# Infini-AI-Lab/TriForce

Measured on AMD Instinct MI355X. Metric: decode tokens/sec + avg accepted len, Llama-7B-128K @124K ctx, higher is better.
Workload: dtype f16

## Files before the change

### include/triforce_hip.h

```cpp
#ifndef TRIFORCE_HIP_H
#define TRIFORCE_HIP_H

#include <stdint.h>

#ifdef __cplusplus
extern "C" {
#endif

#define TF_OK        0
#define TF_EINVAL  (-22)
#define TF_ENOSPC  (-28)
#define TF_ERANGE  (-34)

int tf_abi_version(void);

int64_t tf_attn_decode_ws_floats(int H, int sq, int D, int nsplit);
int tf_attn_decode_pick_nsplit(int H, int sk);
int tf_attn_decode(const void* q, const void* k, const void* v, void* out,
                   int64_t stride_t, int64_t stride_h,
                   int sq, int sk, const int32_t* sk_dev, int H, int D, float scale,
                   int nsplit, float* ws, int64_t ws_floats, void* stream);
int tf_attn_decode_fused(const void* q, const void* k, const void* v, void* out,
                         int64_t stride_t, int64_t stride_h,
                         int sq, int sk, const int32_t* sk_dev, int H, int D, float scale,
                         int nsplit, float* ws, int64_t ws_floats, uint32_t* tickets, void* stream);
int tf_attn_decode_act(const void* q, const void* k, const void* v, void* out, int64_t out_sm, int64_t out_sk,
                       int64_t stride_t, int64_t stride_h, int sq, int sk, const int32_t* sk_dev, int H, int D,
                       float scale, int nsplit, float* ws, int64_t ws_floats, uint32_t* tickets, void* stream);
int tf_attn_tune(int key, int value);

int64_t tf_attn_block_ws_floats(int H, int D, int nsplit);
int tf_attn_block_pick_nsplit(int H, int sq, int sk);
int tf_attn_block(const void* q, const void* k, const void* v, void* out,
                  int64_t stride_t, int64_t stride_h, int sq, int sk, int H, int D, float scale,
                  int nsplit, float* ws, int64_t ws_floats,
                  const uint32_t* mask, int mask_words, int mask_row0, int tree_start, void* stream);

int tf_attn_prefill_pick_nsplit(int H, int sq, int sk);
int64_t tf_attn_prefill_ws_floats(int H, int sq, int D, int nsplit);
int tf_attn_prefill(const void* q, const void* k, const void* v, void* out,
                    int64_t stride_t, int64_t stride_h, int sq, int sk, int H, int D, float scale,
                    int nsplit, float* ws, int64_t ws_floats, void* stream);

int tf_attn_rope_on_read(const void* q, const void* k, const void* v, const void* cos, const void* sin,
                         void* out, int64_t stride_t, int64_t stride_h,
                         int sq, int kv_len, int H, int D, float scale, void* stream);

#define TF_DRAFT_MAX_LAYERS 8
typedef struct TfDraftModel {
    const void* embed;
    const void* ln1[TF_DRAFT_MAX_LAYERS];
    const void* wqkv[TF_DRAFT_MAX_LAYERS];
    const void* wo[TF_DRAFT_MAX_LAYERS];
    const void* ln2[TF_DRAFT_MAX_LAYERS];
    const void* wgate[TF_DRAFT_MAX_LAYERS];
    const void* wup[TF_DRAFT_MAX_LAYERS];
    const void* wdown[TF_DRAFT_MAX_LAYERS];
    const void* norm;
    const void* lm_head;
    const void* cos;
    const void* sin;
    int32_t layers, hidden, heads, head_dim, inter, vocab;
    float eps, scale;
} TfDraftModel;
typedef struct TfDraftCache {
    void* k[TF_DRAFT_MAX_LAYERS];
    void* v[TF_DRAFT_MAX_LAYERS];
    int64_t stride_t, stride_h;
} TfDraftCache;
int64_t tf_draft_forward_ws_bytes(const TfDraftModel* model, int n);
int tf_draft_forward_68m(const TfDraftModel* model, const TfDraftCache* cache, const int64_t* ids, int n, int slot0,
                         int kv_len, float* logits_out, float* probs_out, float temperature, float top_p,
                         void* ws, int64_t ws_bytes, void* stream);

int64_t tf_draft_persist_ctl_bytes(void);
int64_t tf_draft_persist_ws_bytes(const TfDraftModel* model);
int tf_draft_persist_supported(const TfDraftModel* model, int n, int kv_len);
int tf_draft_forward_68m_persist(const TfDraftModel* model, const TfDraftCache* cache, const int64_t* ids, int n, int slot0,
                                 int kv_len, float* logits_out, float* probs_out, float temperature, float top_p,
                                 void* ws, int64_t ws_bytes, void* ctl, void* stream);
int tf_draft_persist_tune(int key, int value);
int tf_draft_persist_stamps(void* buf);
int tf_draft_persist_error(const void* ctl);
int tf_draft_persist_reset(void* ctl, void* host_mirror, int set_mirror);

int tf_retrieval_score(const void* k, int64_t stride_t, int64_t stride_h, const void* q,
                       void* scores, int C, int chunk, int H, int D, void* stream);
int tf_retrieval_topk(const void* scores, int32_t* idx, int C, int sets, int H, void* stream);
int tf_retrieval_gather(const void* k_src, const void* v_src, int64_t src_stride_t, int64_t src_stride_h,
                        const int32_t* idx, void* k_dst, void* v_dst, int64_t dst_stride_t,
                        int64_t dst_stride_h, int sets, int chunk, int H, int D, void* stream);

int tf_chunk_mean(const void* k, int64_t stride_t, int64_t stride_h, void* index_layer, int64_t index_stride_h,
                  int c0, int c1, int chunk, int H, int D, void* stream);
int tf_retrieval_score_indexed(const void* index_layer, int64_t index_stride_h, const void* q, void* scores,
                               int C, int H, int D, void* stream);

int tf_kv_copy_rows(const void* src, int64_t src_stride_l, int64_t src_stride_t, int64_t src_stride_h,
                    void* dst, int64_t dst_stride_l, int64_t dst_stride_t, int64_t dst_stride_h,
                    int src_t0, int dst_t0, int n, int L, int H, int D, void* stream);
int tf_kv_shift_rows(void* cache, int64_t stride_l, int64_t stride_t, int64_t stride_h,
                     int src_t0, int dst_t0, int n, int L, int H, int D, void* stream);
int tf_kv_copy_rows_pair(const void* src_k, const void* src_v, int64_t src_stride_l, int64_t src_stride_t,
                         int64_t src_stride_h, void* dst_k, void* dst_v, int64_t dst_stride_l, int64_t dst_stride_t,
                         int64_t dst_stride_h, int src_t0, int dst_t0, int n, int L, int H, int D, void* stream);
int tf_kv_shift_rows_pair(void* k_cache, void* v_cache, int64_t stride_l, int64_t stride_t, int64_t stride_h,
                          int src_t0, int dst_t0, int n, int L, int H, int D, void* stream);

int tf_kv_gather_rows(void* k_cache, void* v_cache, int64_t stride_l, int64_t stride_t, int64_t stride_h,
                      int offset, const int32_t* idx, int n, int L, int H, int D, void* stream);

int tf_rmsnorm(const void* x, const void* res, const void* w, void* y, void* sum_out,
               int rows, int hidden, float eps, void* stream);
int tf_rope_append(const void* qkv, int64_t qkv_row_stride, const void* cos, const void* sin,
                   const int64_t* positions, void* q_out, void* k_cache, void* v_cache,
                   int64_t stride_t, int64_t stride_h, int slot0, const int32_t* slot0_dev,
                   int rows, int H, int D, int rotate_k, void* stream);
int tf_silu_mul(const void* gate_up, void* out, int rows, int I, void* stream);
int tf_embed_rows(const void* embed, const int64_t* ids, void* out, int64_t out_sm, int64_t out_sk, int n, int hidden,
                  int vocab, void* stream);
int tf_set_tokens(int64_t* dst, int n_dst, const int64_t* host_vals, int n_vals, int64_t pad, int64_t* pos, int n_pos,
                  int64_t pos0, int32_t* slot, int32_t* sk, int32_t sk_val, void* stream);

int tf_skinny_gemm(const void* w_packed, const void* x, int64_t ldx, void* y, int64_t ldy, int M, int N, int K,
                   int out_f32, void* stream);
int tf_skinny_gemm_swiglu(const void* gate_packed, const void* up_packed, const void* x, int64_t ldx, void* act,
                          int64_t ldy, int M, int I, int K, void* stream);

int tf_skinny_gemm_ex(const void* w_packed, const void* x, int64_t ldx, const void* ln_w, float eps,
                      const float* ss_in, const void* resid, int64_t ldr, float* ss_out, void* y, int64_t ldy,
                      int M, int N, int K, int out_f32, void* stream);
int tf_skinny_gemm_swiglu_ex(const void* gate_packed, const void* up_packed, const void* x, int64_t ldx,
                             const void* ln_w, float eps, const float* ss_in, void* act, int64_t ldy,
                             int M, int I, int K, void* stream);
int tf_skinny_qkv_rope(const void* wqkv_packed, const void* x, int64_t ldx, const void* ln_w, float eps,
                       const float* ss_in, const void* cos, const void* sin, const int64_t* positions, void* q_out,
                       void* k_cache, void* v_cache, int64_t stride_t, int64_t stride_h, int slot0,
                       const int32_t* slot0_dev, int M, int H, int D, int K, int rotate_k, void* stream);

int tf_skinny_gemm_act(const void* w_packed, const void* x, int64_t xs_m, int64_t xs_k, const void* ln_w, float eps,
                       const float* ss_in, const void* resid, int64_t rs_m, int64_t rs_k, float* ss_out, void* y,
                       int64_t ys_m, int64_t ys_k, int M, int N, int K, int out_f32, void* stream);
int tf_skinny_gemm_swiglu_act(const void* gate_packed, const void* up_packed, const void* x, int64_t xs_m,
                              int64_t xs_k, const void* ln_w, float eps, const float* ss_in, void* act, int64_t ys_m,
                              int64_t ys_k, int M, int I, int K, void* stream);
int tf_skinny_qkv_rope_act(const void* wqkv_packed, const void* x, int64_t xs_m, int64_t xs_k, const void* ln_w,
                           float eps, const float* ss_in, const void* cos, const void* sin, const int64_t* positions,
                           void* q_out, void* k_cache, void* v_cache, int64_t stride_t, int64_t stride_h, int slot0,
                           const int32_t* slot0_dev, int M, int H, int D, int K, int rotate_k, void* stream);
int tf_sg_tune(int key, int value);
int tf_skinny_gemm_swiglu_n8(const void* gate_n8, const void* up_n8, const void* x, int64_t xs_m, int64_t xs_k,
                             const void* ln_w, float eps, const float* ss_in, void* act, int64_t ys_m, int64_t ys_k,
                             int M, int I, int K, void* stream);
int tf_skinny_qkv_rope_n8(const void* wqkv_n8, const void* x, int64_t xs_m, int64_t xs_k, const void* ln_w, float eps,
                          const float* ss_in, const void* cos, const void* sin, const int64_t* positions, void* q_out,
                          void* k_cache, void* v_cache, int64_t stride_t, int64_t stride_h, int slot0,
                          const int32_t* slot0_dev, int M, int H, int D, int K, int rotate_k, void* stream);
int tf_skinny_gemm_fp8_act(const void* w_fp8, const float* scale, const void* x, int64_t xs_m, int64_t xs_k,
                           const void* ln_w, float eps, const float* ss_in, const void* resid, int64_t rs_m, int64_t rs_k,
                           float* ss_out, void* y, int64_t ys_m, int64_t ys_k, int M, int N, int K, int out_f32,
                           void* stream);
int tf_skinny_gemm_swiglu_fp8_act(const void* gate_fp8, const float* gate_scale, const void* up_fp8,
                                  const float* up_scale, const void* x, int64_t xs_m, int64_t xs_k, const void* ln_w,
                                  float eps, const float* ss_in, void* act, int64_t ys_m, int64_t ys_k, int M, int I, int K,
                                  void* stream);
int tf_skinny_qkv_rope_fp8_act(const void* wqkv_fp8, const float* scale, const void* x, int64_t xs_m, int64_t xs_k,
                               const void* ln_w, float eps, const float* ss_in, const void* cos, const void* sin,
                               const int64_t* positions, void* q_out, void* k_cache, void* v_cache, int64_t stride_t,
                               int64_t stride_h, int slot0, const int32_t* slot0_dev, int M, int H, int D, int K,
                               int rotate_k, void* stream);
int tf_kv_quant_rows(const void* k_in, const void* v_in, int64_t in_stride_t, int64_t in_stride_h, void* k_codes,
                     void* v_codes, void* k_exp, void* v_exp, int64_t code_stride_t, int64_t code_stride_h,
                     int64_t exp_stride_h, int slot0, const int32_t* slot0_dev, int n, int H, int D, void* k_deq,
                     void* v_deq, void* stream);
int tf_attn_decode_fp8_act(const void* q, const void* k_codes, const void* v_codes, const void* k_exp, const void* v_exp,
                           void* out, int64_t out_sm, int64_t out_sk, int64_t stride_t, int64_t stride_h,
                           int64_t exp_stride_h, int sq, int sk, const int32_t* sk_dev, int H, int D, float scale,
                           int nsplit, float* ws, int64_t ws_floats, uint32_t* tickets, void* stream);
int tf_kv_dequant_rows_pair(const void* src_k, const void* src_v, int64_t src_stride_l, int64_t src_stride_t,
                            int64_t src_stride_h, const void* exp_k, const void* exp_v, int64_t exp_stride_l,
                            int64_t exp_stride_h, void* dst_k, void* dst_v, int64_t dst_stride_l, int64_t dst_stride_t,
                            int64_t dst_stride_h, int src_t0, int dst_t0, int n, int L, int H, int D, void* stream);
int tf_retrieval_gather_fp8(const void* k_src, const void* v_src, int64_t src_stride_t, int64_t src_stride_h,
                            const void* k_src_exp, const void* v_src_exp, int64_t src_exp_stride_h, const int32_t* idx,
                            void* k_codes, void* v_codes, void* k_exp, void* v_exp, int64_t code_stride_t,
                            int64_t code_stride_h, int64_t exp_stride_h, int sets, int chunk, int H, int D, void* stream);
int tf_kv_quant_rows_pair(const void* src_k, const void* src_v, int64_t src_stride_l, int64_t src_stride_t,
                          int64_t src_stride_h, const void* src_exp_k, const void* src_exp_v, int64_t src_exp_stride_l,
                          int64_t src_exp_stride_h, void* k_codes, void* v_codes, int64_t code_stride_l,
                          int64_t code_stride_t, int64_t code_stride_h, void* k_exp, void* v_exp, int64_t exp_stride_l,
                          int64_t exp_stride_h, int src_t0, int dst_t0, int n, int L, int H, int D, void* stream);
int tf_attn_decode_fp8_tail_act(const void* q, const void* k_codes, const void* v_codes, const void* k_exp, const void* v_exp,
                                const void* k_tail, const void* v_tail, void* out, int64_t out_sm, int64_t out_sk,
                                int64_t stride_t, int64_t stride_h, int64_t exp_stride_h, int64_t tail_stride_t,
                                int64_t tail_stride_h, int sq, int sk_codes, int n_tail, const int32_t* sk_dev, int H, int D,
                                float scale, int nsplit, float* ws, int64_t ws_floats, uint32_t* tickets, void* stream);
int tf_sg_workspace(void* ws, int64_t bytes);

int tf_topp_probs(const float* logits, float* probs, int rows, int V, float temperature, float top_p, void* stream);
int tf_topk_topp_probs(const float* logits, float* probs, int rows, int V, float temperature, int top_k, float top_p,
                       void* stream);
int tf_sample_inverse_cdf(const float* probs, const float* u, int64_t* token_out, int V, void* stream);
int tf_accept_chain(const float* p, const float* q, const int64_t* tokens, const float* uniforms,
                    int g2, int V, int inclusive, int64_t eos_token_id, int64_t* out, void* stream);
int tf_middle_accept(const float* p, const float* q_d, int64_t* tokens, const float* uniforms,
                     int n, int gamma, int V, int64_t* out, void* stream);
int tf_mid_record_tokens(const int64_t* rec, int64_t* tokens, int tokens_len, int n, void* stream);
int64_t tf_topp_multi_ctl_bytes(void);
int64_t tf_topp_multi_ws_bytes(int rows, int V);
int tf_topp_probs_multi(const float* logits, const float* panel_max, float* probs, int rows, int V, float temperature,
                        float top_p, void* ctl, void* ws, int64_t ws_bytes, void* stream);
int tf_topp_multi_tune(int key, int value);
int tf_topp_multi_error(const void* ctl);
int tf_topp_multi_reset(void* ctl);

int tf_sample_inverse_cdf_cur(const float* probs, const float* ubuf, const int64_t* cursor, int off, int64_t* token_out,
                              int V, void* stream);
int tf_middle_accept_cur(const float* p, const float* q_d, int64_t* tokens, int tokens_len, const float* ubuf,
                         int64_t* cursor, int n, int gamma, int V, int64_t* out, void* stream);
int tf_accept_chain_cur(const float* p, const float* q, const int64_t* tokens, const float* ubuf, int64_t* cursor, int g2,
                        int V, int inclusive, int64_t eos_token_id, int64_t* out, void* stream);
int tf_accept_chain_step(const float* p, const float* q, int64_t* tok_buf, int tok_len, const float* ubuf, int64_t* cursor,
                         int g2, int V, int inclusive, int64_t eos_token_id, int64_t pad, const int32_t* s_src, int nsets,
                         int64_t* pos_a, int n_pos_a, int32_t* slot_a, int32_t* sk_a, int qlen_a, int64_t* pos_b, int n_pos_b,
                         int32_t* slot_b, int32_t* sk_b, int qlen_b, int64_t* out, void* stream);

int tf_tree_accept(const float* p_rows, const float* draft_logits, const int64_t* tokens,
                   const int32_t* succ_off, const int32_t* succ, const float* uniforms, int V,
                   float temperature, int64_t* out, void* stream);

int tf_sample_without_replacement(const float* logits, const void* rand_f16, int64_t* out, int rows, int V, int k,
                                  float temperature, void* stream);

int tf_kv_h2d_async(void* dst_dev, int64_t dst_pitch_elems, const void* src_host, int64_t src_pitch_elems,
                    int64_t width_elems, int H, void* copy_stream);
int tf_kv_d2h_async(void* dst_host, int64_t dst_pitch_elems, const void* src_dev, int64_t src_pitch_elems,
                    int64_t width_elems, int H, void* copy_stream);

int tf_ar_flags_bytes(void);
int tf_ar_ipc_handle_bytes(void);
int tf_ar_alloc(int64_t bytes, void** ptr);
int tf_ar_free(void* ptr);
int tf_ar_get_ipc_handle(void* ptr, void* handle_out);
int tf_ar_open_ipc_handle(const void* handle, void** ptr_out);
int tf_ar_close_ipc_handle(void* ptr);
int tf_allreduce_oneshot(void* const* peer_data, void* const* peer_flags, int rank, int world, void* out, int64_t n,
                         void* stream);
int tf_allreduce_oneshot_add(void* const* peer_data, void* const* peer_flags, int rank, int world, const void* resid,
                             void* out, int64_t n, void* stream);
int tf_allreduce_oneshot_add_ss(void* const* peer_data, void* const* peer_flags, int rank, int world, const void* resid,
                                void* out, int64_t n, int hidden, float* ss_out, void* stream);
int tf_allreduce_oneshot_alt(void* const* peer_data, void* const* peer_flags, int rank, int world, const void* resid,
                             void* out, int64_t n, int hidden, float* ss_out, int64_t half_elems, int expect_half,
                             void* stream);
int tf_allreduce_oneshot_act(void* const* peer_data, void* const* peer_flags, int rank, int world, const void* resid,
                             void* out, int64_t n, int hidden, int pack_rows, float* ss_out, int64_t half_elems,
                             int expect_half, void* stream);
int64_t tf_xchg_ctl_bytes(void);
int tf_skinny_gemm_xchg(const void* w_packed, const void* x, int64_t xs_m, int64_t xs_k, void* const* peer_stage,
                        void* const* peer_ctl, int rank, int world, int64_t half_elems, const void* resid, int64_t rs_m,
                        int64_t rs_k, void* out, int64_t os_m, int64_t os_k, float* ss_out, int M, int N, int K,
                        void* stream);
int tf_xchg_error(const void* ctl);
int tf_xchg_set_error(void* ctl, int code, void* host_mirror, int set_mirror);
int tf_xchg_tune(int key, int value);
int tf_xchg_reset(void* ctl);
int tf_ar_litmus_stage(void* staging, int64_t n, int rank, uint32_t* it_dev, void* stream);
int tf_ar_litmus_check(const void* out, int64_t n, int world, const uint32_t* it_dev, uint64_t* bad, void* stream);
int tf_ar_error(const void* flags_local);
int64_t tf_ar_epoch(const void* flags_local);
int tf_ar_set_error_mirror(void* flags_local, void* host_word);
int tf_ar_inject_error(void* flags_local, int code);

int tf_attn_decode_gqa_act(const void* q, const void* k, const void* v, void* out, int64_t out_sm, int64_t out_sk,
                           int64_t stride_t, int64_t stride_h, int sq, int sk, const int32_t* sk_dev, int H, int Hkv, int D,
                           float scale, int nsplit, float* ws, int64_t ws_floats, uint32_t* tickets, void* stream);
int tf_attn_prefill_gqa(const void* q, const void* k, const void* v, void* out, int64_t stride_t, int64_t stride_h,
                        int sq, int sk, int H, int Hkv, int D, float scale, int nsplit, float* ws, int64_t ws_floats,
                        void* stream);
int tf_skinny_qkv_rope_gqa_act(const void* wqkv_packed, const void* x, int64_t xs_m, int64_t xs_k, const void* ln_w,
                               float eps, const float* ss_in, const void* cos, const void* sin, const int64_t* positions,
                               void* q_out, void* k_cache, void* v_cache, int64_t stride_t, int64_t stride_h, int slot0,
                               const int32_t* slot0_dev, int M, int H, int Hkv, int D, int K, int rotate_k, void* stream);
int tf_rope_append_gqa(const void* qkv, int64_t qkv_row_stride, const void* cos, const void* sin,
                       const int64_t* positions, void* q_out, void* k_cache, void* v_cache,
                       int64_t stride_t, int64_t stride_h, int slot0, const int32_t* slot0_dev,
                       int rows, int H, int Hkv, int D, int rotate_k, void* stream);

#ifdef __cplusplus
}
#endif
#endif
```

### triforce_amd/build.py

```python
import os
import shutil
import subprocess

HERE = os.path.dirname(os.path.abspath(__file__))
CSRC = os.path.join(HERE, "csrc")
LIB_DIR = os.path.join(HERE, "lib")
LIB_PATH = os.path.join(LIB_DIR, "libtriforce_hip.so")
SOURCES = ["attn.hip", "retrieval.hip", "elementwise.hip", "sampling.hip", "offload.hip", "gemv.hip", "gemv_fp8.hip", "kv_fp8.hip", "allreduce.hip", "draft.hip", "draft_persist.hip", "topp_multi.hip", "abi.hip"]
FLAGS = ["--offload-arch=gfx950", "-O3", "-std=c++17", "-fPIC", "-shared", "-ffp-contract=off",
         "-fno-gpu-rdc", "-Wno-unused-result", "-mllvm", "-amdgpu-kernarg-preload-count=14"]


def hipcc_path():
    p = shutil.which("hipcc") or "/opt/rocm/bin/hipcc"
    if not os.path.exists(p):
        raise RuntimeError("hipcc not found: cannot build libtriforce_hip.so")
    return p


def sources():
    return [os.path.join(CSRC, s) for s in SOURCES if os.path.exists(os.path.join(CSRC, s))]


def needs_build():
    if not os.path.exists(LIB_PATH):
        return True
    t = os.path.getmtime(LIB_PATH)
    deps = sources() + [os.path.join(CSRC, "common.h"), os.path.join(CSRC, "tree_mask.h"), os.path.join(CSRC, "select_common.h"),
                        os.path.join(CSRC, "sg_rule.h"),
                        os.path.join(HERE, "..", "include", "triforce_hip.h"), os.path.abspath(__file__)]
    return any(os.path.getmtime(d) > t for d in deps if os.path.exists(d))


def build_variant(name, defines, verbose=True):
    out = os.path.join(LIB_DIR, f"libtriforce_hip_{name}.so")
    drop = {d[1:] for d in defines if d.startswith("!")}
    flags = [f for f in FLAGS if f not in drop]
    if "kernarg-preload" in drop:
        flags = [f for f in flags if f != "-mllvm" and not f.startswith("-amdgpu-kernarg-preload-count")]
    cmd = [hipcc_path()] + flags + [d if d.startswith("-") else f"-D{d}" for d in defines if not d.startswith("!")] \
        + sources() + ["-o", out]
    if verbose:
        print("[triforce_amd.build]", " ".join(cmd), flush=True)
    subprocess.run(cmd, check=True)
    return out


def build_library(force=False, verbose=True):
    if not force and not needs_build():
        return LIB_PATH
    os.makedirs(LIB_DIR, exist_ok=True)
    cmd = [hipcc_path()] + FLAGS + sources() + ["-o", LIB_PATH]
    if verbose:
        print("[triforce_amd.build]", " ".join(cmd), flush=True)
    subprocess.run(cmd, check=True)
    return LIB_PATH


if __name__ == "__main__":
    build_library(force=True)
```

### triforce_amd/csrc/gemv.hip

```cpp
#include "common.h"
#include "sg_rule.h"

#define SG_LOAD(p) __builtin_nontemporal_load(p)

constexpr int SG_U = 4;

struct SgAct {
    int64_t sm, sk;
};

struct SgKsplit {
    float* ws;
    unsigned* tickets;
    unsigned long long* stamps;
};
#ifndef SG_STAMPS
#define SG_STAMPS 0
#endif
#if SG_STAMPS
#define SG_STAMP(i)                                                                                                      \
    do {                                                                                                                 \
        if (tid == 0 && kx.stamps) {                                                                                     \
            kx.stamps[((int64_t)blockIdx.x * gridDim.y + blockIdx.y) * 16 + (i)] = __builtin_readcyclecounter();        \
            if ((i) == 0 || (i) == 6) kx.stamps[((int64_t)blockIdx.x * gridDim.y + blockIdx.y) * 16 + 8 + (i) / 6] = wall_clock64(); \
        }                                                                                                                \
    } while (0)
#else
#define SG_STAMP(i) do { } while (0)
#endif
static void* g_sg_ws[16] = {};
static int64_t g_sg_ws_bytes[16] = {};
#define SG_WS_SLOTS 4
static hipStream_t g_sg_slot_stream[16][SG_WS_SLOTS] = {};
static int g_sg_slots_used[16] = {};
#include <mutex>
static std::mutex g_sg_slot_mutex;
static int sg_slot_of(int dev, hipStream_t st) {
    std::lock_guard<std::mutex> lock(g_sg_slot_mutex);
    for (int i = 0; i < g_sg_slots_used[dev]; ++i)
        if (g_sg_slot_stream[dev][i] == st) return i;
    if (g_sg_slots_used[dev] >= SG_WS_SLOTS) return -1;
    g_sg_slot_stream[dev][g_sg_slots_used[dev]] = st;
    return g_sg_slots_used[dev]++;
}

static SgKnobs g_sg_knobs;

__device__ __forceinline__ void sg_st_agent(float* p, float v) { __hip_atomic_store(p, v, __ATOMIC_RELAXED, __HIP_MEMORY_SCOPE_AGENT); }
__device__ __forceinline__ float sg_ld_agent(const float* p) { return __hip_atomic_load(p, __ATOMIC_RELAXED, __HIP_MEMORY_SCOPE_AGENT); }

#define XC_MAXP 512
#define XC_MAX_WORLD 8
#define XC_SPIN_LIMIT (1u << 27)
#define XC_WALL_HZ 100000000ull
static int g_xc_timeout_ms = 5000;
static int g_xc_fence = 0;
struct XcCtl {
    unsigned epoch, ticket, error, pad;
    unsigned long long mirror;
};
#define XC_PEPOCH_OFF (1024 + XC_MAX_WORLD * XC_MAXP * 4)
struct SgXchg {
    h16* stage[XC_MAX_WORLD];
    unsigned* pf[XC_MAX_WORLD];
    XcCtl* ctl;
    unsigned* pepoch;
    int64_t half_elems;
    int rank, world;
    int fence;
    unsigned long long timeout_ticks;
};
__device__ __forceinline__ unsigned xc_ld(const unsigned* p) { return __hip_atomic_load(p, __ATOMIC_RELAXED, __HIP_MEMORY_SCOPE_SYSTEM); }
__device__ __forceinline__ void xc_st(unsigned* p, unsigned v) { __hip_atomic_store(p, v, __ATOMIC_RELAXED, __HIP_MEMORY_SCOPE_SYSTEM); }
__device__ __forceinline__ void xc_st8(h16* p, half4 v) {
    __hip_atomic_store(reinterpret_cast<unsigned long long*>(p), __builtin_bit_cast(unsigned long long, v), __ATOMIC_RELAXED,
                       __HIP_MEMORY_SCOPE_SYSTEM);
}
__device__ __forceinline__ half4 xc_ld8(const h16* p) {
    return __builtin_bit_cast(half4, __hip_atomic_load(reinterpret_cast<const unsigned long long*>(p), __ATOMIC_RELAXED,
                                                       __HIP_MEMORY_SCOPE_SYSTEM));
}

struct SgRope {
    const h16* cosb;
    const h16* sinb;
    const int64_t* positions;
    h16* q_out;
    h16* k_cache;
    h16* v_cache;
    int64_t stride_t, stride_h;
    const int32_t* slot0_dev;
    int slot0, H, D, rotate_k;
};

template <int MODE>
__device__ __forceinline__ void sg_rope_heads(const SgRope& rp, int& H, int& Hkv) {
    if (MODE == SG_QKVG) {
        H = rp.H & 0xffff;
        Hkv = rp.H >> 16;
    } else {
        H = Hkv = rp.H;
    }
}

__device__ __forceinline__ half8 sg_normalise(half8 xv, half8 wv, float inv) {
    half8 o;
#pragma unroll
    for (int e = 0; e < 8; ++e) o[e] = hmul_rn(wv[e], (h16)((float)xv[e] * inv));
    return o;
}

template <int MT, int MODE, bool NORM, int WAVES, int P, bool KSPLIT, bool XCHG = false>
__global__ __launch_bounds__(WAVES * 64) void skinny_gemm_kernel(const half8* __restrict__ wp,
                                                                 const half8* __restrict__ wp_up,
                                                                 const h16* __restrict__ x,
                                                                 const float* __restrict__ ss_in,
                                                                 const h16* __restrict__ ln_w, int K, int M,
                                                                 int xa_sm, int xa_sk, float eps, int N,
                                                                 const h16* resid, SgAct ra, void* yv, SgAct ya,
                                                                 SgRope rp, float* __restrict__ ss_out, SgKsplit kx,
                                                                 SgXchg xc) {
    const SgAct xa = {(int64_t)xa_sm, (int64_t)xa_sk};
    static_assert(!XCHG || (MODE == SG_PLAIN && P == 1 && !KSPLIT), "the exchange form is the plain one-panel GEMM");
    constexpr bool GATEUP = MODE == SG_GATEUP;
    constexpr int NA = GATEUP ? 2 : 1;
    constexpr int U = (P * NA >= 2) ? (8 / (P * NA)) : SG_U;
    static_assert(P <= WAVES && U >= 1, "one epilogue wave per panel");
    const int panel0 = blockIdx.x * P;
    const int tid = threadIdx.x, lane = tid & 63, wave = tid >> 6;
    const int li = lane & 15, g = lane >> 4;
    SG_STAMP(0);
    const int nchunks = K >> 5;
    const int KS = KSPLIT ? (int)gridDim.y : 1, ks = KSPLIT ? (int)blockIdx.y : 0;
    const int g0c = (int)((int64_t)nchunks * ks / KS), g1c = (int)((int64_t)nchunks * (ks + 1) / KS);
    const int cpw = (g1c - g0c + WAVES - 1) / WAVES;
    const int c0 = g0c + wave * cpw, c1 = min(g1c, c0 + cpw);

    __shared__ float sm[WAVES][P * NA][MT][64][4];
    __shared__ float sm_ss[NORM ? WAVES : 1][MT][16];

    f32x4 acc[P][NA][MT];
#pragma unroll
    for (int j = 0; j < P; ++j)
#pragma unroll
        for (int a = 0; a < NA; ++a)
#pragma unroll
            for (int t = 0; t < MT; ++t) acc[j][a][t] = f32x4{0.f, 0.f, 0.f, 0.f};
    const int64_t pstride = (int64_t)nchunks * 64;
    const half8* wa = wp + (int64_t)panel0 * pstride + lane;
    const half8* wu = GATEUP ? (wp_up + (int64_t)panel0 * pstride + lane) : nullptr;
    const int64_t xcs = 4 * xa.sk;
    const h16* xr[MT];
    bool xok[MT];
#pragma unroll
    for (int t = 0; t < MT; ++t) {
        const int m = t * 16 + li;
        xok[t] = m < M;
        xr[t] = x + (int64_t)(xok[t] ? m : 0) * xa.sm + (int64_t)g * xa.sk;
    }
    const half8 zero8 = {0, 0, 0, 0, 0, 0, 0, 0};

    constexpr int SSB = MT == 1 ? 3 : 2;
    constexpr bool BPRE = MT == 1;
    constexpr int G = WAVES * 4;
    const int nparts = K >> 4;
    const int pg = tid >> 4, m16 = tid & 15;
    float ssv[MT][SSB][8], part0[MT];
    half8 a_pre[U][P][NA], b_pre[BPRE ? U : 1][MT];
    const bool pre = NORM && (c0 + U <= c1);
    if constexpr (NORM) {
        const float* ssp = ss_in ? ss_in : reinterpret_cast<const float*>(wp);
#pragma unroll
        for (int t = 0; t < MT; ++t)
#pragma unroll
            for (int bb = 0; bb < SSB; ++bb)
#pragma unroll
                for (int j = 0; j < 8; ++j) {
                    const int p = pg + bb * 8 * G + j * G;
                    const float v = ssp[(int64_t)min(p, nparts - 1) * 32 + t * 16 + m16];
                    ssv[t][bb][j] = (p < nparts) ? v : 0.f;
                }
        if constexpr (BPRE) {
#pragma unroll
            for (int u = 0; u < U; ++u) {
                const int cu = min(c0 + u, nchunks - 1);
#pragma unroll
                for (int t = 0; t < MT; ++t) {
                    const half8 v = load_half8(xr[t] + xcs * cu);
                    b_pre[u][t] = xok[t] ? v : zero8;
                }
            }
        }
#pragma unroll
        for (int u = 0; u < U; ++u) {
            const int cu = min(c0 + u, nchunks - 1);
#pragma unroll
            for (int j = 0; j < P; ++j) {
                a_pre[u][j][0] = SG_LOAD(wa + j * pstride + (int64_t)cu * 64);
                if (GATEUP) a_pre[u][j][NA - 1] = SG_LOAD(wu + j * pstride + (int64_t)cu * 64);
            }
        }
        asm volatile("" ::: "memory");
        __builtin_amdgcn_sched_barrier(0);
#pragma unroll
        for (int t = 0; t < MT; ++t) {
            float part = 0.f;
#pragma unroll
            for (int bb = 0; bb < SSB; ++bb)
#pragma unroll
                for (int j = 0; j < 8; ++j) part += ssv[t][bb][j];
            asm volatile("" : "+v"(part));
            part0[t] = part;
        }
        __builtin_amdgcn_sched_barrier(0);
    }

    SG_STAMP(1);
    float inv[MT];
#pragma unroll
    for (int t = 0; t < MT; ++t) inv[t] = 1.f;
    if (NORM) {
        float tot[MT];
        if (ss_in) {
            float* red = &sm[0][0][0][0][0];
#pragma unroll
            for (int t = 0; t < MT; ++t) {
                float part = part0[t];
                for (int p0 = pg + SSB * 8 * G; p0 < nparts; p0 += 8 * G) {
                    float v[8];
#pragma unroll
                    for (int j = 0; j < 8; ++j) {
                        const int p = p0 + j * G;
                        v[j] = (p < nparts) ? ss_in[(int64_t)p * 32 + t * 16 + m16] : 0.f;
                    }
#pragma unroll
                    for (int j = 0; j < 8; ++j) part += v[j];
                }
                red[(t * G + pg) * 16 + m16] = part;
            }
            __syncthreads();
#pragma unroll
            for (int t = 0; t < MT; ++t) {
                tot[t] = 0.f;
                for (int j = 0; j < G; ++j) tot[t] += red[(t * G + j) * 16 + li];
            }
            __syncthreads();
        } else {
            float ss[MT];
#pragma unroll
            for (int t = 0; t < MT; ++t) ss[t] = 0.f;
            const int cpa = (nchunks + WAVES - 1) / WAVES;
            const int n0 = wave * cpa, n1 = min(nchunks, n0 + cpa);
            int cc = n0;
            for (; cc + 8 <= n1; cc += 8) {
                half8 v[8][MT];
#pragma unroll
                for (int j = 0; j < 8; ++j)
#pragma unroll
                    for (int t = 0; t < MT; ++t) v[j][t] = xok[t] ? load_half8(xr[t] + xcs * (cc + j)) : zero8;
#pragma unroll
                for (int j = 0; j < 8; ++j)
#pragma unroll
                    for (int t = 0; t < MT; ++t)
#pragma unroll
                        for (int e = 0; e < 8; ++e) {
                            const float f = (float)v[j][t][e];
                            ss[t] = fmaf(f, f, ss[t]);
                        }
            }
            for (; cc < n1; ++cc) {
#pragma unroll
                for (int t = 0; t < MT; ++t) {
                    const half8 v = xok[t] ? load_half8(xr[t] + xcs * cc) : zero8;
#pragma unroll
                    for (int e = 0; e < 8; ++e) {
                        const float f = (float)v[e];
                        ss[t] = fmaf(f, f, ss[t]);
                    }
                }
            }
#pragma unroll
            for (int t = 0; t < MT; ++t) {
                ss[t] += __shfl_xor(ss[t], 16, 64);
                ss[t] += __shfl_xor(ss[t], 32, 64);
                if (g == 0) sm_ss[wave][t][li] = ss[t];
            }
            __syncthreads();
#pragma unroll
            for (int t = 0; t < MT; ++t) {
                tot[t] = 0.f;
#pragma unroll
                for (int w = 0; w < WAVES; ++w) tot[t] += sm_ss[w][t][li];
            }
        }
#pragma unroll
        for (int t = 0; t < MT; ++t) inv[t] = 1.0f / sqrtf(tot[t] / (float)K + eps);
    }

    SG_STAMP(2);
    const bool epi = wave < P;
    const int panel = panel0 + (epi ? wave : 0);

    unsigned xepoch = 0, xerr = 0;
    half4 rope_cs[MT], rope_sn[MT], res_pre[MT];
    int64_t r_off = 0, y_off = 0;
    bool res_early = false;
    auto prefetch_epi = [&]() {
        if constexpr (XCHG) {
            if (epi) {
                xepoch = xc_ld(&xc.pepoch[panel]) + 1u;
                xerr = xc_ld(&xc.ctl->error);
            }
        }
        if ((MODE == SG_QKV || MODE == SG_QKVG) && epi) {
            const int D = rp.D, pph = D >> 4;
            int H, Hkv;
            sg_rope_heads<MODE>(rp, H, Hkv);
            int sec = panel / (H * pph);
            if (MODE == SG_QKVG) sec = panel < H * pph ? 0 : (panel < (H + Hkv) * pph ? 1 : 2);
            const int pp = panel % pph;
            const int d = 8 * pp + 4 * (g & 1) + ((g >= 2) ? (D >> 1) : 0);
#pragma unroll
            for (int t = 0; t < MT; ++t) {
                const int m = t * 16 + li;
                rope_cs[t] = half4{0, 0, 0, 0};
                rope_sn[t] = half4{0, 0, 0, 0};
                if (m < M && sec != 2 && (sec == 0 || rp.rotate_k)) {
                    const int64_t pos = rp.positions[m];
                    rope_cs[t] = *reinterpret_cast<const half4*>(rp.cosb + pos * D + d);
                    rope_sn[t] = *reinterpret_cast<const half4*>(rp.sinb + pos * D + d);
                }
            }
        }
        r_off = (int64_t)(2 * panel + (g >> 1)) * ra.sk + 4 * (g & 1);
        y_off = (int64_t)(2 * panel + (g >> 1)) * ya.sk + 4 * (g & 1);
        res_early = MODE == SG_PLAIN && resid != nullptr && epi && (ra.sm % 4) == 0 &&
                    (ra.sk % 4) == 0 && (reinterpret_cast<uintptr_t>(resid) % 8) == 0;
        if (res_early) {
#pragma unroll
            for (int t = 0; t < MT; ++t) {
                const int m = t * 16 + li;
                res_pre[t] = half4{0, 0, 0, 0};
                if (m < M) res_pre[t] = *reinterpret_cast<const half4*>(resid + (int64_t)m * ra.sm + r_off);
            }
        }
    };
    constexpr bool EPI_LATE = !NORM;
    if (!EPI_LATE || !(c0 + U <= c1)) prefetch_epi();

    int c = c0;
    for (; c + U <= c1; c += U) {
        half8 a[U][P][NA], b[U][MT];
#pragma unroll
        for (int u = 0; u < U; ++u) {
#pragma unroll
            for (int j = 0; j < P; ++j) {
                if (NORM && c == c0 && pre) {
                    a[u][j][0] = a_pre[u][j][0];
                    if (GATEUP) a[u][j][NA - 1] = a_pre[u][j][NA - 1];
                } else {
                    a[u][j][0] = SG_LOAD(wa + j * pstride + (int64_t)(c + u) * 64);
                    if (GATEUP) a[u][j][NA - 1] = SG_LOAD(wu + j * pstride + (int64_t)(c + u) * 64);
                }
            }
#pragma unroll
            for (int t = 0; t < MT; ++t) {
                if (BPRE && NORM && c == c0 && pre) b[u][t] = b_pre[BPRE ? u : 0][t];
                else b[u][t] = xok[t] ? load_half8(xr[t] + xcs * (c + u)) : zero8;
                if (NORM) {
                    const half8 lw = load_half8(ln_w + 32 * (c + u) + 8 * g);
                    b[u][t] = sg_normalise(b[u][t], lw, inv[t]);
                }
            }
        }
        if constexpr (EPI_LATE) {
            if (c == c0) prefetch_epi();
        }
#pragma unroll
        for (int u = 0; u < U; ++u)
#pragma unroll
            for (int t = 0; t < MT; ++t)
#pragma unroll
                for (int j = 0; j < P; ++j)
#pragma unroll
                    for (int aa = 0; aa < NA; ++aa)
                        acc[j][aa][t] = __builtin_amdgcn_mfma_f32_16x16x32_f16(a[u][j][aa], b[u][t], acc[j][aa][t], 0, 0, 0);
#if SG_STAMPS
        if (c == c0) {
            asm volatile("s_nop 15\n\ts_nop 15" ::: "memory");
            SG_STAMP(3);
        }
#endif
    }
    SG_STAMP(4);
    if constexpr (NORM) {
        for (; c < c1; ++c) {
            half8 a[P][NA];
#pragma unroll
            for (int j = 0; j < P; ++j) {
                a[j][0] = SG_LOAD(wa + j * pstride + (int64_t)c * 64);
                if (GATEUP) a[j][NA - 1] = SG_LOAD(wu + j * pstride + (int64_t)c * 64);
            }
#pragma unroll
            for (int t = 0; t < MT; ++t) {
                half8 b = xok[t] ? load_half8(xr[t] + xcs * c) : zero8;
                if (NORM) b = sg_normalise(b, load_half8(ln_w + 32 * c + 8 * g), inv[t]);
#pragma unroll
                for (int j = 0; j < P; ++j)
#pragma unroll
                    for (int aa = 0; aa < NA; ++aa)
                        acc[j][aa][t] = __builtin_amdgcn_mfma_f32_16x16x32_f16(a[j][aa], b, acc[j][aa][t], 0, 0, 0);
            }
        }
    } else if (c < c1) {
        half8 a[U][P][NA], b[U][MT];
#pragma unroll
        for (int u = 0; u < U - 1; ++u) {
            const int cc = min(c + u, c1 - 1);
#pragma unroll
            for (int j = 0; j < P; ++j) {
                a[u][j][0] = SG_LOAD(wa + j * pstride + (int64_t)cc * 64);
                if (GATEUP) a[u][j][NA - 1] = SG_LOAD(wu + j * pstride + (int64_t)cc * 64);
            }
#pragma unroll
            for (int t = 0; t < MT; ++t) {
                b[u][t] = xok[t] ? load_half8(xr[t] + xcs * cc) : zero8;
                if (NORM) b[u][t] = sg_normalise(b[u][t], load_half8(ln_w + 32 * cc + 8 * g), inv[t]);
            }
        }
#pragma unroll
        for (int u = 0; u < U - 1; ++u)
            if (c + u < c1) {
#pragma unroll
                for (int t = 0; t < MT; ++t)
#pragma unroll
                    for (int j = 0; j < P; ++j)
#pragma unroll
                        for (int aa = 0; aa < NA; ++aa)
                            acc[j][aa][t] = __builtin_amdgcn_mfma_f32_16x16x32_f16(a[u][j][aa], b[u][t], acc[j][aa][t], 0, 0, 0);
            }
    }

#pragma unroll
    for (int j = 0; j < P; ++j)
#pragma unroll
        for (int aa = 0; aa < NA; ++aa)
#pragma unroll
            for (int t = 0; t < MT; ++t)
                *reinterpret_cast<f32x4*>(&sm[wave][j * NA + aa][t][lane][0]) = acc[j][aa][t];
    __syncthreads();
    SG_STAMP(5);
    if (!epi) return;
    float S[MT][4], S2[MT][4];
#pragma unroll
    for (int t = 0; t < MT; ++t) {
#pragma unroll
        for (int r = 0; r < 4; ++r) {
            S[t][r] = 0.f;
            S2[t][r] = 0.f;
        }
#pragma unroll
        for (int w = 0; w < WAVES; ++w) {
            const f32x4 v = *reinterpret_cast<const f32x4*>(&sm[w][wave * NA][t][lane][0]);
            f32x4 v2 = {0.f, 0.f, 0.f, 0.f};
            if (GATEUP) v2 = *reinterpret_cast<const f32x4*>(&sm[w][wave * NA + NA - 1][t][lane][0]);
#pragma unroll
            for (int r = 0; r < 4; ++r) {
                S[t][r] += v[r];
                if (GATEUP) S2[t][r] += v2[r];
            }
        }
    }
    if constexpr (KSPLIT) {
        float* base = kx.ws + ((int64_t)panel * KS * NA * MT) * 256 + lane * 4;
        float* mine = base + (int64_t)ks * NA * MT * 256;
#pragma unroll
        for (int t = 0; t < MT; ++t)
#pragma unroll
            for (int r = 0; r < 4; ++r) {
                sg_st_agent(mine + t * 256 + r, S[t][r]);
                if (GATEUP) sg_st_agent(mine + (MT + t) * 256 + r, S2[t][r]);
            }
        asm volatile("s_waitcnt vmcnt(0)" ::: "memory");
        unsigned tk = 0;
        if (lane == 0) tk = __hip_atomic_fetch_add(&kx.tickets[panel], 1u, __ATOMIC_RELAXED, __HIP_MEMORY_SCOPE_AGENT);
        tk = __builtin_amdgcn_readfirstlane(tk);
        if (tk != (unsigned)(KS - 1)) return;
        float P1[SG_KSPLIT_MAX][MT][4], P2[SG_KSPLIT_MAX][MT][4];
#pragma unroll
        for (int k = 0; k < SG_KSPLIT_MAX; ++k)
            if (k < KS) {
                const float* src = base + (int64_t)k * NA * MT * 256;
#pragma unroll
                for (int t = 0; t < MT; ++t)
#pragma unroll
                    for (int r = 0; r < 4; ++r) {
                        P1[k][t][r] = sg_ld_agent(src + t * 256 + r);
                        if (GATEUP) P2[k][t][r] = sg_ld_agent(src + (MT + t) * 256 + r);
                    }
            }
#pragma unroll
        for (int t = 0; t < MT; ++t)
#pragma unroll
            for (int r = 0; r < 4; ++r) {
                float a = 0.f, b = 0.f;
#pragma unroll
                for (int k = 0; k < SG_KSPLIT_MAX; ++k)
                    if (k < KS) {
                        a += P1[k][t][r];
                        if (GATEUP) b += P2[k][t][r];
                    }
                S[t][r] = a;
                S2[t][r] = b;
            }
        if (lane == 0) __hip_atomic_store(&kx.tickets[panel], 0u, __ATOMIC_RELAXED, __HIP_MEMORY_SCOPE_AGENT);
    }
    if constexpr (XCHG) {
        xepoch = __builtin_amdgcn_readfirstlane(xepoch);
        bool ok = __builtin_amdgcn_readfirstlane(xerr) == 0u;
        const int64_t hb = xc.half_elems * (int64_t)(xepoch & 1u);
        half4 part[MT];
#pragma unroll
        for (int t = 0; t < MT; ++t) {
#pragma unroll
            for (int r = 0; r < 4; ++r) part[t][r] = (h16)S[t][r];
            if (ok && t * 16 + li < M) xc_st8(xc.stage[xc.rank] + hb + (int64_t)(t * 16 + li) * ya.sm + y_off, part[t]);
        }
        asm volatile("s_waitcnt vmcnt(0)" ::: "memory");
        if (xc.fence) __builtin_amdgcn_fence(__ATOMIC_RELEASE, "");
        if (ok) {
            const bool peer = lane < xc.world && lane != xc.rank;
            if (peer) xc_st(xc.pf[lane] + xc.rank * XC_MAXP + panel, xepoch);
            bool seen = true;
            if (peer) {
                seen = false;
                const unsigned* slot = xc.pf[xc.rank] + lane * XC_MAXP + panel;
                const unsigned long long t0 = wall_clock64();
                for (unsigned spins = 0; spins < XC_SPIN_LIMIT; ++spins) {
                    if ((int)(xc_ld(slot) - xepoch) >= 0) { seen = true; break; }
                    __builtin_amdgcn_s_sleep(1);
                    if ((spins & 63u) == 63u && wall_clock64() - t0 > xc.timeout_ticks) break;
                }
            }
            ok = __builtin_amdgcn_ballot_w64(!seen) == 0ull;
            if (xc.fence) __builtin_amdgcn_fence(__ATOMIC_ACQUIRE, "");
            if (!ok && lane == 0) {
                xc_st(&xc.ctl->error, 1u);
                unsigned* mir = reinterpret_cast<unsigned*>(xc.ctl->mirror);
                if (mir) xc_st(mir, 1u);
            }
        }
        asm volatile("" ::: "memory");
#pragma unroll
        for (int t = 0; t < MT; ++t) {
            const bool rowv = t * 16 + li < M;
            half4 pv[XC_MAX_WORLD];
#pragma unroll
            for (int q = 0; q < XC_MAX_WORLD; ++q) {
                pv[q] = part[t];
                if (ok && rowv && q < xc.world && q != xc.rank)
                    pv[q] = xc_ld8(xc.stage[q] + hb + (int64_t)(t * 16 + li) * ya.sm + y_off);
            }
#pragma unroll
            for (int r = 0; r < 4; ++r) {
                float acc = 0.f;
#pragma unroll
                for (int q = 0; q < XC_MAX_WORLD; ++q)
                    if (q < xc.world) acc += (float)pv[q][r];
                S[t][r] = ok ? (float)(h16)acc : __builtin_nanf("");
            }
        }
    }
#pragma unroll
    for (int t = 0; t < MT; ++t) {
        const int m = t * 16 + li;
// ... 259 lines not shown
    for (int t = 0; t < MT; ++t) inv[t] = 1.0f / sqrtf(tot[t] / (float)K + eps);

    const bool epi = wave == 0;
    half4 rope_cs[MT], rope_sn[MT];
    if (MODE == SG_QKV && epi) {
        const int H = rp.H, D = rp.D, pph = D >> 3;
        const int sec = panel / (H * pph), pp = panel % pph;
        const int d = 4 * pp + ((g & 1) ? (D >> 1) : 0);
#pragma unroll
        for (int t = 0; t < MT; ++t) {
            const int m = t * 8 + lr;
            rope_cs[t] = half4{0, 0, 0, 0};
            rope_sn[t] = half4{0, 0, 0, 0};
            if (m < M && sec != 2 && (sec == 0 || rp.rotate_k)) {
                const int64_t pos = rp.positions[m];
                rope_cs[t] = *reinterpret_cast<const half4*>(rp.cosb + pos * D + d);
                rope_sn[t] = *reinterpret_cast<const half4*>(rp.sinb + pos * D + d);
            }
        }
    }

    auto compute = [&](int c) {
#pragma unroll
        for (int u = 0; u < U; ++u) {
            if (c + u < c1) {
#pragma unroll
                for (int t = 0; t < MT; ++t) {
                    const half8 bn = sg_normalise(b[u][t], lw[u], inv[t]);
#pragma unroll
                    for (int aa = 0; aa < NA; ++aa)
                        acc[aa][t] = __builtin_amdgcn_mfma_f32_16x16x32_f16(a[u][aa], bn, acc[aa][t], 0, 0, 0);
                }
            }
        }
    };
    compute(c0);
    for (int c = c0 + U; c < c1; c += U) {
#pragma unroll
        for (int u = 0; u < U; ++u) {
            const int cu = min(c + u, last);
#pragma unroll
            for (int t = 0; t < MT; ++t) {
                const half8 v = load_half8(xr[t] + xcs * cu);
                b[u][t] = xok[t] ? v : zero8;
            }
            lw[u] = load_half8(lnp + 64 * cu);
        }
#pragma unroll
        for (int u = 0; u < U; ++u) {
            const int cu = min(c + u, last);
            a[u][0] = SG_LOAD(wa + (int64_t)cu * 64);
            if (GATEUP) a[u][NA - 1] = SG_LOAD(wu + (int64_t)cu * 64);
        }
        compute(c);
    }

#pragma unroll
    for (int aa = 0; aa < NA; ++aa)
#pragma unroll
        for (int t = 0; t < MT; ++t) *reinterpret_cast<f32x4*>(&sm[wave][aa][t][lane][0]) = acc[aa][t];
    __syncthreads();
    if (!epi) return;
    const bool vl = g < 2 && li < 8;
    const int lo = vl ? lane : 0, hi_l = vl ? lane + 40 : 40;
    float S[MT][4], S2[MT][4];
#pragma unroll
    for (int t = 0; t < MT; ++t) {
#pragma unroll
        for (int r = 0; r < 4; ++r) {
            S[t][r] = 0.f;
            S2[t][r] = 0.f;
        }
#pragma unroll 2
        for (int w = 0; w < WAVES; ++w) {
            const f32x4 e0 = *reinterpret_cast<const f32x4*>(&sm[w][0][t][lo][0]);
            const f32x4 o0 = *reinterpret_cast<const f32x4*>(&sm[w][0][t][hi_l][0]);
#pragma unroll
            for (int r = 0; r < 4; ++r) S[t][r] += e0[r] + o0[r];
            if (GATEUP) {
                const f32x4 e1 = *reinterpret_cast<const f32x4*>(&sm[w][NA - 1][t][lo][0]);
                const f32x4 o1 = *reinterpret_cast<const f32x4*>(&sm[w][NA - 1][t][hi_l][0]);
#pragma unroll
                for (int r = 0; r < 4; ++r) S2[t][r] += e1[r] + o1[r];
            }
        }
    }
#pragma unroll
    for (int t = 0; t < MT; ++t) {
        const int m = t * 8 + lr;
        if (MODE == SG_QKV) {
            const int H = rp.H, D = rp.D, half = D >> 1, pph = D >> 3;
            const int sec = panel / (H * pph), hd = (panel / pph) % H, pp = panel % pph;
            h16 val[4], oth[4];
#pragma unroll
            for (int r = 0; r < 4; ++r) {
                val[r] = (h16)S[t][r];
                oth[r] = (h16)__shfl_xor((float)val[r], 16, 64);
            }
            if (!vl || m >= M) continue;
            const int slot = (rp.slot0_dev ? *rp.slot0_dev : rp.slot0) + m;
            half4 out;
            if (sec == 2) {
#pragma unroll
                for (int r = 0; r < 4; ++r) out[r] = val[r];
                h16* dst = rp.v_cache + (int64_t)slot * rp.stride_t + (int64_t)hd * rp.stride_h + 8 * pp + 4 * g;
                *reinterpret_cast<half4*>(dst) = out;
                continue;
            }
            const bool hi = g == 1;
            const int d = 4 * pp + (hi ? half : 0);
            if (sec == 0 || rp.rotate_k) {
#pragma unroll
                for (int r = 0; r < 4; ++r) {
                    const h16 cs = rope_cs[t][r], sn = rope_sn[t][r];
                    const h16 rh = hi ? oth[r] : (h16)(-(float)oth[r]);
                    out[r] = hadd_rn(hmul_rn(val[r], cs), hmul_rn(rh, sn));
                }
            } else {
#pragma unroll
                for (int r = 0; r < 4; ++r) out[r] = val[r];
            }
            h16* dst = (sec == 0) ? rp.q_out + ((int64_t)m * H + hd) * D + d
                                  : rp.k_cache + (int64_t)slot * rp.stride_t + (int64_t)hd * rp.stride_h + d;
            *reinterpret_cast<half4*>(dst) = out;
        } else {
            if (!vl || m >= M) continue;
            half4 o;
#pragma unroll
            for (int r = 0; r < 4; ++r) {
                const h16 gt = (h16)S[t][r], up = (h16)S2[t][r];
                const float gf = (float)gt;
                const h16 act = (h16)(gf / (1.0f + expf(-gf)));
                o[r] = hmul_rn(act, up);
            }
            h16* dst = (h16*)yv + (int64_t)m * ya.sm + (int64_t)panel * ya.sk + 4 * g;
            if (((ya.sm | ya.sk) % 4) == 0 && (reinterpret_cast<uintptr_t>(yv) % 8) == 0) {
                *reinterpret_cast<half4*>(dst) = o;
            } else {
#pragma unroll
                for (int r = 0; r < 4; ++r) dst[r] = o[r];
            }
        }
    }
}

struct SgArgs {
    const void *wp, *wp_up, *x, *ln_w, *resid;
    void* y;
    SgAct xa, ra, ya;
    float eps;
    int M, N, K;
    const float* ss_in;
    float* ss_out;
};

static unsigned long long* sg_stamps_ptr() {
#if SG_STAMPS
    int dev = 0;
    if (hipGetDevice(&dev) == hipSuccess && dev >= 0 && dev < 16 && g_sg_ws[dev] && g_sg_ws_bytes[dev] >= (6 << 20))
        return reinterpret_cast<unsigned long long*>(reinterpret_cast<char*>(g_sg_ws[dev]) + (4 << 20));
#endif
    return nullptr;
}

static int sg_ksplit(const SgArgs& a, const SgForm& f, int mode, SgKsplit& kx, hipStream_t st) {
    const int panels = a.N / 16, NA = mode == SG_GATEUP ? 2 : 1;
    const int ks = sg_pick_ks(panels, f.P, a.K >> 5, f.WAVES, mode, g_sg_knobs);
    int dev = 0;
    if (ks <= 1 || hipGetDevice(&dev) != hipSuccess || dev < 0 || dev >= 16 || !g_sg_ws[dev]) return 1;
    const int64_t need = (int64_t)SG_TICKETS * 4 + (int64_t)panels * ks * NA * f.MT * 256 * 4;
    const int64_t slot_bytes = (g_sg_ws_bytes[dev] / SG_WS_SLOTS) & ~(int64_t)255;
    if (need > slot_bytes) return 1;
    const int slot = sg_slot_of(dev, st);
    if (slot < 0) return 1;
    char* base = reinterpret_cast<char*>(g_sg_ws[dev]) + slot * slot_bytes;
    kx.tickets = reinterpret_cast<unsigned*>(base);
    kx.ws = reinterpret_cast<float*>(base + (int64_t)SG_TICKETS * 4);
    return ks;
}

template <int MT, int MODE, bool NORM, int WAVES, int P>
static int launch_sg_form(const SgArgs& a, const SgRope& rp, const SgKsplit& kx, int ks, hipStream_t st) {
    constexpr bool REACHABLE = MODE != SG_GATEUP || WAVES == SG_WAVES || MT == 2;
    constexpr bool CAN_SPLIT = P == 1 && MODE != SG_F32;
#define SG_LAUNCH(KSPLIT_)                                                                                                 \
    hipLaunchKernelGGL((skinny_gemm_kernel<MT, MODE, NORM, WAVES, P, KSPLIT_>), dim3(a.N / 16 / P, ks), dim3(WAVES * 64), 0, \
                       st, (const half8*)a.wp, (const half8*)a.wp_up, (const h16*)a.x, a.ss_in, (const h16*)a.ln_w, a.K,  \
                       a.M, (int)a.xa.sm, (int)a.xa.sk, a.eps, a.N, (const h16*)a.resid, a.ra, a.y, a.ya, rp, a.ss_out,  \
                       kx, SgXchg{})
    if constexpr (!REACHABLE) {
        return TF_EINVAL;
    } else {
        if (ks == 1) {
            SG_LAUNCH(false);
        } else if constexpr (CAN_SPLIT) {
            SG_LAUNCH(true);
        } else {
            return TF_EINVAL;
        }
        TF_LAUNCH_CHECK();
        return TF_OK;
    }
#undef SG_LAUNCH
}

template <int MODE, bool NORM>
static int launch_sg(const SgArgs& a, const SgRope& rp, hipStream_t st) {
    const SgForm f = sg_pick_form(MODE, NORM, a.M, a.N, a.K, g_sg_knobs);
    SgKsplit kx = {nullptr, nullptr, (f.P == 1 && MODE != SG_F32) ? sg_stamps_ptr() : nullptr};
    const int ks = sg_ksplit(a, f, MODE, kx, st);
#define SG_FORM(MT_, W_, P_) \
    if (f.MT == MT_ && f.WAVES == W_ && f.P == P_) return launch_sg_form<MT_, MODE, NORM, W_, P_>(a, rp, kx, ks, st)
    SG_FORM(1, SG_WAVES, 1);
    SG_FORM(2, SG_WAVES, 1);
    SG_FORM(1, SG_WAVES_WIDE, 1);
    SG_FORM(2, SG_WAVES_WIDE, 1);
    SG_FORM(1, SG_WAVES, 2);
    SG_FORM(2, SG_WAVES, 2);
#undef SG_FORM
    return TF_EINVAL;
}

static bool sg_act_ok(const SgAct& s) { return s.sm > 0 && s.sk > 0 && (s.sm % 8) == 0 && (s.sk % 8) == 0; }

static bool sg_shape_ok(int M, int N, int K, const SgAct& xa) {
    return M >= 1 && M <= 32 && N >= 16 && (N % 16) == 0 && K >= 32 && (K % 32) == 0 && sg_act_ok(xa) &&
           xa.sm <= 0x7fffffff && xa.sk <= 0x7fffffff;
}

extern "C" int tf_sg_tune(int key, int value) {
    SgKnobs& k = g_sg_knobs;
    int* slot = key == 0 ? &k.p2_rows : key == 2 ? &k.p2_groups : key == 3 ? &k.ksplit_max_groups
                : key == 4 ? &k.ksplit_force : key == 5 ? &k.few_panels : nullptr;
    if (!slot) return -1;
    const int old = *slot;
    *slot = value;
    return old;
}

extern "C" int tf_sg_workspace(void* ws, int64_t bytes) {
    int dev = 0;
    hipError_t e = hipGetDevice(&dev);
    if (e != hipSuccess) return (int)e;
    if (dev < 0 || dev >= 16 || (ws && bytes < (int64_t)SG_TICKETS * 4 + 4096) || (reinterpret_cast<uintptr_t>(ws) % 16)) return TF_EINVAL;
    g_sg_ws[dev] = ws;
    g_sg_ws_bytes[dev] = ws ? bytes : 0;
    {
        std::lock_guard<std::mutex> lock(g_sg_slot_mutex);
        g_sg_slots_used[dev] = 0;
    }
    return TF_OK;
}

extern "C" int tf_skinny_gemm_act(const void* w_packed, const void* x, int64_t xs_m, int64_t xs_k, const void* ln_w,
                                  float eps, const float* ss_in, const void* resid, int64_t rs_m, int64_t rs_k,
                                  float* ss_out, void* y, int64_t ys_m, int64_t ys_k, int M, int N, int K, int out_f32,
                                  void* stream) {
    SgArgs a = {};
    a.wp = w_packed, a.x = x, a.ln_w = ln_w, a.resid = resid, a.y = y;
    a.xa = SgAct{xs_m, xs_k}, a.ra = SgAct{rs_m, rs_k}, a.ya = SgAct{ys_m, ys_k};
    a.eps = eps, a.M = M, a.N = N, a.K = K, a.ss_in = ss_in, a.ss_out = ss_out;
    if (!w_packed || !x || !y || !sg_shape_ok(M, N, K, a.xa)) return TF_EINVAL;
    if ((out_f32 && (resid || ss_out)) || (ss_in && !ln_w)) return TF_EINVAL;
    if (ys_m <= 0 || (!out_f32 && ys_k <= 0) || (resid && (rs_m <= 0 || rs_k <= 0))) return TF_EINVAL;
    hipStream_t st = (hipStream_t)stream;
    const SgRope rp = {};
    if (out_f32) return ln_w ? launch_sg<SG_F32, true>(a, rp, st) : launch_sg<SG_F32, false>(a, rp, st);
    return ln_w ? launch_sg<SG_PLAIN, true>(a, rp, st) : launch_sg<SG_PLAIN, false>(a, rp, st);
}

extern "C" int tf_skinny_gemm_ex(const void* w_packed, const void* x, int64_t ldx, const void* ln_w, float eps,
                                 const float* ss_in, const void* resid, int64_t ldr, float* ss_out, void* y,
                                 int64_t ldy, int M, int N, int K, int out_f32, void* stream) {
    return tf_skinny_gemm_act(w_packed, x, ldx, 8, ln_w, eps, ss_in, resid, ldr, 8, ss_out, y, ldy, 8, M, N, K, out_f32,
                              stream);
}

extern "C" int tf_skinny_gemm(const void* w_packed, const void* x, int64_t ldx, void* y, int64_t ldy, int M, int N,
                              int K, int out_f32, void* stream) {
    return tf_skinny_gemm_ex(w_packed, x, ldx, nullptr, 0.f, nullptr, nullptr, 0, nullptr, y, ldy, M, N, K, out_f32, stream);
}

extern "C" int tf_skinny_gemm_swiglu_act(const void* gate_packed, const void* up_packed, const void* x, int64_t xs_m,
                                         int64_t xs_k, const void* ln_w, float eps, const float* ss_in, void* act,
                                         int64_t ys_m, int64_t ys_k, int M, int I, int K, void* stream) {
    SgArgs a = {};
    a.wp = gate_packed, a.wp_up = up_packed, a.x = x, a.ln_w = ln_w, a.y = act;
    a.xa = SgAct{xs_m, xs_k}, a.ya = SgAct{ys_m, ys_k}, a.ra = SgAct{8, 8};
    a.eps = eps, a.M = M, a.N = I, a.K = K, a.ss_in = ss_in;
    if (!gate_packed || !up_packed || !x || !act || !sg_shape_ok(M, I, K, a.xa) || (ss_in && !ln_w)) return TF_EINVAL;
    if (ys_m <= 0 || ys_k <= 0) return TF_EINVAL;
    hipStream_t st = (hipStream_t)stream;
    const SgRope rp = {};
    return ln_w ? launch_sg<SG_GATEUP, true>(a, rp, st) : launch_sg<SG_GATEUP, false>(a, rp, st);
}

extern "C" int tf_skinny_gemm_swiglu_ex(const void* gate_packed, const void* up_packed, const void* x, int64_t ldx,
                                        const void* ln_w, float eps, const float* ss_in, void* act, int64_t ldy, int M,
                                        int I, int K, void* stream) {
    return tf_skinny_gemm_swiglu_act(gate_packed, up_packed, x, ldx, 8, ln_w, eps, ss_in, act, ldy, 8, M, I, K, stream);
}

extern "C" int tf_skinny_gemm_swiglu(const void* gate_packed, const void* up_packed, const void* x, int64_t ldx,
                                     void* act, int64_t ldy, int M, int I, int K, void* stream) {
    return tf_skinny_gemm_swiglu_ex(gate_packed, up_packed, x, ldx, nullptr, 0.f, nullptr, act, ldy, M, I, K, stream);
}

extern "C" int tf_skinny_qkv_rope_act(const void* wqkv_packed, const void* x, int64_t xs_m, int64_t xs_k,
                                      const void* ln_w, float eps, const float* ss_in, const void* cosb,
                                      const void* sinb, const int64_t* positions, void* q_out, void* k_cache,
                                      void* v_cache, int64_t stride_t, int64_t stride_h, int slot0,
                                      const int32_t* slot0_dev, int M, int H, int D, int K, int rotate_k, void* stream) {
    if (!wqkv_packed || !x || !cosb || !sinb || !positions || !q_out || !k_cache || !v_cache) return TF_EINVAL;
    SgArgs a = {};
    a.wp = wqkv_packed, a.x = x, a.ln_w = ln_w;
    a.xa = SgAct{xs_m, xs_k}, a.ra = SgAct{8, 8}, a.ya = SgAct{8, 8};
    a.eps = eps, a.M = M, a.N = 3 * H * D, a.K = K, a.ss_in = ss_in;
    if (H < 1 || D < 32 || (D % 32) || !sg_shape_ok(M, a.N, K, a.xa) || (ss_in && !ln_w)) return TF_EINVAL;
    if ((stride_t % 4) || (stride_h % 4)) return TF_EINVAL;
    hipStream_t st = (hipStream_t)stream;
    SgRope rp;
    rp.cosb = (const h16*)cosb;
    rp.sinb = (const h16*)sinb;
    rp.positions = positions;
    rp.q_out = (h16*)q_out;
    rp.k_cache = (h16*)k_cache;
    rp.v_cache = (h16*)v_cache;
    rp.stride_t = stride_t;
    rp.stride_h = stride_h;
    rp.slot0_dev = slot0_dev;
    rp.slot0 = slot0;
    rp.H = H;
    rp.D = D;
    rp.rotate_k = rotate_k;
    return ln_w ? launch_sg<SG_QKV, true>(a, rp, st) : launch_sg<SG_QKV, false>(a, rp, st);
}

extern "C" int tf_skinny_qkv_rope_gqa_act(const void* wqkv_packed, const void* x, int64_t xs_m, int64_t xs_k,
                                          const void* ln_w, float eps, const float* ss_in, const void* cosb,
                                          const void* sinb, const int64_t* positions, void* q_out, void* k_cache,
                                          void* v_cache, int64_t stride_t, int64_t stride_h, int slot0,
                                          const int32_t* slot0_dev, int M, int H, int Hkv, int D, int K, int rotate_k,
                                          void* stream) {
    if (!wqkv_packed || !x || !cosb || !sinb || !positions || !q_out || !k_cache || !v_cache) return TF_EINVAL;
    if (H < 1 || Hkv < 1 || (H % Hkv) || H > 0x7fff || (D != 64 && D != 128)) return TF_EINVAL;
    SgArgs a = {};
    a.wp = wqkv_packed, a.x = x, a.ln_w = ln_w;
    a.xa = SgAct{xs_m, xs_k}, a.ra = SgAct{8, 8}, a.ya = SgAct{8, 8};
    a.eps = eps, a.M = M, a.N = (H + 2 * Hkv) * D, a.K = K, a.ss_in = ss_in;
    if (!sg_shape_ok(M, a.N, K, a.xa) || (ss_in && !ln_w)) return TF_EINVAL;
    if ((stride_t % 4) || (stride_h % 4)) return TF_EINVAL;
    hipStream_t st = (hipStream_t)stream;
    SgRope rp;
    rp.cosb = (const h16*)cosb;
    rp.sinb = (const h16*)sinb;
    rp.positions = positions;
    rp.q_out = (h16*)q_out;
    rp.k_cache = (h16*)k_cache;
    rp.v_cache = (h16*)v_cache;
    rp.stride_t = stride_t;
    rp.stride_h = stride_h;
    rp.slot0_dev = slot0_dev;
    rp.slot0 = slot0;
    rp.H = H | (Hkv << 16);
    rp.D = D;
    rp.rotate_k = rotate_k;
    return ln_w ? launch_sg<SG_QKVG, true>(a, rp, st) : launch_sg<SG_QKVG, false>(a, rp, st);
}

extern "C" int tf_skinny_qkv_rope(const void* wqkv_packed, const void* x, int64_t ldx, const void* ln_w, float eps,
                                  const float* ss_in, const void* cosb, const void* sinb, const int64_t* positions,
                                  void* q_out, void* k_cache, void* v_cache, int64_t stride_t, int64_t stride_h,
                                  int slot0, const int32_t* slot0_dev, int M, int H, int D, int K, int rotate_k,
                                  void* stream) {
    return tf_skinny_qkv_rope_act(wqkv_packed, x, ldx, 8, ln_w, eps, ss_in, cosb, sinb, positions, q_out, k_cache,
                                  v_cache, stride_t, stride_h, slot0, slot0_dev, M, H, D, K, rotate_k, stream);
}

static bool sg_n8_ok(int M, int N, int K, const SgAct& xa) {
    return M >= 1 && M <= 24 && N >= 8 && (N % 8) == 0 && K >= 64 * 2 * SG_N8_WAVES && (K % 64) == 0 && sg_act_ok(xa) &&
           xa.sm <= 0x7fffffff && xa.sk <= 0x7fffffff;
}

template <int MODE>
static int launch_sg_n8(const SgArgs& a, const SgRope& rp, hipStream_t st) {
    const SgN8Form f = sg_pick_n8(MODE, a.M, a.K);
#define N8_FORM(MT_, U_, FOR_)                                                                                               \
    if constexpr (FOR_) {                                                                                                    \
        if (f.MT == MT_ && f.U == U_) {                                                                                      \
            hipLaunchKernelGGL((skinny_gemm_n8_kernel<MT_, MODE, SG_N8_WAVES, U_>), dim3(a.N / 8), dim3(SG_N8_WAVES * 64), 0, \
                               st, (const half8*)a.wp, (const half8*)a.wp_up, (const h16*)a.x, a.ss_in, (const h16*)a.ln_w,   \
                               a.K, a.M, (int)a.xa.sm, (int)a.xa.sk, a.eps, a.y, a.ya, rp);                                  \
            TF_LAUNCH_CHECK();                                                                                               \
            return TF_OK;                                                                                                    \
        }                                                                                                                    \
    }
    N8_FORM(1, 5, true)
    N8_FORM(1, 8, true)
    N8_FORM(2, 5, true)
    N8_FORM(3, 5, true)
    N8_FORM(2, 4, MODE == SG_GATEUP)
    N8_FORM(3, 4, MODE == SG_GATEUP)
    N8_FORM(2, 8, MODE != SG_GATEUP)
#undef N8_FORM
    return TF_EINVAL;
}

extern "C" int tf_skinny_gemm_swiglu_n8(const void* gate_n8, const void* up_n8, const void* x, int64_t xs_m, int64_t xs_k,
                                        const void* ln_w, float eps, const float* ss_in, void* act, int64_t ys_m,
                                        int64_t ys_k, int M, int I, int K, void* stream) {
    SgArgs a = {};
    a.wp = gate_n8, a.wp_up = up_n8, a.x = x, a.ln_w = ln_w, a.y = act;
    a.xa = SgAct{xs_m, xs_k}, a.ya = SgAct{ys_m, ys_k}, a.ra = SgAct{8, 8};
    a.eps = eps, a.M = M, a.N = I, a.K = K, a.ss_in = ss_in;
    if (!gate_n8 || !up_n8 || !x || !act || !ln_w || !sg_n8_ok(M, I, K, a.xa)) return TF_EINVAL;
    if (ys_m <= 0 || ys_k <= 0) return TF_EINVAL;
    const SgRope rp = {};
    return launch_sg_n8<SG_GATEUP>(a, rp, (hipStream_t)stream);
}

extern "C" int tf_skinny_qkv_rope_n8(const void* wqkv_n8, const void* x, int64_t xs_m, int64_t xs_k, const void* ln_w,
                                     float eps, const float* ss_in, const void* cosb, const void* sinb,
                                     const int64_t* positions, void* q_out, void* k_cache, void* v_cache, int64_t stride_t,
                                     int64_t stride_h, int slot0, const int32_t* slot0_dev, int M, int H, int D, int K,
                                     int rotate_k, void* stream) {
    if (!wqkv_n8 || !x || !ln_w || !cosb || !sinb || !positions || !q_out || !k_cache || !v_cache) return TF_EINVAL;
    SgArgs a = {};
    a.wp = wqkv_n8, a.x = x, a.ln_w = ln_w;
    a.xa = SgAct{xs_m, xs_k}, a.ra = SgAct{8, 8}, a.ya = SgAct{8, 8};
    a.eps = eps, a.M = M, a.N = 3 * H * D, a.K = K, a.ss_in = ss_in;
    if (H < 1 || D < 32 || (D % 32) || !sg_n8_ok(M, a.N, K, a.xa)) return TF_EINVAL;
    if ((stride_t % 4) || (stride_h % 4)) return TF_EINVAL;
    SgRope rp;
    rp.cosb = (const h16*)cosb;
    rp.sinb = (const h16*)sinb;
    rp.positions = positions;
    rp.q_out = (h16*)q_out;
    rp.k_cache = (h16*)k_cache;
    rp.v_cache = (h16*)v_cache;
    rp.stride_t = stride_t;
    rp.stride_h = stride_h;
    rp.slot0_dev = slot0_dev;
    rp.slot0 = slot0;
    rp.H = H;
    rp.D = D;
    rp.rotate_k = rotate_k;
    return launch_sg_n8<SG_QKV>(a, rp, (hipStream_t)stream);
}

extern "C" int64_t tf_xchg_ctl_bytes(void) { return XC_PEPOCH_OFF + (int64_t)XC_MAXP * 4; }

extern "C" int tf_skinny_gemm_xchg(const void* w_packed, const void* x, int64_t xs_m, int64_t xs_k,
                                   void* const* peer_stage, void* const* peer_ctl, int rank, int world, int64_t half_elems,
                                   const void* resid, int64_t rs_m, int64_t rs_k, void* out, int64_t os_m, int64_t os_k,
                                   float* ss_out, int M, int N, int K, void* stream) {
    SgArgs a = {};
    a.wp = w_packed, a.x = x, a.resid = resid, a.y = out;
    a.xa = SgAct{xs_m, xs_k}, a.ra = SgAct{rs_m, rs_k}, a.ya = SgAct{os_m, os_k};
    a.M = M, a.N = N, a.K = K, a.ss_out = ss_out;
    if (!w_packed || !x || !out || !peer_stage || !peer_ctl || !sg_shape_ok(M, N, K, a.xa) || !sg_act_ok(a.ya)) return TF_EINVAL;
    if (world < 1 || world > XC_MAX_WORLD || rank < 0 || rank >= world || N / 16 > XC_MAXP) return TF_EINVAL;
    if (half_elems < 8 || (half_elems % 8) || (resid && !sg_act_ok(a.ra))) return TF_EINVAL;
    const int64_t last = (int64_t)(M - 1) * os_m + (int64_t)(N / 8 - 1) * os_k + 7;
    if (last >= half_elems) return TF_EINVAL;
    SgXchg xc = {};
    for (int r = 0; r < world; ++r) {
        if (!peer_stage[r] || !peer_ctl[r]) return TF_EINVAL;
        xc.stage[r] = (h16*)peer_stage[r];
        xc.pf[r] = reinterpret_cast<unsigned*>(reinterpret_cast<char*>(peer_ctl[r]) + 1024);
    }
    xc.ctl = reinterpret_cast<XcCtl*>(peer_ctl[rank]);
    xc.pepoch = reinterpret_cast<unsigned*>(reinterpret_cast<char*>(peer_ctl[rank]) + XC_PEPOCH_OFF);
    xc.half_elems = half_elems, xc.rank = rank, xc.world = world;
    xc.fence = g_xc_fence;
    xc.timeout_ticks = (unsigned long long)(g_xc_timeout_ms > 0 ? g_xc_timeout_ms : 1) * (XC_WALL_HZ / 1000ull);
    if ((const void*)out == (const void*)xc.stage[rank] || (const void*)resid == (const void*)xc.stage[rank]) return TF_EINVAL;
    hipStream_t st = (hipStream_t)stream;
    const SgRope rp = {};
    const SgKsplit kx = {nullptr, nullptr, sg_stamps_ptr()};
    const bool wide = sg_xchg_waves(K) == SG_WAVES_WIDE;
#define XCHG_LAUNCH(MT_, W_)                                                                                                  \
    hipLaunchKernelGGL((skinny_gemm_kernel<MT_, SG_PLAIN, false, W_, 1, false, true>), dim3(N / 16), dim3(W_ * 64), 0, st, \
                       (const half8*)a.wp, (const half8*)nullptr, (const h16*)a.x, (const float*)nullptr,              \
                       (const h16*)nullptr, a.K, a.M, (int)a.xa.sm, (int)a.xa.sk, 0.f, a.N, (const h16*)a.resid, a.ra, a.y, a.ya, rp, a.ss_out, \
                       kx, xc)
    if (M <= 16) {
        if (wide) XCHG_LAUNCH(1, SG_WAVES_WIDE);
        else XCHG_LAUNCH(1, SG_WAVES);
    } else {
        if (wide) XCHG_LAUNCH(2, SG_WAVES_WIDE);
        else XCHG_LAUNCH(2, SG_WAVES);
    }
#undef XCHG_LAUNCH
    TF_LAUNCH_CHECK();
    return TF_OK;
}

extern "C" int tf_xchg_tune(int key, int value) {
    int* slot = key == 0 ? &g_xc_fence : key == 1 ? &g_xc_timeout_ms : nullptr;
    if (!slot) return -1;
    const int old = *slot;
    if (key == 0 && value != 0 && value != 1) return old;
    if (key == 1 && value < 1) return old;
    *slot = value;
    return old;
}

extern "C" int tf_xchg_reset(void* ctl) {
    if (!ctl) return TF_EINVAL;
    hipError_t e = hipDeviceSynchronize();
    if (e != hipSuccess) return (int)e;
    XcCtl c;
    e = hipMemcpy(&c, ctl, sizeof(c), hipMemcpyDeviceToHost);
    if (e != hipSuccess) return (int)e;
    const unsigned long long mirror = c.mirror;
    e = hipMemset(ctl, 0, (size_t)tf_xchg_ctl_bytes());
    if (e != hipSuccess) return (int)e;
    e = hipMemcpy(&reinterpret_cast<XcCtl*>(ctl)->mirror, &mirror, sizeof(mirror), hipMemcpyHostToDevice);
    if (e != hipSuccess) return (int)e;
    if (mirror) *reinterpret_cast<volatile unsigned*>(mirror) = 0u;
    return (int)hipDeviceSynchronize();
}

extern "C" int tf_xchg_error(const void* ctl) {
    if (!ctl) return TF_EINVAL;
    XcCtl c;
    hipError_t e = hipMemcpy(&c, ctl, sizeof(c), hipMemcpyDeviceToHost);
    return e == hipSuccess ? (int)c.error : (int)e;
}
extern "C" int tf_xchg_set_error(void* ctl, int code, void* host_mirror, int set_mirror) {
    if (!ctl || code < 0) return TF_EINVAL;
    XcCtl* c = reinterpret_cast<XcCtl*>(ctl);
    const unsigned v = (unsigned)code;
    hipError_t e = hipMemcpy(&c->error, &v, sizeof(v), hipMemcpyHostToDevice);
    if (e != hipSuccess) return (int)e;
    if (set_mirror) {
        const unsigned long long m = (unsigned long long)(uintptr_t)host_mirror;
        e = hipMemcpy(&c->mirror, &m, sizeof(m), hipMemcpyHostToDevice);
        if (e != hipSuccess) return (int)e;
    }
    unsigned long long m = 0;
    e = hipMemcpy(&m, &c->mirror, sizeof(m), hipMemcpyDeviceToHost);
    if (e != hipSuccess) return (int)e;
    if (m) *reinterpret_cast<volatile unsigned*>(m) = v;
    return TF_OK;
}
```

### triforce_amd/hip.py

```python
import ctypes
import os

from .build import LIB_PATH

_c = ctypes
_vp, _i32, _i64, _f32 = _c.c_void_p, _c.c_int, _c.c_int64, _c.c_float

SIGNATURES = {
    "tf_abi_version": (_i32, []),
    "tf_attn_decode_ws_floats": (_i64, [_i32, _i32, _i32, _i32]),
    "tf_attn_decode_pick_nsplit": (_i32, [_i32, _i32]),
    "tf_attn_decode": (_i32, [_vp, _vp, _vp, _vp, _i64, _i64, _i32, _i32, _vp, _i32, _i32, _f32, _i32, _vp, _i64, _vp]),
    "tf_attn_decode_fused": (_i32, [_vp, _vp, _vp, _vp, _i64, _i64, _i32, _i32, _vp, _i32, _i32, _f32, _i32, _vp, _i64, _vp,
                                    _vp]),
    "tf_attn_decode_act": (_i32, [_vp, _vp, _vp, _vp, _i64, _i64, _i64, _i64, _i32, _i32, _vp, _i32, _i32, _f32, _i32, _vp,
                                  _i64, _vp, _vp]),
    "tf_attn_tune": (_i32, [_i32, _i32]),
    "tf_attn_block_ws_floats": (_i64, [_i32, _i32, _i32]),
    "tf_attn_block_pick_nsplit": (_i32, [_i32, _i32, _i32]),
    "tf_attn_prefill_pick_nsplit": (_i32, [_i32, _i32, _i32]),
    "tf_attn_prefill_ws_floats": (_i64, [_i32, _i32, _i32, _i32]),
    "tf_attn_prefill": (_i32, [_vp, _vp, _vp, _vp, _i64, _i64, _i32, _i32, _i32, _i32, _f32, _i32, _vp, _i64, _vp]),
    "tf_attn_block": (_i32, [_vp, _vp, _vp, _vp, _i64, _i64, _i32, _i32, _i32, _i32, _f32, _i32, _vp, _i64, _vp, _i32,
                             _i32, _i32, _vp]),
    "tf_attn_rope_on_read": (_i32, [_vp, _vp, _vp, _vp, _vp, _vp, _i64, _i64, _i32, _i32, _i32, _i32, _f32, _vp]),
    "tf_retrieval_score": (_i32, [_vp, _i64, _i64, _vp, _vp, _i32, _i32, _i32, _i32, _vp]),
    "tf_retrieval_topk": (_i32, [_vp, _vp, _i32, _i32, _i32, _vp]),
    "tf_retrieval_gather": (_i32, [_vp, _vp, _i64, _i64, _vp, _vp, _vp, _i64, _i64, _i32, _i32, _i32, _i32, _vp]),
    "tf_chunk_mean": (_i32, [_vp, _i64, _i64, _vp, _i64, _i32, _i32, _i32, _i32, _i32, _vp]),
    "tf_retrieval_score_indexed": (_i32, [_vp, _i64, _vp, _vp, _i32, _i32, _i32, _vp]),
    "tf_kv_copy_rows": (_i32, [_vp, _i64, _i64, _i64, _vp, _i64, _i64, _i64, _i32, _i32, _i32, _i32, _i32, _i32, _vp]),
    "tf_kv_shift_rows": (_i32, [_vp, _i64, _i64, _i64, _i32, _i32, _i32, _i32, _i32, _i32, _vp]),
    "tf_kv_copy_rows_pair": (_i32, [_vp, _vp, _i64, _i64, _i64, _vp, _vp, _i64, _i64, _i64, _i32, _i32, _i32, _i32, _i32,
                                    _i32, _vp]),
    "tf_kv_shift_rows_pair": (_i32, [_vp, _vp, _i64, _i64, _i64, _i32, _i32, _i32, _i32, _i32, _i32, _vp]),
    "tf_kv_gather_rows": (_i32, [_vp, _vp, _i64, _i64, _i64, _i32, _vp, _i32, _i32, _i32, _i32, _vp]),
    "tf_tree_accept": (_i32, [_vp, _vp, _vp, _vp, _vp, _vp, _i32, _f32, _vp, _vp]),
    "tf_sample_without_replacement": (_i32, [_vp, _vp, _vp, _i32, _i32, _i32, _f32, _vp]),
    "tf_rmsnorm": (_i32, [_vp, _vp, _vp, _vp, _vp, _i32, _i32, _f32, _vp]),
    "tf_rope_append": (_i32, [_vp, _i64, _vp, _vp, _vp, _vp, _vp, _vp, _i64, _i64, _i32, _vp, _i32, _i32, _i32, _i32, _vp]),
    "tf_silu_mul": (_i32, [_vp, _vp, _i32, _i32, _vp]),
    "tf_embed_rows": (_i32, [_vp, _vp, _vp, _i64, _i64, _i32, _i32, _i32, _vp]),
    "tf_set_tokens": (_i32, [_vp, _i32, _vp, _i32, _i64, _vp, _i32, _i64, _vp, _vp, _i32, _vp]),
    "tf_skinny_gemm": (_i32, [_vp, _vp, _i64, _vp, _i64, _i32, _i32, _i32, _i32, _vp]),
    "tf_skinny_gemm_ex": (_i32, [_vp, _vp, _i64, _vp, _f32, _vp, _vp, _i64, _vp, _vp, _i64, _i32, _i32, _i32, _i32, _vp]),
    "tf_skinny_gemm_swiglu_ex": (_i32, [_vp, _vp, _vp, _i64, _vp, _f32, _vp, _vp, _i64, _i32, _i32, _i32, _vp]),
    "tf_skinny_qkv_rope": (_i32, [_vp, _vp, _i64, _vp, _f32, _vp, _vp, _vp, _vp, _vp, _vp, _vp, _i64, _i64, _i32, _vp,
                                  _i32, _i32, _i32, _i32, _i32, _vp]),
    "tf_skinny_gemm_swiglu": (_i32, [_vp, _vp, _vp, _i64, _vp, _i64, _i32, _i32, _i32, _vp]),
    "tf_skinny_gemm_act": (_i32, [_vp, _vp, _i64, _i64, _vp, _f32, _vp, _vp, _i64, _i64, _vp, _vp, _i64, _i64, _i32, _i32,
                                  _i32, _i32, _vp]),
    "tf_skinny_gemm_swiglu_act": (_i32, [_vp, _vp, _vp, _i64, _i64, _vp, _f32, _vp, _vp, _i64, _i64, _i32, _i32, _i32, _vp]),
    "tf_skinny_qkv_rope_act": (_i32, [_vp, _vp, _i64, _i64, _vp, _f32, _vp, _vp, _vp, _vp, _vp, _vp, _vp, _i64, _i64, _i32,
                                      _vp, _i32, _i32, _i32, _i32, _i32, _vp]),
    "tf_skinny_gemm_swiglu_n8": (_i32, [_vp, _vp, _vp, _i64, _i64, _vp, _f32, _vp, _vp, _i64, _i64, _i32, _i32, _i32, _vp]),
    "tf_skinny_qkv_rope_n8": (_i32, [_vp, _vp, _i64, _i64, _vp, _f32, _vp, _vp, _vp, _vp, _vp, _vp, _vp, _i64, _i64, _i32,
                                     _vp, _i32, _i32, _i32, _i32, _i32, _vp]),
    "tf_sg_tune": (_i32, [_i32, _i32]),
    "tf_skinny_gemm_fp8_act": (_i32, [_vp, _vp, _vp, _i64, _i64, _vp, _f32, _vp, _vp, _i64, _i64, _vp, _vp, _i64, _i64, _i32,
                                      _i32, _i32, _i32, _vp]),
    "tf_skinny_gemm_swiglu_fp8_act": (_i32, [_vp, _vp, _vp, _vp, _vp, _i64, _i64, _vp, _f32, _vp, _vp, _i64, _i64, _i32, _i32,
                                             _i32, _vp]),
    "tf_skinny_qkv_rope_fp8_act": (_i32, [_vp, _vp, _vp, _i64, _i64, _vp, _f32, _vp, _vp, _vp, _vp, _vp, _vp, _vp, _i64, _i64,
                                          _i32, _vp, _i32, _i32, _i32, _i32, _i32, _vp]),
    "tf_sg_workspace": (_i32, [_vp, _i64]),
    "tf_kv_quant_rows": (_i32, [_vp, _vp, _i64, _i64, _vp, _vp, _vp, _vp, _i64, _i64, _i64, _i32, _vp, _i32, _i32, _i32, _vp,
                                _vp, _vp]),
    "tf_attn_decode_fp8_act": (_i32, [_vp, _vp, _vp, _vp, _vp, _vp, _i64, _i64, _i64, _i64, _i64, _i32, _i32, _vp, _i32, _i32,
                                      _f32, _i32, _vp, _i64, _vp, _vp]),
    "tf_kv_dequant_rows_pair": (_i32, [_vp, _vp, _i64, _i64, _i64, _vp, _vp, _i64, _i64, _vp, _vp, _i64, _i64, _i64, _i32, _i32,
                                       _i32, _i32, _i32, _i32, _vp]),
    "tf_retrieval_gather_fp8": (_i32, [_vp, _vp, _i64, _i64, _vp, _vp, _i64, _vp, _vp, _vp, _vp, _vp, _i64, _i64, _i64, _i32, _i32,
                                       _i32, _i32, _vp]),
    "tf_kv_quant_rows_pair": (_i32, [_vp, _vp, _i64, _i64, _i64, _vp, _vp, _i64, _i64, _vp, _vp, _i64, _i64, _i64, _vp, _vp, _i64,
                                     _i64, _i32, _i32, _i32, _i32, _i32, _i32, _vp]),
    "tf_attn_decode_fp8_tail_act": (_i32, [_vp, _vp, _vp, _vp, _vp, _vp, _vp, _vp, _i64, _i64, _i64, _i64, _i64, _i64, _i64, _i32,
                                           _i32, _i32, _vp, _i32, _i32, _f32, _i32, _vp, _i64, _vp, _vp]),
    "tf_topp_probs": (_i32, [_vp, _vp, _i32, _i32, _f32, _f32, _vp]),
    "tf_topk_topp_probs": (_i32, [_vp, _vp, _i32, _i32, _f32, _i32, _f32, _vp]),
    "tf_sample_inverse_cdf": (_i32, [_vp, _vp, _vp, _i32, _vp]),
    "tf_accept_chain": (_i32, [_vp, _vp, _vp, _vp, _i32, _i32, _i32, _i64, _vp, _vp]),
    "tf_middle_accept": (_i32, [_vp, _vp, _vp, _vp, _i32, _i32, _i32, _vp, _vp]),
    "tf_mid_record_tokens": (_i32, [_vp, _vp, _i32, _i32, _vp]),
    "tf_sample_inverse_cdf_cur": (_i32, [_vp, _vp, _vp, _i32, _vp, _i32, _vp]),
    "tf_middle_accept_cur": (_i32, [_vp, _vp, _vp, _i32, _vp, _vp, _i32, _i32, _i32, _vp, _vp]),
    "tf_accept_chain_step": (_i32, [_vp, _vp, _vp, _i32, _vp, _vp, _i32, _i32, _i32, _i64, _i64, _vp, _i32,
                                    _vp, _i32, _vp, _vp, _i32, _vp, _i32, _vp, _vp, _i32, _vp, _vp]),
    "tf_accept_chain_cur": (_i32, [_vp, _vp, _vp, _vp, _vp, _i32, _i32, _i32, _i64, _vp, _vp]),
    "tf_kv_h2d_async": (_i32, [_vp, _i64, _vp, _i64, _i64, _i32, _vp]),
    "tf_kv_d2h_async": (_i32, [_vp, _i64, _vp, _i64, _i64, _i32, _vp]),
    "tf_ar_flags_bytes": (_i32, []),
    "tf_ar_ipc_handle_bytes": (_i32, []),
    "tf_ar_alloc": (_i32, [_i64, _vp]),
    "tf_ar_free": (_i32, [_vp]),
    "tf_ar_get_ipc_handle": (_i32, [_vp, _vp]),
    "tf_ar_open_ipc_handle": (_i32, [_vp, _vp]),
    "tf_ar_close_ipc_handle": (_i32, [_vp]),
    "tf_allreduce_oneshot": (_i32, [_vp, _vp, _i32, _i32, _vp, _i64, _vp]),
    "tf_allreduce_oneshot_add": (_i32, [_vp, _vp, _i32, _i32, _vp, _vp, _i64, _vp]),
    "tf_allreduce_oneshot_add_ss": (_i32, [_vp, _vp, _i32, _i32, _vp, _vp, _i64, _i32, _vp, _vp]),
    "tf_allreduce_oneshot_alt": (_i32, [_vp, _vp, _i32, _i32, _vp, _vp, _i64, _i32, _vp, _i64, _i32, _vp]),
    "tf_allreduce_oneshot_act": (_i32, [_vp, _vp, _i32, _i32, _vp, _vp, _i64, _i32, _i32, _vp, _i64, _i32, _vp]),
    "tf_ar_litmus_stage": (_i32, [_vp, _i64, _i32, _vp, _vp]),
    "tf_ar_litmus_check": (_i32, [_vp, _i64, _i32, _vp, _vp, _vp]),
    "tf_xchg_ctl_bytes": (_i64, []),
    "tf_skinny_gemm_xchg": (_i32, [_vp, _vp, _i64, _i64, _vp, _vp, _i32, _i32, _i64, _vp, _i64, _i64, _vp, _i64, _i64, _vp,
                                   _i32, _i32, _i32, _vp]),
    "tf_xchg_error": (_i32, [_vp]),
    "tf_xchg_set_error": (_i32, [_vp, _i32, _vp, _i32]),
    "tf_xchg_tune": (_i32, [_i32, _i32]),
    "tf_xchg_reset": (_i32, [_vp]),
    "tf_ar_error": (_i32, [_vp]),
    "tf_ar_epoch": (_i64, [_vp]),
    "tf_ar_set_error_mirror": (_i32, [_vp, _vp]),
    "tf_ar_inject_error": (_i32, [_vp, _i32]),
}

TF_DRAFT_MAX_LAYERS = 8


class TfDraftModel(_c.Structure):
    _fields_ = ([("embed", _vp)] + [(n, _vp * TF_DRAFT_MAX_LAYERS) for n in
                                    ("ln1", "wqkv", "wo", "ln2", "wgate", "wup", "wdown")]
                + [("norm", _vp), ("lm_head", _vp), ("cos", _vp), ("sin", _vp)]
                + [(n, _i32) for n in ("layers", "hidden", "heads", "head_dim", "inter", "vocab")]
                + [("eps", _f32), ("scale", _f32)])


class TfDraftCache(_c.Structure):
    _fields_ = [("k", _vp * TF_DRAFT_MAX_LAYERS), ("v", _vp * TF_DRAFT_MAX_LAYERS), ("stride_t", _i64), ("stride_h", _i64)]


SIGNATURES["tf_draft_forward_ws_bytes"] = (_i64, [_c.POINTER(TfDraftModel), _i32])
SIGNATURES["tf_draft_forward_68m"] = (_i32, [_c.POINTER(TfDraftModel), _c.POINTER(TfDraftCache), _vp, _i32, _i32, _i32, _vp,
                                             _vp, _f32, _f32, _vp, _i64, _vp])
SIGNATURES["tf_topp_multi_ctl_bytes"] = (_i64, [])
SIGNATURES["tf_topp_multi_ws_bytes"] = (_i64, [_i32, _i32])
SIGNATURES["tf_topp_probs_multi"] = (_i32, [_vp, _vp, _vp, _i32, _i32, _f32, _f32, _vp, _vp, _i64, _vp])
SIGNATURES["tf_topp_multi_tune"] = (_i32, [_i32, _i32])
SIGNATURES["tf_topp_multi_error"] = (_i32, [_vp])
SIGNATURES["tf_topp_multi_reset"] = (_i32, [_vp])
SIGNATURES["tf_draft_persist_ctl_bytes"] = (_i64, [])
SIGNATURES["tf_draft_persist_ws_bytes"] = (_i64, [_c.POINTER(TfDraftModel)])
SIGNATURES["tf_draft_persist_supported"] = (_i32, [_c.POINTER(TfDraftModel), _i32, _i32])
SIGNATURES["tf_draft_forward_68m_persist"] = (_i32, [_c.POINTER(TfDraftModel), _c.POINTER(TfDraftCache), _vp, _i32, _i32, _i32,
                                                     _vp, _vp, _f32, _f32, _vp, _i64, _vp, _vp])
SIGNATURES["tf_draft_persist_tune"] = (_i32, [_i32, _i32])
SIGNATURES["tf_draft_persist_stamps"] = (_i32, [_vp])
SIGNATURES["tf_draft_persist_error"] = (_i32, [_vp])
SIGNATURES["tf_draft_persist_reset"] = (_i32, [_vp, _vp, _i32])

SIGNATURES["tf_attn_decode_gqa_act"] = (_i32, [_vp, _vp, _vp, _vp, _i64, _i64, _i64, _i64, _i32, _i32, _vp, _i32, _i32, _i32,
                                               _f32, _i32, _vp, _i64, _vp, _vp])
SIGNATURES["tf_attn_prefill_gqa"] = (_i32, [_vp, _vp, _vp, _vp, _i64, _i64, _i32, _i32, _i32, _i32, _i32, _f32, _i32, _vp,
                                            _i64, _vp])
SIGNATURES["tf_skinny_qkv_rope_gqa_act"] = (_i32, [_vp, _vp, _i64, _i64, _vp, _f32, _vp, _vp, _vp, _vp, _vp, _vp, _vp, _i64,
                                                   _i64, _i32, _vp, _i32, _i32, _i32, _i32, _i32, _i32, _vp])
SIGNATURES["tf_rope_append_gqa"] = (_i32, [_vp, _i64, _vp, _vp, _vp, _vp, _vp, _vp, _i64, _i64, _i32, _vp, _i32, _i32, _i32,
                                           _i32, _i32, _vp])

ABI_VERSION = 1
_lib = None


class TriforceHipError(RuntimeError):
    pass


def _preload_torch_hip_runtime():
    import torch
    cand = os.path.join(os.path.dirname(torch.__file__), "lib", "libamdhip64.so")
    if os.path.exists(cand):
        ctypes.CDLL(cand, mode=ctypes.RTLD_GLOBAL)


def lib():
    global _lib
    if _lib is None:
        _preload_torch_hip_runtime()
        path = os.environ.get("TRIFORCE_HIP_LIB", LIB_PATH)
        if not os.path.exists(path):
            raise TriforceHipError(
                f"{path} not found: the HIP extension is required (python -m triforce_amd.build); "
                "there is no CPU fallback")
        L = ctypes.CDLL(path)
        for name, (res, args) in SIGNATURES.items():
            try:
                fn = getattr(L, name)
            except AttributeError as e:
                raise TriforceHipError(f"{path} does not export {name}") from e
            fn.restype, fn.argtypes = res, args
        if L.tf_abi_version() != ABI_VERSION:
            raise TriforceHipError(f"ABI mismatch: library {L.tf_abi_version()} != binding {ABI_VERSION}")
        _lib = L
    return _lib


def check(rc, what):
    if rc != 0:
        kind = {-22: "TF_EINVAL", -28: "TF_ENOSPC", -34: "TF_ERANGE"}.get(rc, f"hipError {rc}" if rc > 0 else str(rc))
        raise TriforceHipError(f"{what} failed: {kind}")
```

### triforce_amd/models/llama_core.py

```python
import json
import math
import os
import zlib

import torch

from .. import ops
from .config_yarn import LlamaConfig


def rope_tables_plain(dim, max_pos, base):
    inv_freq = 1.0 / (base ** (torch.arange(0, dim, 2).float() / dim))
    freqs = torch.outer(torch.arange(max_pos, dtype=inv_freq.dtype), inv_freq)
    emb = torch.cat((freqs, freqs), dim=-1)
    return emb.cos().to(torch.float16), emb.sin().to(torch.float16)


def rope_tables_yarn(dim, max_pos, factor, orig_max_pos, base=10000.0, beta_fast=32, beta_slow=1):
    def corr_dim(n_rot):
        return (dim * math.log(orig_max_pos / (n_rot * 2 * math.pi))) / (2 * math.log(base))

    pos_freqs = base ** (torch.arange(0, dim, 2).float() / dim)
    inv_extrapolation = 1.0 / pos_freqs
    inv_interpolation = 1.0 / (factor * pos_freqs)
# ... 2 lines not shown
    if low == high:
        high += 0.001
    ramp = torch.clamp((torch.arange(dim // 2, dtype=torch.float32) - low) / (high - low), 0, 1)
    mask = 1 - ramp
    inv_freq = inv_interpolation * (1 - mask) + inv_extrapolation * mask
    mscale = 1.0 if factor <= 1 else 0.1 * math.log(factor) + 1.0
    freqs = torch.outer(torch.arange(max_pos, dtype=torch.float32), inv_freq)
    emb = torch.cat((freqs, freqs), dim=-1)
    return (emb.cos() * mscale).to(torch.float16), (emb.sin() * mscale).to(torch.float16)


def rope_tables_for(cfg, force_plain=False):
    D = cfg.hidden_size // cfg.num_attention_heads
    rs = cfg.rope_scaling
    if rs is None or force_plain:
        return rope_tables_plain(D, cfg.max_position_embeddings, cfg.rope_theta)
    return rope_tables_yarn(D, cfg.max_position_embeddings, rs["factor"], rs["original_max_position_embeddings"])


def softmax_scale_for(head_dim):
    return float(1 / torch.sqrt(torch.tensor(head_dim, dtype=torch.float16)))


RETRIEVAL_WEIGHTS_ENV = "TRIFORCE_RETRIEVAL_WEIGHTS"


def retrieval_weights():
    v = os.environ.get(RETRIEVAL_WEIGHTS_ENV, "fp16").strip().lower() or "fp16"
    if v not in ("fp16", "fp8"):
        raise ValueError(f"{RETRIEVAL_WEIGHTS_ENV}={v!r}: expected fp16 or fp8")
    if v == "fp8" and ops.FUSE_MODE != "all":
        raise ValueError(f"{RETRIEVAL_WEIGHTS_ENV}=fp8 needs the fused decode layer (TRIFORCE_FUSE=all, got {ops.FUSE_MODE!r}): "
                         "the FP8 kernels exist only in that form")
    return v


class CausalLMOutput:
    __slots__ = ("logits", "probs")

    def __init__(self, logits, probs=None):
        self.logits = logits
        self.probs = probs


class LlamaWeights:

    def __init__(self, cfg: LlamaConfig, device, rank=0, world_size=1):
        self.cfg, self.device, self.rank, self.world_size = cfg, torch.device(device), rank, world_size
        self.L = cfg.num_hidden_layers
        self.H = cfg.num_attention_heads
        self.D = cfg.hidden_size // self.H
        self.Hkv = cfg.num_key_value_heads
        if self.Hkv != self.H and world_size > 1:
            raise ValueError(f"GQA ({self.H} query / {self.Hkv} KV heads) is not supported by tensor-parallel weight shards "
                             f"(world_size={world_size})")
        assert self.H % world_size == 0 and cfg.intermediate_size % world_size == 0
        self.H_local = self.H // world_size
        self.Hkv_local = self.Hkv // world_size if self.Hkv == self.H else self.Hkv
        self.I_local = cfg.intermediate_size // world_size
        self.eps = cfg.rms_norm_eps
        self.embed = self.lm_head = self.norm = None
        self.wqkv, self.wo, self.wgu, self.wd, self.ln1, self.ln2 = [], [], [], [], [], []
        self.aligned = None
        self.capture = None
        self.retrieval_fp8 = False
        self.fp8_tier = True

    def _shard_rows(self, w, n_local):
        return w[self.rank * n_local:(self.rank + 1) * n_local]

    def _shard_cols(self, w, n_local):
        return w[:, self.rank * n_local:(self.rank + 1) * n_local]

    def load_state_dict(self, sd):
        dev, hd, kvd = self.device, self.H_local * self.D, self.Hkv_local * self.D

        def get(name):
            return sd[name].to(torch.float16)

        self.embed = get("model.embed_tokens.weight").to(dev)
        self.lm_head = get("lm_head.weight").to(dev) if "lm_head.weight" in sd else self.embed
        self.norm = get("model.norm.weight").to(dev)
        for i in range(self.L):
            p = f"model.layers.{i}."
            q = self._shard_rows(get(p + "self_attn.q_proj.weight"), hd)
            k = self._shard_rows(get(p + "self_attn.k_proj.weight"), kvd)
            v = self._shard_rows(get(p + "self_attn.v_proj.weight"), kvd)
            self.wqkv.append(torch.cat([q, k, v], dim=0).contiguous().to(dev))
            self.wo.append(self._shard_cols(get(p + "self_attn.o_proj.weight"), hd).contiguous().to(dev))
            g = self._shard_rows(get(p + "mlp.gate_proj.weight"), self.I_local)
            u = self._shard_rows(get(p + "mlp.up_proj.weight"), self.I_local)
            self.wgu.append(torch.cat([g, u], dim=0).contiguous().to(dev))
            self.wd.append(self._shard_cols(get(p + "mlp.down_proj.weight"), self.I_local).contiguous().to(dev))
            self.ln1.append(get(p + "input_layernorm.weight").to(dev))
            self.ln2.append(get(p + "post_attention_layernorm.weight").to(dev))
        return self.finalize()

    def init_random(self, seed, std=0.02):
        dev, cfg = self.device, self.cfg
        hid, hd = cfg.hidden_size, self.H_local * self.D

        def draw(tag, *shape):
            g = torch.Generator(device=dev)
            g.manual_seed((seed * 1000003 + zlib.crc32(repr(tag).encode())) % (2 ** 31))
            return (torch.randn(*shape, generator=g, device=dev, dtype=torch.float32) * std).to(torch.float16)

        self.embed = draw("embed", cfg.vocab_size, hid)
        self.lm_head = draw("lm_head", cfg.vocab_size, hid)
        self.norm = torch.ones(hid, dtype=torch.float16, device=dev)
        for i in range(self.L):
            self.wqkv.append(draw(("qkv", i, self.rank), hd + 2 * self.Hkv_local * self.D, hid))
            self.wo.append(draw(("o", i, self.rank), hid, hd))
            self.wgu.append(draw(("gu", i, self.rank), 2 * self.I_local, hid))
            self.wd.append(draw(("d", i, self.rank), hid, self.I_local))
            self.ln1.append(torch.ones(hid, dtype=torch.float16, device=dev))
            self.ln2.append(torch.ones(hid, dtype=torch.float16, device=dev))
        return self.finalize()

    def overwrite_random_(self, seed, std=0.02):
        dev, cfg = self.device, self.cfg
        assert isinstance(self.lm_head, ops.PackedLinear), "finalize() first"

        def draw_into(dst, tag):
            g = torch.Generator(device=dev)
            g.manual_seed((seed * 1000003 + zlib.crc32(repr(tag).encode())) % (2 ** 31))
            dst.copy_((torch.randn(*dst.shape, generator=g, device=dev, dtype=torch.float32) * std).to(torch.float16))

        tied = self.embed is self.lm_head.w
        draw_into(self.lm_head.w, "lm_head")
        self.lm_head.refresh_()
        if not tied:
            draw_into(self.embed, "embed")
        self.norm.fill_(1.0)
        for i in range(self.L):
            for lst, tag in ((self.wqkv, "qkv"), (self.wo, "o"), (self.wgu, "gu"), (self.wd, "d")):
                draw_into(lst[i].w, (tag, i, self.rank))
                lst[i].refresh_()
            self.ln1[i].fill_(1.0)
            self.ln2[i].fill_(1.0)
        self.aligned = None
        return self

    def init_aligned(self, spec, role, attn_keys=4096):
        from . import aligned
        from .config_yarn import refuse_gqa
        refuse_gqa(self.cfg, "aligned synthetic weights (models/aligned.py init_aligned)")
        return aligned.init_weights(self, spec, role, attn_keys=attn_keys)

    def finalize(self):
        PL = ops.PackedLinear
        if isinstance(self.lm_head, PL):
            return self
        tied = self.lm_head is self.embed
        self.lm_head = PL(self.lm_head)
        if tied:
            self.embed = self.lm_head.w
        rope = (self.H_local, self.D) if self.Hkv == self.H else (self.H_local, self.Hkv_local, self.D)
        self.wqkv = [PL(w, rope=rope) for w in self.wqkv]
        self.wo = [PL(w) for w in self.wo]
        self.wgu = [PL(w, split=2) for w in self.wgu]
        self.wd = [PL(w) for w in self.wd]
        if self.retrieval_fp8:
            self.build_fp8_()
        return self

    def build_fp8_(self):
        if self.Hkv != self.H:
            raise ValueError(f"GQA ({self.H} query / {self.Hkv} KV heads) is not supported by {RETRIEVAL_WEIGHTS_ENV}=fp8: "
                             "no grouped-query FP8 q|k|v epilogue exists")
        for pl in [self.lm_head] + self.wqkv + self.wo + self.wgu + self.wd:
            if pl.fp8 is None:
                pl.fp8 = ops.Fp8Linear(pl)
        return self

    def fp8_active(self):
        return self.retrieval_fp8 and self.fp8_tier and self.lm_head.fp8 is not None

    def nbytes(self):
        ts = [self.embed, self.lm_head, self.norm] + self.wqkv + self.wo + self.wgu + self.wd + self.ln1 + self.ln2
        ts = [ops._w(t) for t in ts]
        return sum(t.numel() * t.element_size() for t in ts)


class DecoderLayers:

    def __init__(self, W, cos, sin, rotate_k=True):
        self.W, self.cos, self.sin, self.rotate_k = W, cos, sin, rotate_k

    def _kv_heads(self):
        W = self.W
        return {} if W.Hkv_local == W.H_local else {"Hkv": W.Hkv_local}

    def _capture(self, x):
        if self.W.capture is not None:
            self.W.capture.append(x.rows() if isinstance(x, ops.Act) else x.clone())

    def qkv_fused(self, i, x, ss, pos, kl, vl, slot, slot_dev=None, f8=False):
        W = self.W
        w = W.wqkv[i]
        return ops.qkv_rope(x, w.fp8 if f8 else w, W.ln1[i], W.eps, self.cos, self.sin, pos, kl, vl, slot, W.H_local, W.D,
                            rotate_k=self.rotate_k, slot0_dev=slot_dev, ss_in=ss if i > 0 else None, **self._kv_heads())

    def o_fused(self, i, a, x, ss, f8=False, out=None):
        w = self.W.wo[i].fp8 if f8 else self.W.wo[i]
        if out is None:
            return ops.linear(a, w, resid=x, out=x, ss_out=ss)
        return ops.linear(a, w, out=out)

    def gate_up_fused(self, i, x, ss, f8=False):
        W = self.W
        w = W.wgu[i]
        return ops.mlp_act(x, w.fp8 if f8 else w, ln=W.ln2[i], eps=W.eps, ss_in=ss)

    def down_fused(self, i, act, x, ss, f8=False, out=None):
        w = self.W.wd[i].fp8 if f8 else self.W.wd[i]
        if out is None:
            return ops.linear(act, w, resid=x, out=x, ss_out=ss)
        return ops.linear(act, w, out=out)

    def head_fused(self, x, ss, f8=False):
        W = self.W
        self._capture(x)
        return ops.linear(x, W.lm_head.fp8 if f8 else W.lm_head, out_f32=True, ln=W.norm, eps=W.eps, ss_in=ss).unsqueeze(0)

    def qkv(self, i, x, d, pos, kl, vl, slot, slot_dev=None):
        W = self.W
        if d is None:
            h = ops.rmsnorm(x, W.ln1[i], W.eps)
        else:
            h = ops.rmsnorm(d, W.ln1[i], W.eps, residual=x, sum_out=x)
        return ops.rope_append(ops.linear(h, W.wqkv[i]), self.cos, self.sin, pos, kl, vl, slot, W.H_local, W.D,
                               rotate_k=self.rotate_k, slot0_dev=slot_dev, **self._kv_heads())

    def o_proj(self, i, a, out=None):
        return ops.linear(a, self.W.wo[i], out=out)

    def mlp(self, i, x, o, out=None):
        W = self.W
        h = ops.rmsnorm(o, W.ln2[i], W.eps, residual=x, sum_out=x)
        return ops.linear(ops.mlp_act(h, W.wgu[i]), W.wd[i], out=out)

    def head(self, x, d, last_rows=None):
        W = self.W
        h = ops.rmsnorm(d, W.norm, W.eps, residual=x, sum_out=x)
        self._capture(x)
        if last_rows is not None and last_rows < h.shape[0]:
            h = h[-last_rows:]
        return ops.linear(h, W.lm_head, out_f32=True).unsqueeze(0)


def load_checkpoint_state_dict(path):
    sd = {}
    st_files = sorted(f for f in os.listdir(path) if f.endswith(".safetensors"))
    if st_files:
        from safetensors.torch import load_file
        for f in st_files:
            sd.update(load_file(os.path.join(path, f)))
        return sd
    bins = sorted(f for f in os.listdir(path) if f.endswith(".bin"))
    if not bins:
        raise FileNotFoundError(f"no *.safetensors / *.bin weights under {path}")
    for f in bins:
        sd.update(torch.load(os.path.join(path, f), map_location="cpu"))
    return sd


def parse_random_spec(name_or_path):
    if isinstance(name_or_path, str) and name_or_path.startswith("random"):
        parts = name_or_path.split(":")
        return int(parts[1]) if len(parts) > 1 and parts[1] else 0
    return None


def save_config(cfg, path):
    os.makedirs(path, exist_ok=True)
    with open(os.path.join(path, "config.json"), "w") as f:
        json.dump({k: v for k, v in cfg.to_dict().items() if not k.startswith("_")}, f, indent=1)
```

### triforce_amd/ops.py

```python
import ctypes
import functools

import torch
import torch.nn.functional as F

from . import hip

_HALF = torch.float16


def _stream():
    return ctypes.c_void_p(torch.cuda.current_stream().cuda_stream)


def _ptr(t):
    return ctypes.c_void_p(t.data_ptr()) if t is not None else None


def _dev(*ts):
    for t in ts:
        if t is not None and not t.is_cuda:
            raise hip.TriforceHipError("triforce_amd ops need HIP device tensors (no CPU fallback)")


def _dev_or_pinned(t):
    if not (t.is_cuda or t.is_pinned()):
        raise hip.TriforceHipError("result record must be a HIP device tensor or pinned host memory")


def _kv(t):
    assert t.dim() == 3 and t.stride(2) == 1 and t.dtype == _HALF, "KV layer view must be (H,T,D) fp16, D contiguous"
    return t.stride(1), t.stride(0)


SKINNY_MAX_ROWS = 32
import os as _os


def fuse_mode():
    v = _os.environ.get("TRIFORCE_FUSE", "all")
    if v not in ("all", "none"):
        raise ValueError(f"TRIFORCE_FUSE={v!r}: expected all or none")
    return v


FUSE_MODE = fuse_mode()


def pack_weight(w):
    N, K = w.shape
    assert N % 16 == 0 and K % 32 == 0 and w.dtype == _HALF
    return w.view(N // 16, 16, K // 32, 4, 8).permute(0, 2, 3, 1, 4).contiguous()


def rope_row_order(H, Hkv, D, device=None):
    assert D % 32 == 0
    d = torch.arange(D // 2, device=device).view(D // 16, 8)
    per_head = torch.cat([d, d + D // 2], dim=1).reshape(-1)
    qk = (torch.arange(H + Hkv, device=device).view(-1, 1) * D + per_head.view(1, -1)).reshape(-1)
    return torch.cat([qk, torch.arange((H + Hkv) * D, (H + 2 * Hkv) * D, device=device)])


def gqa_stack(g, sq):
    assert g >= 1 and 1 <= sq <= SKINNY_MAX_ROWS
    gs = max(d for d in range(1, g + 1) if g % d == 0 and d * sq <= SKINNY_MAX_ROWS)
    return gs, g // gs


def group_mean_query(q, Hkv):
    H, D = q.shape
    if H == Hkv:
        return q
    assert H % Hkv == 0
    return q.view(Hkv, H // Hkv, D).float().mean(dim=1).to(q.dtype)


N8_ENABLED = _os.environ.get("TRIFORCE_GEMM_N8", "1") != "0"
N8_MAX_PANELS = int(_os.environ.get("TRIFORCE_GEMM_N8_MAX_PANELS", "128"))
N8_MAX_ROWS = 24
N8_MIN_K = 1024


def pack_weight_n8(w):
    N, K = w.shape
    assert N % 8 == 0 and K % 64 == 0 and w.dtype == _HALF
    return w.view(N // 8, 8, K // 64, 2, 4, 8).permute(0, 2, 4, 3, 1, 5).contiguous()


def rope_row_order_n8(H, D, device=None):
    assert D % 32 == 0
    d = torch.arange(D // 2, device=device).view(D // 8, 4)
    per_head = torch.cat([d, d + D // 2], dim=1).reshape(-1)
    qk = (torch.arange(2 * H, device=device).view(-1, 1) * D + per_head.view(1, -1)).reshape(-1)
    return torch.cat([qk, torch.arange(2 * H * D, 3 * H * D, device=device)])


def n8_applies(N_stream, K):
    return (N8_ENABLED and N_stream % 16 == 0 and N_stream // 16 <= N8_MAX_PANELS and K % 64 == 0 and K >= N8_MIN_K)


_SG_WS = {}
_SG_WS_BYTES = 8 << 20


def _ensure_sg_workspace(device):
    device = torch.device(device)
    if device.type != "cuda" or device in _SG_WS:
        return
    with torch.cuda.device(device):
        ws = torch.zeros(_SG_WS_BYTES, dtype=torch.uint8, device=device)
        torch.cuda.synchronize(device)
        hip.check(hip.lib().tf_sg_workspace(_ptr(ws), ws.numel()), "tf_sg_workspace")
        if _os.environ.get("TRIFORCE_GEMM_KSPLIT", "0") == "1":
            hip.lib().tf_sg_tune(3, 200)
        if "TRIFORCE_GEMM_P2_GROUPS" in _os.environ:
            hip.lib().tf_sg_tune(2, int(_os.environ["TRIFORCE_GEMM_P2_GROUPS"]))
        if "TRIFORCE_GEMM_FEW_PANELS" in _os.environ:
            hip.lib().tf_sg_tune(5, int(_os.environ["TRIFORCE_GEMM_FEW_PANELS"]))
    _SG_WS[device] = ws


def _rope3(rope):
    return (rope[0], rope[0], rope[1]) if len(rope) == 2 else tuple(rope)


def _rope_rows(rope):
    H, Hkv, D = _rope3(rope)
    return (H + 2 * Hkv) * D


class PackedLinear:

    def __init__(self, w, split=1, pack=None, rope=None):
        self.w = w
        self.N, self.K = w.shape
        self.split = split
        pack = w.is_cuda if pack is None else pack
        ok = pack and (self.N // split) % 16 == 0 and self.K % 32 == 0
        if ok and w.is_cuda:
            _ensure_sg_workspace(w.device)
        self.parts = [pack_weight(b) for b in w.chunk(split, dim=0)] if ok else None
        self.wp = self.parts[0] if (ok and split == 1) else None
        self.rope = rope
        self.wp_rope = None
        self.gqa = rope is not None and len(rope) == 3 and rope[1] != rope[0]
        if rope is not None and len(rope) == 3 and not self.gqa:
            self.rope = rope = (rope[0], rope[2])
        if ok and rope is not None and rope[-1] % 32 == 0 and self.N == _rope_rows(rope):
            self.wp_rope = pack_weight(w[rope_row_order(*_rope3(rope), w.device)])
        self.parts_n8 = self.wp_rope_n8 = None
        if ok and w.is_cuda and split == 2 and n8_applies(self.N // split, self.K):
            self.parts_n8 = [pack_weight_n8(b) for b in w.chunk(split, dim=0)]
        if self.wp_rope is not None and not self.gqa and w.is_cuda and n8_applies(self.N, self.K):
            self.wp_rope_n8 = pack_weight_n8(w[rope_row_order_n8(rope[0], rope[1], w.device)])
        self.fp8 = None

    def refresh_(self):
        if self.parts is not None:
            for dst, blk in zip(self.parts, self.w.chunk(self.split, dim=0)):
                dst.copy_(pack_weight(blk))
        if self.wp_rope is not None:
            self.wp_rope.copy_(pack_weight(self.w[rope_row_order(*_rope3(self.rope), self.w.device)]))
        if self.parts_n8 is not None:
            for dst, blk in zip(self.parts_n8, self.w.chunk(self.split, dim=0)):
                dst.copy_(pack_weight_n8(blk))
        if self.wp_rope_n8 is not None:
            self.wp_rope_n8.copy_(pack_weight_n8(self.w[rope_row_order_n8(self.rope[0], self.rope[1], self.w.device)]))
        if self.fp8 is not None:
            self.fp8.refresh_()
        return self


FP8_MAX = 448.0


def quantize_fp8_rows(w):
    w32 = w.float()
    amax = w32.abs().amax(dim=1)
    s = torch.where(amax > 0, amax / FP8_MAX, torch.ones_like(amax))
    q = (w32 / s[:, None]).clamp_(-FP8_MAX, FP8_MAX).to(torch.float8_e4m3fn)
    return q.view(torch.uint8), s


def dequantize_fp8_rows(codes, scale):
    return codes.view(torch.float8_e4m3fn).float() * scale.float()[:, None]


def pack_weight_fp8(codes):
    N, K = codes.shape
    assert N % 16 == 0 and K % 64 == 0 and codes.dtype == torch.uint8
    return codes.view(N // 16, 16, K // 64, 2, 4, 8).permute(0, 2, 4, 1, 3, 5).reshape(N // 16, K // 64, 4, 16, 16).contiguous()


def unpack_weight_fp8(packed):
    P, S = packed.shape[0], packed.shape[1]
    return packed.view(P, S, 4, 16, 2, 8).permute(0, 3, 1, 4, 2, 5).reshape(P * 16, S * 64).contiguous()


class Fp8Linear:

    def __init__(self, pl):
        assert isinstance(pl, PackedLinear)
        self.src, self.N, self.K, self.split, self.rope = pl, pl.N, pl.K, pl.split, pl.rope
        if getattr(pl, "gqa", False):
            raise ValueError(f"GQA q|k|v weight (H, Hkv, D = {pl.rope}) is not supported by the FP8 weight tier (Fp8Linear): "
                             "no grouped-query FP8 epilogue exists")
        if not pl.w.is_cuda:
            raise hip.TriforceHipError("FP8 weights need a HIP device tensor (no CPU fallback)")
        if self.K % 64 or (self.N // self.split) % 16 or self.N % self.split:
            raise hip.TriforceHipError(f"FP8 weights: unsupported shape {self.N} x {self.K} (rows per stream % 16, K % 64)")
        if self.rope is not None and (self.rope[1] % 32 or self.N != 3 * self.rope[0] * self.rope[1]):
            raise hip.TriforceHipError(f"FP8 weights: q|k|v weight {self.N} x {self.K} does not match H, D = {self.rope}")
        self.codes, self.scales = [], []
        for blk in self._streams():
            c, s = quantize_fp8_rows(blk)
            self.codes.append(pack_weight_fp8(c))
            self.scales.append(s.contiguous())

    def _streams(self):
        w = self.src.w
        if self.rope is not None:
            return [w[rope_row_order(self.rope[0], self.rope[0], self.rope[1], w.device)]]
        return list(w.chunk(self.split, dim=0))

    def refresh_(self):
        for dst_c, dst_s, blk in zip(self.codes, self.scales, self._streams()):
            c, s = quantize_fp8_rows(blk)
            dst_c.copy_(pack_weight_fp8(c))
            dst_s.copy_(s)
        return self

    def dequantized(self):
        rows = [dequantize_fp8_rows(unpack_weight_fp8(c), s) for c, s in zip(self.codes, self.scales)]
        w = torch.cat(rows, dim=0)
        if self.rope is not None:
            out = torch.empty_like(w)
            out[rope_row_order(self.rope[0], self.rope[0], self.rope[1], w.device)] = w
            return out
        return w

    def nbytes(self):
        return sum(c.numel() + 4 * s.numel() for c, s in zip(self.codes, self.scales))


def _fp8_rows_ok(x, w):
    if not (x.is_cuda and x.shape[0] <= SKINNY_MAX_ROWS and x.dtype == _HALF and x.shape[1] == w.K):
        raise hip.TriforceHipError(f"FP8 weights run only on the skinny decode kernels (<= {SKINNY_MAX_ROWS} fp16 device rows "
                                   f"of width {w.K}); got {tuple(x.shape)} {x.dtype}")


def _w(w):
    return w.w if isinstance(w, PackedLinear) else w


ACT_LAYOUT = _os.environ.get("TRIFORCE_ACT_LAYOUT", "auto")
ACT_PACKED_MIN_ROWS = int(_os.environ.get("TRIFORCE_ACT_PACKED_MIN_ROWS", "17"))


def act_packed(rows):
    if ACT_LAYOUT == "packed":
        return True
    if ACT_LAYOUT == "rows":
        return False
    return rows >= ACT_PACKED_MIN_ROWS


class Act:
    __slots__ = ("t", "M", "K")

    def __init__(self, t, M):
        assert t.dim() == 3 and t.shape[2] == 8 and t.is_contiguous() and t.dtype == _HALF and t.shape[1] >= M
        self.t, self.M, self.K = t, M, t.shape[0] * 8

    @classmethod
    def empty(cls, M, K, device, R=None):
        return cls(torch.empty(K // 8, M if R is None else R, 8, dtype=_HALF, device=device), M)

    @classmethod
    def from_rows(cls, x, R=None):
        return cls(pack_act(x, R), x.shape[0])

    @classmethod
    def over(cls, flat, M, K):
        assert flat.numel() == M * K and flat.is_contiguous()
        return cls(flat.view(K // 8, M, 8), M)

    R = property(lambda self: self.t.shape[1])
    sm = property(lambda self: 8)
    sk = property(lambda self: 8 * self.t.shape[1])
    shape = property(lambda self: (self.M, self.K))
    device = property(lambda self: self.t.device)
    dtype = property(lambda self: self.t.dtype)
    is_cuda = property(lambda self: self.t.is_cuda)

    def data_ptr(self):
        return self.t.data_ptr()

    def numel(self):
        return self.M * self.K

    def rows(self):
        return unpack_act(self.t, self.M)

    def clone(self):
        return Act(self.t.clone(), self.M)

    def copy_(self, other):
        if isinstance(other, Act):
            assert other.shape == self.shape and other.R == self.R
            self.t.copy_(other.t)
        else:
            self.t[:, :self.M].copy_(other.view(self.M, self.K // 8, 8).permute(1, 0, 2))
        return self


def _lay(x):
    if x is None:
        return None, 8, 8
    if isinstance(x, Act):
        return _ptr(x.t), x.sm, x.sk
    assert x.dim() == 2 and x.stride(1) == 1 and x.dtype == _HALF
    return _ptr(x), x.stride(0), 8


def pack_act(x, R=None):
    M, K = x.shape
    R = M if R is None else R
    assert K % 8 == 0 and R >= M and x.dtype == _HALF
    out = torch.zeros(K // 8, R, 8, dtype=_HALF, device=x.device)
    out[:, :M] = x.reshape(M, K // 8, 8).permute(1, 0, 2)
    return out


def unpack_act(xp, M):
    K8, R, _ = xp.shape
    return xp[:, :M].permute(1, 0, 2).reshape(M, K8 * 8).contiguous()


def embed_rows(embed, ids, packed, out=None):
    ids = ids.reshape(-1)
    if not packed:
        if embed.is_cuda and embed.dtype == _HALF and embed.is_contiguous() and ids.numel() <= 32 and ids.dtype == torch.int64 \
                and ids.is_contiguous() and embed.shape[1] % 8 == 0 and (out is None or (out.is_contiguous() and out.dtype == _HALF)):
            n, (V, hid) = ids.numel(), embed.shape
            x = torch.empty(n, hid, dtype=_HALF, device=embed.device) if out is None else out
            assert tuple(x.shape) == (n, hid)
            hip.check(hip.lib().tf_embed_rows(_ptr(embed), _ptr(ids), _ptr(x), hid, 8, n, hid, V, _stream()), "tf_embed_rows")
            return x
        if out is None:
            return embed[ids]
        return out.copy_(embed[ids])
    _dev(embed, ids)
    assert embed.dtype == _HALF and embed.is_contiguous() and ids.dtype == torch.int64 and ids.is_contiguous()
    n, (V, hid) = ids.numel(), embed.shape
    x = Act.empty(n, hid, embed.device) if out is None else out
    assert isinstance(x, Act) and x.shape == (n, hid)
    hip.check(hip.lib().tf_embed_rows(_ptr(embed), _ptr(ids), _ptr(x.t), x.sm, x.sk, n, hid, V, _stream()), "tf_embed_rows")
    return x


def set_tokens(dst, vals, pad, pos=None, pos0=0, slot=None, sk=None, sk_val=0):
    n_dst = 0 if dst is None else dst.numel()
    n_vals = len(vals)
    assert n_vals <= 32 and n_dst <= 32 and (dst is None or (dst.dtype == torch.int64 and dst.is_contiguous()))
    assert pos is None or (pos.dtype == torch.int64 and pos.is_contiguous() and pos.numel() <= 64)
    assert (slot is None or slot.dtype == torch.int32) and (sk is None or sk.dtype == torch.int32)
    _dev(dst, pos, slot, sk)
    host = (ctypes.c_int64 * max(n_vals, 1))(*[int(v) for v in vals])
    hip.check(hip.lib().tf_set_tokens(_ptr(dst), n_dst, host, n_vals, int(pad), _ptr(pos), 0 if pos is None else pos.numel(),
                                      int(pos0), _ptr(slot), _ptr(sk), int(sk_val), _stream()), "tf_set_tokens")


def can_fuse(x, *ws):
    return (x.is_cuda and x.dim() == 2 and x.shape[0] <= SKINNY_MAX_ROWS and x.dtype == _HALF and x.stride(1) == 1
            and all(isinstance(w, PackedLinear) and w.parts is not None for w in ws))


def can_fuse_rows(rows, embed, *ws):
    return (embed.is_cuda and embed.dtype == _HALF and rows <= SKINNY_MAX_ROWS
            and all(isinstance(w, PackedLinear) and w.parts is not None for w in ws))


def linear(x, w, out_f32=False, ln=None, eps=0.0, resid=None, out=None, ss_in=None, ss_out=None):
    M = x.shape[0]
    f8 = isinstance(w, Fp8Linear)
    if f8:
        _fp8_rows_ok(x, w)
        assert w.split == 1 and w.rope is None, "an FP8 gate|up / q|k|v weight runs through mlp_act / qkv_rope"
    if f8 or (isinstance(w, PackedLinear) and w.wp is not None and M <= SKINNY_MAX_ROWS and x.is_cuda):
        assert x.dtype == _HALF and x.shape[1] == w.K
        if out is None:
            if out_f32 or not isinstance(x, Act):
                out = torch.empty(M, w.N, dtype=torch.float32 if out_f32 else _HALF, device=x.device)
            else:
                out = Act.empty(M, w.N, x.device)
        assert tuple(out.shape) == (M, w.N)
        if resid is not None:
            assert tuple(resid.shape) == tuple(out.shape) and resid.dtype == _HALF and not out_f32
        if ss_in is not None:
            assert ss_in.dtype == torch.float32 and ss_in.shape == (w.K // 16, 32) and ss_in.is_contiguous()
        if ss_out is not None:
            assert ss_out.dtype == torch.float32 and ss_out.shape == (w.N // 16, 32) and ss_out.is_contiguous()
        xp, xsm, xsk = _lay(x)
        rp, rsm, rsk = _lay(resid)
        if out_f32:
            assert out.dtype == torch.float32 and out.stride(1) == 1
            yp, ysm, ysk = _ptr(out), out.stride(0), 8
        else:
            yp, ysm, ysk = _lay(out)
        if f8:
            hip.check(hip.lib().tf_skinny_gemm_fp8_act(_ptr(w.codes[0]), _ptr(w.scales[0]), xp, xsm, xsk, _ptr(ln), float(eps),
                                                       _ptr(ss_in), rp, rsm, rsk, _ptr(ss_out), yp, ysm, ysk, M, w.N, w.K,
                                                       1 if out_f32 else 0, _stream()), "tf_skinny_gemm_fp8_act")
            return out
        hip.check(hip.lib().tf_skinny_gemm_act(_ptr(w.wp), xp, xsm, xsk, _ptr(ln), float(eps), _ptr(ss_in), rp, rsm, rsk,
                                               _ptr(ss_out), yp, ysm, ysk, M, w.N, w.K, 1 if out_f32 else 0, _stream()),
                  "tf_skinny_gemm_act")
        return out
    assert ln is None and resid is None and out is None and ss_in is None and ss_out is None, \
        "fused linear needs the skinny kernel (ops.can_fuse)"
    assert not isinstance(x, Act), "k-octet-major activations exist only on the skinny decode path"
    y = F.linear(x, _w(w))
    return y.float() if out_f32 else y


def mlp_act(h, wgu, ln=None, eps=0.0, ss_in=None):
    M = h.shape[0]
    if isinstance(wgu, Fp8Linear):
        _fp8_rows_ok(h, wgu)
        assert wgu.split == 2, "mlp_act takes a fused gate|up weight"
        I = wgu.N // 2
        act = Act.empty(M, I, h.device) if isinstance(h, Act) else torch.empty(M, I, dtype=_HALF, device=h.device)
        hp, hsm, hsk = _lay(h)
        ap, asm, ask = _lay(act)
        hip.check(hip.lib().tf_skinny_gemm_swiglu_fp8_act(_ptr(wgu.codes[0]), _ptr(wgu.scales[0]), _ptr(wgu.codes[1]),
                                                          _ptr(wgu.scales[1]), hp, hsm, hsk, _ptr(ln), float(eps), _ptr(ss_in),
                                                          ap, asm, ask, M, I, wgu.K, _stream()), "tf_skinny_gemm_swiglu_fp8_act")
        return act
    if isinstance(wgu, PackedLinear) and wgu.parts is not None and wgu.split == 2 and M <= SKINNY_MAX_ROWS \
            and h.is_cuda:
        I = wgu.N // 2
        act = Act.empty(M, I, h.device) if isinstance(h, Act) else torch.empty(M, I, dtype=_HALF, device=h.device)
        hp, hsm, hsk = _lay(h)
        ap, asm, ask = _lay(act)
        if wgu.parts_n8 is not None and ln is not None and M <= N8_MAX_ROWS:
            hip.check(hip.lib().tf_skinny_gemm_swiglu_n8(_ptr(wgu.parts_n8[0]), _ptr(wgu.parts_n8[1]), hp, hsm, hsk, _ptr(ln),
                                                         float(eps), _ptr(ss_in), ap, asm, ask, M, I, wgu.K, _stream()),
                      "tf_skinny_gemm_swiglu_n8")
            return act
        hip.check(hip.lib().tf_skinny_gemm_swiglu_act(_ptr(wgu.parts[0]), _ptr(wgu.parts[1]), hp, hsm, hsk, _ptr(ln),
                                                      float(eps), _ptr(ss_in), ap, asm, ask, M, I, wgu.K, _stream()),
                  "tf_skinny_gemm_swiglu_act")
        return act
    assert ln is None and not isinstance(h, Act), "fused mlp_act needs the skinny kernel (ops.can_fuse)"
    return silu_mul(F.linear(h, _w(wgu)))


def ss_buffer(hidden, device):
    return torch.empty(hidden // 16, 32, dtype=torch.float32, device=device)


def qkv_rope(x, wqkv, ln, eps, cos, sin, positions, k_layer, v_layer, slot0, H, D, rotate_k=True, slot0_dev=None,
             ss_in=None, Hkv=None):
    _dev(ln, cos, sin, positions, k_layer, v_layer, slot0_dev)
    gqa = Hkv is not None and Hkv != H
    f8 = isinstance(wqkv, Fp8Linear)
    if f8:
        _fp8_rows_ok(x, wqkv)
    assert f8 or (isinstance(wqkv, PackedLinear) and wqkv.wp_rope is not None)
    assert wqkv.rope == ((H, Hkv, D) if gqa else (H, D))
    rows = x.shape[0]
    assert x.is_cuda and x.dtype == _HALF and x.shape[1] == wqkv.K and rows <= SKINNY_MAX_ROWS
    assert positions.dtype == torch.int64 and positions.numel() == rows and positions.is_contiguous()
    assert cos.dtype == _HALF and cos.is_contiguous() and cos.shape[1] == D
    st, sh = _kv(k_layer)
    assert _kv(v_layer) == (st, sh)
    q = torch.empty(rows, H, D, dtype=_HALF, device=x.device)
    xp, xsm, xsk = _lay(x)
    if gqa:
        assert not f8 and k_layer.shape[0] == Hkv and v_layer.shape[0] == Hkv and H % Hkv == 0
        hip.check(hip.lib().tf_skinny_qkv_rope_gqa_act(_ptr(wqkv.wp_rope), xp, xsm, xsk, _ptr(ln), float(eps), _ptr(ss_in),
                                                       _ptr(cos), _ptr(sin), _ptr(positions), _ptr(q), _ptr(k_layer),
                                                       _ptr(v_layer), st, sh, int(slot0), _ptr(slot0_dev), rows, H, Hkv, D,
                                                       wqkv.K, 1 if rotate_k else 0, _stream()), "tf_skinny_qkv_rope_gqa_act")
        return q
    if f8:
        hip.check(hip.lib().tf_skinny_qkv_rope_fp8_act(_ptr(wqkv.codes[0]), _ptr(wqkv.scales[0]), xp, xsm, xsk, _ptr(ln),
                                                       float(eps), _ptr(ss_in), _ptr(cos), _ptr(sin), _ptr(positions), _ptr(q),
                                                       _ptr(k_layer), _ptr(v_layer), st, sh, int(slot0), _ptr(slot0_dev), rows,
                                                       H, D, wqkv.K, 1 if rotate_k else 0, _stream()),
                  "tf_skinny_qkv_rope_fp8_act")
        return q
    if wqkv.wp_rope_n8 is not None and ln is not None and rows <= N8_MAX_ROWS:
        hip.check(hip.lib().tf_skinny_qkv_rope_n8(_ptr(wqkv.wp_rope_n8), xp, xsm, xsk, _ptr(ln), float(eps), _ptr(ss_in),
                                                  _ptr(cos), _ptr(sin), _ptr(positions), _ptr(q), _ptr(k_layer),
                                                  _ptr(v_layer), st, sh, int(slot0), _ptr(slot0_dev), rows, H, D, wqkv.K,
                                                  1 if rotate_k else 0, _stream()), "tf_skinny_qkv_rope_n8")
        return q
    hip.check(hip.lib().tf_skinny_qkv_rope_act(_ptr(wqkv.wp_rope), xp, xsm, xsk, _ptr(ln), float(eps), _ptr(ss_in),
                                               _ptr(cos), _ptr(sin), _ptr(positions), _ptr(q), _ptr(k_layer),
                                               _ptr(v_layer), st, sh, int(slot0), _ptr(slot0_dev), rows, H, D, wqkv.K,
                                               1 if rotate_k else 0, _stream()), "tf_skinny_qkv_rope_act")
    return q


def rmsnorm(x, w, eps, residual=None, sum_out=None):
    _dev(x, w, residual, sum_out)
    assert x.dtype == _HALF and x.is_contiguous() and x.dim() == 2
    y = torch.empty_like(x)
    hip.check(hip.lib().tf_rmsnorm(_ptr(x), _ptr(residual), _ptr(w), _ptr(y), _ptr(sum_out), x.shape[0], x.shape[1],
                                   float(eps), _stream()), "tf_rmsnorm")
    return y


def rope_append(qkv, cos, sin, positions, k_layer, v_layer, slot0, H, D, rotate_k=True, slot0_dev=None, Hkv=None):
    _dev(qkv, cos, sin, positions, k_layer, v_layer)
    rows = qkv.shape[0]
    if Hkv is not None and Hkv != H:
        assert qkv.dtype == _HALF and qkv.stride(1) == 1 and qkv.shape[1] == (H + 2 * Hkv) * D and H % Hkv == 0
        assert positions.dtype == torch.int64 and positions.numel() == rows and positions.is_contiguous()
        assert cos.dtype == _HALF and cos.is_contiguous() and cos.shape[1] == D
        st, sh = _kv(k_layer)
        assert _kv(v_layer) == (st, sh) and k_layer.shape[0] == Hkv and v_layer.shape[0] == Hkv
        q = torch.empty(rows, H, D, dtype=_HALF, device=qkv.device)
        hip.check(hip.lib().tf_rope_append_gqa(_ptr(qkv), qkv.stride(0), _ptr(cos), _ptr(sin), _ptr(positions), _ptr(q),
                                               _ptr(k_layer), _ptr(v_layer), st, sh, int(slot0), _ptr(slot0_dev), rows, H, Hkv,
                                               D, 1 if rotate_k else 0, _stream()), "tf_rope_append_gqa")
        return q
    assert qkv.dtype == _HALF and qkv.stride(1) == 1 and qkv.shape[1] == 3 * H * D
    assert positions.dtype == torch.int64 and positions.numel() == rows and positions.is_contiguous()
    assert cos.dtype == _HALF and cos.is_contiguous() and cos.shape[1] == D
    st, sh = _kv(k_layer)
    assert _kv(v_layer) == (st, sh)
    q = torch.empty(rows, H, D, dtype=_HALF, device=qkv.device)
    hip.check(hip.lib().tf_rope_append(_ptr(qkv), qkv.stride(0), _ptr(cos), _ptr(sin), _ptr(positions), _ptr(q),
                                       _ptr(k_layer), _ptr(v_layer), st, sh, int(slot0), _ptr(slot0_dev), rows, H, D,
                                       1 if rotate_k else 0, _stream()), "tf_rope_append")
    return q


def silu_mul(gate_up):
    _dev(gate_up)
    rows, two_i = gate_up.shape
    assert gate_up.dtype == _HALF and gate_up.is_contiguous()
    out = torch.empty(rows, two_i // 2, dtype=_HALF, device=gate_up.device)
    hip.check(hip.lib().tf_silu_mul(_ptr(gate_up), _ptr(out), rows, two_i // 2, _stream()), "tf_silu_mul")
    return out


def _workspace(device, floats):
    return torch.empty(int(floats), dtype=torch.float32, device=device)


ATTN_TIMER = None
ATTN_TIMER_EVERY = max(1, int(_os.environ.get("TRIFORCE_ATTN_TIMER_EVERY", "8")))
_attn_calls = 0


_NSPLIT_FORCE = int(_os.environ.get("TRIFORCE_ATTN_NSPLIT", "0"))


@functools.lru_cache(maxsize=4096)
def _pick_nsplit(H, sk):
    if _NSPLIT_FORCE > 0:
        return max(1, min(_NSPLIT_FORCE, (int(sk) + 15) // 16))
    return hip.lib().tf_attn_decode_pick_nsplit(H, sk)


@functools.lru_cache(maxsize=4096)
def _ws_floats(H, sq, D, nsplit):
    return hip.lib().tf_attn_decode_ws_floats(H, sq, D, nsplit)


ATTN_FUSED_MERGE = _os.environ.get("TRIFORCE_ATTN_FUSED_MERGE", "1") != "0"
if _os.environ.get("TRIFORCE_ATTN_RENDEZVOUS", "0") == "1":
    hip.lib().tf_attn_tune(0, 1)
_TICKET_ROWS, _TICKET_WORDS = 64, 128
_tickets = {}


def _ticket_row(device, stream):
    dev = _tickets.get(device)
    if dev is None:
        dev = _tickets[device] = (torch.zeros(_TICKET_ROWS, _TICKET_WORDS, dtype=torch.int32, device=device), {})
    block, rows = dev
    row = rows.get(stream)
    if row is None:
        if len(rows) >= _TICKET_ROWS:
            return None
        row = rows[stream] = len(rows)
    return block[row]


def attn_decode(q, k_layer, v_layer, sk, scale, sk_dev=None, nsplit=None, packed=False):
    _dev(q, k_layer, v_layer, sk_dev)
    sq, H, D = q.shape
    if k_layer.shape[0] != H:
        return attn_decode_gqa(q, k_layer, v_layer, sk, scale, sk_dev=sk_dev, nsplit=nsplit, packed=packed)
    assert q.dtype == _HALF and q.is_contiguous()
    st, sh = _kv(k_layer)
    assert _kv(v_layer) == (st, sh)
    L = hip.lib()
    if nsplit is None:
        nsplit = _pick_nsplit(H, int(sk))
    ws = _workspace(q.device, _ws_floats(H, sq, D, nsplit))
    out = Act.empty(sq, H * D, q.device) if packed else torch.empty(sq, H * D, dtype=_HALF, device=q.device)
    op, osm, osk = _lay(out)
    timed = False
    if ATTN_TIMER is not None and not torch.cuda.is_current_stream_capturing():
        global _attn_calls
        _attn_calls += 1
        timed = _attn_calls % ATTN_TIMER_EVERY == 0
    if timed:
        ev0, ev1 = torch.cuda.Event(enable_timing=True), torch.cuda.Event(enable_timing=True)
        ev0.record()
    stream = _stream()
    tickets = _ticket_row(q.device, stream.value or 0) if ATTN_FUSED_MERGE and H <= _TICKET_WORDS else None
    hip.check(L.tf_attn_decode_act(_ptr(q), _ptr(k_layer), _ptr(v_layer), op, osm, osk, st, sh, sq, int(sk), _ptr(sk_dev),
                                   H, D, float(scale), nsplit, _ptr(ws), ws.numel(), _ptr(tickets), stream),
              "tf_attn_decode_act")
    if timed:
        ev1.record()
        ATTN_TIMER.append((ev0, ev1, int(sk), H, D))
    return out


def attn_decode_gqa(q, k_layer, v_layer, sk, scale, sk_dev=None, nsplit=None, packed=False, fused_merge=None, out=None):
    _dev(q, k_layer, v_layer, sk_dev)
    sq, H, D = q.shape
    Hkv = k_layer.shape[0]
    assert q.dtype == _HALF and q.is_contiguous() and v_layer.shape[0] == Hkv
    if Hkv < 1 or H % Hkv or sq > SKINNY_MAX_ROWS:
        raise hip.TriforceHipError(f"attn_decode_gqa: {H} query heads over {Hkv} KV heads, {sq} rows")
    st, sh = _kv(k_layer)
    assert _kv(v_layer) == (st, sh)
    gs, sub = gqa_stack(H // Hkv, sq)
    cols = Hkv * sub
    if nsplit is None:
        nsplit = _pick_nsplit(cols, int(sk))
    ws = _workspace(q.device, _ws_floats(cols, gs * sq, D, nsplit))
    if out is None:
        out = Act.empty(sq, H * D, q.device) if packed else torch.empty(sq, H * D, dtype=_HALF, device=q.device)
    assert tuple(out.shape) == (sq, H * D)
    op, osm, osk = _lay(out)
    stream = _stream()
    fused = ATTN_FUSED_MERGE if fused_merge is None else fused_merge
    tickets = _ticket_row(q.device, stream.value or 0) if fused and cols <= _TICKET_WORDS else None
    hip.check(hip.lib().tf_attn_decode_gqa_act(_ptr(q), _ptr(k_layer), _ptr(v_layer), op, osm, osk, st, sh, sq, int(sk),
                                               _ptr(sk_dev), H, Hkv, D, float(scale), nsplit, _ptr(ws), ws.numel(),
                                               _ptr(tickets), stream), "tf_attn_decode_gqa_act")
    return out
# ... 161 lines not shown
class KvQuantPairPlan:

    def __init__(self, src_k, src_v, dst_kc, dst_vc, dst_ke, dst_ve, src_exp=None):
        _dev(src_k, src_v, dst_kc, dst_vc, dst_ke, dst_ve)
        L, H, _, D = src_k.shape
        assert src_k.shape == src_v.shape and dst_kc.shape == dst_vc.shape and dst_ke.shape == dst_ve.shape
        assert dst_kc.shape[0] == L and dst_kc.shape[1] == H and dst_kc.shape[3] == D and dst_ke.shape[:2] == (L, H)
        if src_exp is None:
            src = _lhtd(src_k)
            assert _lhtd(src_v) == src
            exp = (None, None, 0, 0)
            self.src_rows = src_k.shape[2]
        else:
            src = _lhtd_f8(src_k)
            assert _lhtd_f8(src_v) == src
            sek, sev = src_exp
            _dev(sek, sev)
            assert _lht_exp(sek) == _lht_exp(sev) and sek.shape[:2] == (L, H) and sev.shape == sek.shape
            exp = (_ptr(sek), _ptr(sev)) + _lht_exp(sek)
            self.src_rows = min(src_k.shape[2], sek.shape[2])
        dst = _lhtd_f8(dst_kc)
        assert _lhtd_f8(dst_vc) == dst and _lht_exp(dst_ke) == _lht_exp(dst_ve)
        self.keep = (src_k, src_v, dst_kc, dst_vc, dst_ke, dst_ve, src_exp)
        self.dst_rows = min(dst_kc.shape[2], dst_ke.shape[2])
        self.head = (_ptr(src_k), _ptr(src_v)) + src + exp + (_ptr(dst_kc), _ptr(dst_vc)) + dst \
            + (_ptr(dst_ke), _ptr(dst_ve)) + _lht_exp(dst_ke)
        self.dims = (L, H, D)
        self.fn = hip.lib().tf_kv_quant_rows_pair

    def __call__(self, src_t0, dst_t0, n):
        if n <= 0:
            return
        if src_t0 < 0 or dst_t0 < 0 or src_t0 + n > self.src_rows or dst_t0 + n > self.dst_rows:
            raise IndexError(f"kv_quant_rows_pair: rows [{src_t0}, {src_t0 + n}) of {self.src_rows} -> [{dst_t0}, {dst_t0 + n}) of "
                             f"{self.dst_rows} leave the cache (the kernel does not bounds-check)")
        hip.check(self.fn(*self.head, int(src_t0), int(dst_t0), int(n), *self.dims, _stream()), "tf_kv_quant_rows_pair")


def kv_quant_rows_pair(src_k, src_v, dst_kc, dst_vc, dst_ke, dst_ve, src_t0, dst_t0, n, src_exp=None):
    if n <= 0:
        return
    KvQuantPairPlan(src_k, src_v, dst_kc, dst_vc, dst_ke, dst_ve, src_exp)(src_t0, dst_t0, n)


def attn_block(q, k_layer, v_layer, sk, scale, nsplit=None, tree_mask=None, mask_row0=0, tree_start=0):
    _dev(q, k_layer, v_layer, tree_mask)
    sq, H, D = q.shape
    assert q.dtype == _HALF and q.is_contiguous() and sq <= 128
    st, sh = _kv(k_layer)
    assert _kv(v_layer) == (st, sh)
    L = hip.lib()
    if nsplit is None:
        nsplit = L.tf_attn_block_pick_nsplit(H, sq, int(sk))
    ws = _workspace(q.device, L.tf_attn_block_ws_floats(H, D, nsplit))
    out = torch.empty(sq, H * D, dtype=_HALF, device=q.device)
    words = 0
    if tree_mask is not None:
        assert tree_mask.dtype == torch.int32 and tree_mask.dim() == 2 and tree_mask.is_contiguous()
        assert mask_row0 + sq <= tree_mask.shape[0]
        words = tree_mask.shape[1]
    hip.check(L.tf_attn_block(_ptr(q), _ptr(k_layer), _ptr(v_layer), _ptr(out), st, sh, sq, int(sk), H, D, float(scale),
                              nsplit, _ptr(ws), ws.numel(), _ptr(tree_mask), words, int(mask_row0), int(tree_start),
                              _stream()), "tf_attn_block")
    return out


def attn_tree(q, k_layer, v_layer, sk, scale, tree_mask, tree_start, mask_row0=0):
    sq = q.shape[0]
    if sq <= 128:
        return attn_block(q, k_layer, v_layer, sk, scale, tree_mask=tree_mask, mask_row0=mask_row0, tree_start=tree_start)
    outs = []
    for r0 in range(0, sq, 128):
        r1 = min(sq, r0 + 128)
        outs.append(attn_block(q[r0:r1].contiguous(), k_layer, v_layer, sk, scale, tree_mask=tree_mask,
                               mask_row0=mask_row0 + r0, tree_start=tree_start))
    return torch.cat(outs, dim=0)


def pack_tree_mask(visible):
    rows, T = visible.shape
    words = (T + 31) // 32
    v = torch.zeros(rows, words * 32, dtype=torch.int64, device=visible.device)
    v[:, :T] = (visible != 0).to(torch.int64)
    w = (v.view(rows, words, 32) << torch.arange(32, device=visible.device, dtype=torch.int64)).sum(dim=-1)
    w = torch.where(w >= 2 ** 31, w - 2 ** 32, w)
    return w.to(torch.int32).contiguous()


ATTN_PREFILL_ONE_LAUNCH = _os.environ.get("TRIFORCE_PREFILL_ONE_LAUNCH", "1") != "0"


def attn_prefill(q, k_layer, v_layer, sk, scale):
    sq = q.shape[0]
    if sq <= 32:
        return attn_decode(q, k_layer, v_layer, sk, scale)
    if k_layer.shape[0] != q.shape[1]:
        return attn_prefill_gqa(q, k_layer, v_layer, sk, scale)
    if sq <= 128:
        return attn_block(q, k_layer, v_layer, sk, scale)
    if not ATTN_PREFILL_ONE_LAUNCH or sq > 4096:
        outs = []
        for r0 in range(0, sq, 128):
            r1 = min(sq, r0 + 128)
            outs.append(attn_block(q[r0:r1].contiguous(), k_layer, v_layer, sk - (sq - r1), scale))
        return torch.cat(outs, dim=0)
    _dev(q, k_layer, v_layer)
    _, H, D = q.shape
    assert q.dtype == _HALF and q.is_contiguous()
    st, sh = _kv(k_layer)
    assert _kv(v_layer) == (st, sh)
    L = hip.lib()
    nsplit = L.tf_attn_prefill_pick_nsplit(H, sq, int(sk))
    ws = _workspace(q.device, L.tf_attn_prefill_ws_floats(H, sq, D, nsplit))
    out = torch.empty(sq, H * D, dtype=_HALF, device=q.device)
    hip.check(L.tf_attn_prefill(_ptr(q), _ptr(k_layer), _ptr(v_layer), _ptr(out), st, sh, sq, int(sk), H, D, float(scale),
                                nsplit, _ptr(ws), ws.numel(), _stream()), "tf_attn_prefill")
    return out


def attn_prefill_gqa(q, k_layer, v_layer, sk, scale):
    _dev(q, k_layer, v_layer)
    sq, H, D = q.shape
    Hkv = k_layer.shape[0]
    if not ATTN_PREFILL_ONE_LAUNCH:
        raise ValueError("TRIFORCE_PREFILL_ONE_LAUNCH=0 is not supported with a GQA model: the per-block kernel "
                         "(tf_attn_block) has one head count")
    if Hkv < 1 or H % Hkv:
        raise hip.TriforceHipError(f"attn_prefill_gqa: {H} query heads over {Hkv} KV heads")
    if sq > 4096:
        outs = []
        for r0 in range(0, sq, 4096):
            r1 = min(sq, r0 + 4096)
            outs.append(attn_prefill_gqa(q[r0:r1].contiguous(), k_layer, v_layer, sk - (sq - r1), scale))
        return torch.cat(outs, dim=0)
    assert q.dtype == _HALF and q.is_contiguous() and v_layer.shape[0] == Hkv
    st, sh = _kv(k_layer)
    assert _kv(v_layer) == (st, sh)
    L = hip.lib()
    nsplit = L.tf_attn_prefill_pick_nsplit(H, sq, int(sk))
    ws = _workspace(q.device, L.tf_attn_prefill_ws_floats(H, sq, D, nsplit))
    out = torch.empty(sq, H * D, dtype=_HALF, device=q.device)
    hip.check(L.tf_attn_prefill_gqa(_ptr(q), _ptr(k_layer), _ptr(v_layer), _ptr(out), st, sh, sq, int(sk), H, Hkv, D,
                                    float(scale), nsplit, _ptr(ws), ws.numel(), _stream()), "tf_attn_prefill_gqa")
    return out


def draft_model_struct(embed, ln1, wqkv, wo, ln2, wgu, wd, norm, lm_head, cos, sin, H, D, eps, scale):
    L = len(wqkv)
    ws = list(wqkv) + list(wo) + list(wgu) + list(wd) + [lm_head]
    if L > hip.TF_DRAFT_MAX_LAYERS or D != 64 or not all(isinstance(w, PackedLinear) and w.parts is not None for w in ws):
        return None
    if any(w.wp_rope is None for w in wqkv) or any(w.split != 2 for w in wgu) or not embed.is_cuda:
        return None
    m = hip.TfDraftModel()
    m.embed = embed.data_ptr()
    for i in range(L):
        m.ln1[i], m.ln2[i] = ln1[i].data_ptr(), ln2[i].data_ptr()
        m.wqkv[i], m.wo[i], m.wdown[i] = wqkv[i].wp_rope.data_ptr(), wo[i].wp.data_ptr(), wd[i].wp.data_ptr()
        m.wgate[i], m.wup[i] = wgu[i].parts[0].data_ptr(), wgu[i].parts[1].data_ptr()
    m.norm, m.lm_head, m.cos, m.sin = norm.data_ptr(), lm_head.wp.data_ptr(), cos.data_ptr(), sin.data_ptr()
    m.layers, m.hidden, m.heads, m.head_dim = L, embed.shape[1], H, D
    m.inter, m.vocab, m.eps, m.scale = wgu[0].N // 2, lm_head.N, float(eps), float(scale)
    return m


def draft_cache_struct(cache, L):
    c = hip.TfDraftCache()
    st = sh = None
    for i in range(L):
        kl, vl = cache.layer_kv(i)
        _dev(kl, vl)
        assert _kv(vl) == _kv(kl) and (st is None or (st, sh) == _kv(kl))
        st, sh = _kv(kl)
        c.k[i], c.v[i] = kl.data_ptr(), vl.data_ptr()
    c.stride_t, c.stride_h = st, sh
    return c


class DraftPersist:

    def __init__(self, model, device):
        L = hip.lib()
        self.device = torch.device(device)
        self.ctl = torch.zeros(int(L.tf_draft_persist_ctl_bytes()), dtype=torch.uint8, device=self.device)
        self.ws = torch.empty(int(L.tf_draft_persist_ws_bytes(ctypes.byref(model))), dtype=torch.uint8, device=self.device)
        self.mirror = None
        assert self.ctl.data_ptr() % 64 == 0 and self.ws.data_ptr() % 256 == 0
        self.enable_mirror()

    def check(self):
        if self.mirror is not None and int(self.mirror[0]) != 0:
            raise hip.TriforceHipError(f"one-launch draft forward: wait on edge {int(self.mirror[0]) - 1} timed out "
                                       "(a workgroup never became resident, or an arrival was lost); outputs are NaN until "
                                       "DraftPersist.reset()")

    def enable_mirror(self):
        if self.mirror is None:
            self.mirror = torch.zeros(1, dtype=torch.int32).pin_memory()
            hip.check(hip.lib().tf_draft_persist_reset(_ptr(self.ctl), self.mirror.data_ptr(), 1), "tf_draft_persist_reset")
        return self.mirror

    def error(self):
        if self.mirror is not None:
            return int(self.mirror[0])
        return int(hip.lib().tf_draft_persist_error(_ptr(self.ctl)))

    def reset(self):
        hip.check(hip.lib().tf_draft_persist_reset(_ptr(self.ctl), None, 0), "tf_draft_persist_reset")


DRAFT_PERSIST = _os.environ.get("TRIFORCE_DRAFT_PERSIST", "1") != "0"


def draft_persist_supported(model, n, kv_len):
    return hip.lib().tf_draft_persist_supported(ctypes.byref(model), int(n), int(kv_len)) == 0


def draft_forward(model, cache, ids, slot0, kv_len, probs=None, persist=None):
    _dev(ids)
    n = ids.numel()
    assert ids.dtype == torch.int64 and ids.is_contiguous() and 1 <= n <= SKINNY_MAX_ROWS
    L = hip.lib()
    logits = torch.empty(n, model.vocab, dtype=torch.float32, device=ids.device)
    p = torch.empty(model.vocab, dtype=torch.float32, device=ids.device) if probs is not None else None
    T, top_p = probs if probs is not None else (1.0, 1.0)
    if persist is not None and DRAFT_PERSIST and draft_persist_supported(model, n, kv_len):
        hip.check(L.tf_draft_forward_68m_persist(ctypes.byref(model), ctypes.byref(cache), _ptr(ids), n, int(slot0),
                                                 int(kv_len), _ptr(logits), _ptr(p), float(T), float(top_p),
                                                 _ptr(persist.ws), persist.ws.numel(), _ptr(persist.ctl), _stream()),
                  "tf_draft_forward_68m_persist")
        return logits, p
    nbytes = L.tf_draft_forward_ws_bytes(ctypes.byref(model), n)
    ws = torch.empty(nbytes, dtype=torch.uint8, device=ids.device)
    hip.check(L.tf_draft_forward_68m(ctypes.byref(model), ctypes.byref(cache), _ptr(ids), n, int(slot0), int(kv_len),
                                     _ptr(logits), _ptr(p), float(T), float(top_p), _ptr(ws), nbytes, _stream()),
              "tf_draft_forward_68m")
    return logits, p


def attn_rope_on_read(q, k_layer, v_layer, cos, sin, kv_len, scale):
    _dev(q, k_layer, v_layer, cos, sin)
    sq, H, D = q.shape
    assert q.dtype == _HALF and q.is_contiguous()
    st, sh = _kv(k_layer)
    assert _kv(v_layer) == (st, sh)
    out = torch.empty(sq, H * D, dtype=_HALF, device=q.device)
    hip.check(hip.lib().tf_attn_rope_on_read(_ptr(q), _ptr(k_layer), _ptr(v_layer), _ptr(cos), _ptr(sin), _ptr(out),
                                             st, sh, sq, int(kv_len), H, D, float(scale), _stream()),
              "tf_attn_rope_on_read")
    return out


def retrieval_score(k_layer, q, chunks, chunk):
    _dev(k_layer, q)
    H, T, D = k_layer.shape
    st, sh = _kv(k_layer)
    assert q.shape == (H, D) and q.dtype == _HALF and q.is_contiguous() and chunks * chunk <= T
    scores = torch.empty(H, chunks, dtype=_HALF, device=q.device)
    hip.check(hip.lib().tf_retrieval_score(_ptr(k_layer), st, sh, _ptr(q), _ptr(scores), chunks, chunk, H, D,
                                           _stream()), "tf_retrieval_score")
    return scores


def _index_layer(index_layer, H, D):
    assert index_layer.dim() == 3 and index_layer.shape[0] == H and index_layer.shape[2] == D and index_layer.dtype == _HALF \
        and index_layer.stride(2) == 1 and index_layer.stride(1) == D, "(H, Cmax, D) fp16 index layer expected"
    return index_layer.stride(0)


def chunk_mean(k_layer, index_layer, c0, c1, chunk):
    _dev(k_layer, index_layer)
    H, T, D = k_layer.shape
    st, sh = _kv(k_layer)
    ish = _index_layer(index_layer, H, D)
    if not 0 <= c0 <= c1 or c1 > index_layer.shape[1] or c1 * chunk > T:
        raise IndexError(f"chunk_mean: chunks [{c0}, {c1}) of {chunk} rows leave the {index_layer.shape[1]}-chunk index or "
                         f"the {T}-row cache (the kernel does not bounds-check)")
    hip.check(hip.lib().tf_chunk_mean(_ptr(k_layer), st, sh, _ptr(index_layer), ish, int(c0), int(c1), int(chunk), H, D,
                                      _stream()), "tf_chunk_mean")


def retrieval_score_indexed(index_layer, q, chunks):
    _dev(index_layer, q)
    H, Cmax, D = index_layer.shape
    ish = _index_layer(index_layer, H, D)
    assert q.shape == (H, D) and q.dtype == _HALF and q.is_contiguous()
    if not 1 <= chunks <= Cmax:
        raise IndexError(f"retrieval_score_indexed: {chunks} chunks of a {Cmax}-chunk index")
    scores = torch.empty(H, chunks, dtype=_HALF, device=q.device)
    hip.check(hip.lib().tf_retrieval_score_indexed(_ptr(index_layer), ish, _ptr(q), _ptr(scores), int(chunks), H, D,
                                                   _stream()), "tf_retrieval_score_indexed")
    return scores


def retrieval_topk(scores, sets):
    _dev(scores)
    H, C = scores.shape
    assert scores.dtype == _HALF and scores.is_contiguous()
    idx = torch.empty(H, sets, dtype=torch.int32, device=scores.device)
    hip.check(hip.lib().tf_retrieval_topk(_ptr(scores), _ptr(idx), C, sets, H, _stream()), "tf_retrieval_topk")
    return idx


def retrieval_gather(k_src, v_src, idx, k_dst, v_dst, chunk):
    _dev(k_src, v_src, idx, k_dst, v_dst)
    H, _, D = k_src.shape
# ... 336 lines not shown
```

Before: 241.5.

## Pack large skinny-GEMM weights in window-major order for contiguous per-iteration streaming

Adds a window-major weight packing that permutes 512-element tiles so each workgroup's waves read one contiguous window per unrolled iteration, instead of striding across panels. The kernel gets a WIN template path with matching address arithmetic for the main loop, the prefetch and the remainder. Python selects it by default for the down and lm_head projections above 64 MiB. The aim is better DRAM and TLB locality for weight streaming in decode GEMV. In exchange it adds a permutation step at load time, disables K-split for these weights, and makes the draft persistent kernel fall back when window weights are present.

```diff
diff --git a/include/triforce_hip.h b/include/triforce_hip.h
--- a/include/triforce_hip.h
+++ b/include/triforce_hip.h
@@ -149,6 +149,25 @@
                            void* q_out, void* k_cache, void* v_cache, int64_t stride_t, int64_t stride_h, int slot0,
                            const int32_t* slot0_dev, int M, int H, int D, int K, int rotate_k, void* stream);
 int tf_sg_tune(int key, int value);
+int tf_sg_window_form(int mode, int N, int K, int* waves, int* P, int* U);
+int tf_sg_window_perm(int NP, int NC, int waves, int P, int U, int64_t* perm);
+int tf_skinny_gemm_act_win(const void* w_window, const void* x, int64_t xs_m, int64_t xs_k, const void* ln_w, float eps,
+                           const float* ss_in, const void* resid, int64_t rs_m, int64_t rs_k, float* ss_out, void* y,
+                           int64_t ys_m, int64_t ys_k, int M, int N, int K, int out_f32, int win_waves, int win_p,
+                           void* stream);
+int tf_skinny_gemm_swiglu_act_win(const void* gate_window, const void* up_window, const void* x, int64_t xs_m,
+                                  int64_t xs_k, const void* ln_w, float eps, const float* ss_in, void* act, int64_t ys_m,
+                                  int64_t ys_k, int M, int I, int K, int win_waves, int win_p, void* stream);
+int tf_skinny_qkv_rope_act_win(const void* wqkv_window, const void* x, int64_t xs_m, int64_t xs_k, const void* ln_w,
+                               float eps, const float* ss_in, const void* cos, const void* sin, const int64_t* positions,
+                               void* q_out, void* k_cache, void* v_cache, int64_t stride_t, int64_t stride_h, int slot0,
+                               const int32_t* slot0_dev, int M, int H, int D, int K, int rotate_k, int win_waves, int win_p,
+                               void* stream);
+int tf_skinny_qkv_rope_gqa_act_win(const void* wqkv_window, const void* x, int64_t xs_m, int64_t xs_k, const void* ln_w,
+                                   float eps, const float* ss_in, const void* cos, const void* sin,
+                                   const int64_t* positions, void* q_out, void* k_cache, void* v_cache, int64_t stride_t,
+                                   int64_t stride_h, int slot0, const int32_t* slot0_dev, int M, int H, int Hkv, int D,
+                                   int K, int rotate_k, int win_waves, int win_p, void* stream);
 int tf_skinny_gemm_swiglu_n8(const void* gate_n8, const void* up_n8, const void* x, int64_t xs_m, int64_t xs_k,
                              const void* ln_w, float eps, const float* ss_in, void* act, int64_t ys_m, int64_t ys_k,
                              int M, int I, int K, void* stream);
diff --git a/triforce_amd/build.py b/triforce_amd/build.py
--- a/triforce_amd/build.py
+++ b/triforce_amd/build.py
@@ -27,7 +27,7 @@
         return True
     t = os.path.getmtime(LIB_PATH)
     deps = sources() + [os.path.join(CSRC, "common.h"), os.path.join(CSRC, "tree_mask.h"), os.path.join(CSRC, "select_common.h"),
-                        os.path.join(CSRC, "sg_rule.h"),
+                        os.path.join(CSRC, "sg_rule.h"), os.path.join(CSRC, "sg_window.h"),
                         os.path.join(HERE, "..", "include", "triforce_hip.h"), os.path.abspath(__file__)]
     return any(os.path.getmtime(d) > t for d in deps if os.path.exists(d))
 
diff --git a/triforce_amd/csrc/gemv.hip b/triforce_amd/csrc/gemv.hip
--- a/triforce_amd/csrc/gemv.hip
+++ b/triforce_amd/csrc/gemv.hip
@@ -1,5 +1,6 @@
 #include "common.h"
 #include "sg_rule.h"
+#include "sg_window.h"
 
 #define SG_LOAD(p) __builtin_nontemporal_load(p)
 
@@ -110,7 +111,7 @@
     return o;
 }
 
-template <int MT, int MODE, bool NORM, int WAVES, int P, bool KSPLIT, bool XCHG = false>
+template <int MT, int MODE, bool NORM, int WAVES, int P, bool WIN, bool KSPLIT, bool XCHG = false>
 __global__ __launch_bounds__(WAVES * 64) void skinny_gemm_kernel(const half8* __restrict__ wp,
                                                                  const half8* __restrict__ wp_up,
                                                                  const h16* __restrict__ x,
@@ -126,6 +127,8 @@
     constexpr int NA = GATEUP ? 2 : 1;
     constexpr int U = (P * NA >= 2) ? (8 / (P * NA)) : SG_U;
     static_assert(P <= WAVES && U >= 1, "one epilogue wave per panel");
+    static_assert(!WIN || (!KSPLIT && !XCHG), "window-major weights: one workgroup per panel group, no exchange");
+    static_assert(U == sg_batch(P, NA), "sg_window.h packs for this batch");
     const int panel0 = blockIdx.x * P;
     const int tid = threadIdx.x, lane = tid & 63, wave = tid >> 6;
     const int li = lane & 15, g = lane >> 4;
@@ -149,6 +152,17 @@
     const int64_t pstride = (int64_t)nchunks * 64;
     const half8* wa = wp + (int64_t)panel0 * pstride + lane;
     const half8* wu = GATEUP ? (wp_up + (int64_t)panel0 * pstride + lane) : nullptr;
+    const SgWindow win = {N >> 4, nchunks, WAVES, P, U};
+    const int nfull = WIN ? sg_window_full(win) : 0, nrem = WIN ? sg_window_rem(win) : 0;
+    constexpr int64_t JF = (int64_t)WAVES * U * 64;
+    const int64_t it_stride = WIN ? sg_window_it_stride(win) * 64 : 0, jr = (int64_t)WAVES * nrem * 64;
+    const int b0 = nfull > 0 ? U : nrem;
+    const int64_t s0 = WIN ? sg_window_first(win, blockIdx.x, 0, 0) * 64 : 0;
+    const int64_t sr0 = WIN ? sg_window_batch(win, nfull, blockIdx.x, 0, 0) * 64 : 0;
+    const unsigned v0 = wave * (b0 * 64) + lane, vr = wave * (nrem * 64) + lane;
+    auto win_pre = [&](const half8* w, int j, int u) -> const half8* {
+        return (w + (s0 + (int64_t)j * (WAVES * b0 * 64) + (int64_t)min(u, b0 - 1) * 64)) + v0;
+    };
     const int64_t xcs = 4 * xa.sk;
     const h16* xr[MT];
     bool xok[MT];
@@ -196,8 +210,13 @@
             const int cu = min(c0 + u, nchunks - 1);
 #pragma unroll
             for (int j = 0; j < P; ++j) {
-                a_pre[u][j][0] = SG_LOAD(wa + j * pstride + (int64_t)cu * 64);
-                if (GATEUP) a_pre[u][j][NA - 1] = SG_LOAD(wu + j * pstride + (int64_t)cu * 64);
+                if constexpr (WIN) {
+                    a_pre[u][j][0] = SG_LOAD(win_pre(wp, j, u));
+                    if (GATEUP) a_pre[u][j][NA - 1] = SG_LOAD(win_pre(wp_up, j, u));
+                } else {
+                    a_pre[u][j][0] = SG_LOAD(wa + j * pstride + (int64_t)cu * 64);
+                    if (GATEUP) a_pre[u][j][NA - 1] = SG_LOAD(wu + j * pstride + (int64_t)cu * 64);
+                }
             }
         }
         asm volatile("" ::: "memory");
@@ -349,7 +368,8 @@
     if (!EPI_LATE || !(c0 + U <= c1)) prefetch_epi();
 
     int c = c0;
-    for (; c + U <= c1; c += U) {
+    int64_t wo = s0;
+    for (; c + U <= c1; c += U, wo += it_stride) {
         half8 a[U][P][NA], b[U][MT];
 #pragma unroll
         for (int u = 0; u < U; ++u) {
@@ -358,6 +378,9 @@
                 if (NORM && c == c0 && pre) {
                     a[u][j][0] = a_pre[u][j][0];
                     if (GATEUP) a[u][j][NA - 1] = a_pre[u][j][NA - 1];
+                } else if constexpr (WIN) {
+                    a[u][j][0] = SG_LOAD((wp + (wo + j * JF + u * 64)) + v0);
+                    if (GATEUP) a[u][j][NA - 1] = SG_LOAD((wp_up + (wo + j * JF + u * 64)) + v0);
                 } else {
                     a[u][j][0] = SG_LOAD(wa + j * pstride + (int64_t)(c + u) * 64);
                     if (GATEUP) a[u][j][NA - 1] = SG_LOAD(wu + j * pstride + (int64_t)(c + u) * 64);
@@ -393,13 +416,19 @@
 #endif
     }
     SG_STAMP(4);
+    const int cr0 = c;
     if constexpr (NORM) {
         for (; c < c1; ++c) {
             half8 a[P][NA];
 #pragma unroll
             for (int j = 0; j < P; ++j) {
-                a[j][0] = SG_LOAD(wa + j * pstride + (int64_t)c * 64);
-                if (GATEUP) a[j][NA - 1] = SG_LOAD(wu + j * pstride + (int64_t)c * 64);
+                if constexpr (WIN) {
+                    a[j][0] = SG_LOAD((wp + (sr0 + j * jr + (int64_t)(c - cr0) * 64)) + vr);
+                    if (GATEUP) a[j][NA - 1] = SG_LOAD((wp_up + (sr0 + j * jr + (int64_t)(c - cr0) * 64)) + vr);
+                } else {
+                    a[j][0] = SG_LOAD(wa + j * pstride + (int64_t)c * 64);
+                    if (GATEUP) a[j][NA - 1] = SG_LOAD(wu + j * pstride + (int64_t)c * 64);
+                }
             }
 #pragma unroll
             for (int t = 0; t < MT; ++t) {
@@ -419,8 +448,13 @@
             const int cc = min(c + u, c1 - 1);
 #pragma unroll
             for (int j = 0; j < P; ++j) {
-                a[u][j][0] = SG_LOAD(wa + j * pstride + (int64_t)cc * 64);
-                if (GATEUP) a[u][j][NA - 1] = SG_LOAD(wu + j * pstride + (int64_t)cc * 64);
+                if constexpr (WIN) {
+                    a[u][j][0] = SG_LOAD((wp + (sr0 + j * jr + (int64_t)(cc - cr0) * 64)) + vr);
+                    if (GATEUP) a[u][j][NA - 1] = SG_LOAD((wp_up + (sr0 + j * jr + (int64_t)(cc - cr0) * 64)) + vr);
+                } else {
+                    a[u][j][0] = SG_LOAD(wa + j * pstride + (int64_t)cc * 64);
+                    if (GATEUP) a[u][j][NA - 1] = SG_LOAD(wu + j * pstride + (int64_t)cc * 64);
+                }
             }
 #pragma unroll
             for (int t = 0; t < MT; ++t) {
@@ -986,6 +1020,7 @@
     int M, N, K;
     const float* ss_in;
     float* ss_out;
+    int win_waves, win_p;
 };
 
 static unsigned long long* sg_stamps_ptr() {
@@ -1013,12 +1048,12 @@
     return ks;
 }
 
-template <int MT, int MODE, bool NORM, int WAVES, int P>
+template <int MT, int MODE, bool NORM, int WAVES, int P, bool WIN>
 static int launch_sg_form(const SgArgs& a, const SgRope& rp, const SgKsplit& kx, int ks, hipStream_t st) {
     constexpr bool REACHABLE = MODE != SG_GATEUP || WAVES == SG_WAVES || MT == 2;
     constexpr bool CAN_SPLIT = P == 1 && MODE != SG_F32;
 #define SG_LAUNCH(KSPLIT_)                                                                                                 \
-    hipLaunchKernelGGL((skinny_gemm_kernel<MT, MODE, NORM, WAVES, P, KSPLIT_>), dim3(a.N / 16 / P, ks), dim3(WAVES * 64), 0, \
+    hipLaunchKernelGGL((skinny_gemm_kernel<MT, MODE, NORM, WAVES, P, WIN, KSPLIT_>), dim3(a.N / 16 / P, ks), dim3(WAVES * 64), 0, \
                        st, (const half8*)a.wp, (const half8*)a.wp_up, (const h16*)a.x, a.ss_in, (const h16*)a.ln_w, a.K,  \
                        a.M, (int)a.xa.sm, (int)a.xa.sk, a.eps, a.N, (const h16*)a.resid, a.ra, a.y, a.ya, rp, a.ss_out,  \
                        kx, SgXchg{})
@@ -1027,7 +1062,7 @@
     } else {
         if (ks == 1) {
             SG_LAUNCH(false);
-        } else if constexpr (CAN_SPLIT) {
+        } else if constexpr (CAN_SPLIT && !WIN) {
             SG_LAUNCH(true);
         } else {
             return TF_EINVAL;
@@ -1043,8 +1078,14 @@
     const SgForm f = sg_pick_form(MODE, NORM, a.M, a.N, a.K, g_sg_knobs);
     SgKsplit kx = {nullptr, nullptr, (f.P == 1 && MODE != SG_F32) ? sg_stamps_ptr() : nullptr};
     const int ks = sg_ksplit(a, f, MODE, kx, st);
-#define SG_FORM(MT_, W_, P_) \
-    if (f.MT == MT_ && f.WAVES == W_ && f.P == P_) return launch_sg_form<MT_, MODE, NORM, W_, P_>(a, rp, kx, ks, st)
+    const bool win = a.win_waves != 0;
+    if (win && (f.WAVES != a.win_waves || f.P != a.win_p || ks != 1 ||
+                !sg_window_ok(SgWindow{a.N / 16, a.K >> 5, f.WAVES, f.P, sg_batch(f.P, MODE == SG_GATEUP ? 2 : 1)})))
+        return TF_EINVAL;
+#define SG_FORM(MT_, W_, P_)                                                                                     \
+    if (f.MT == MT_ && f.WAVES == W_ && f.P == P_)                                                               \
+        return win ? launch_sg_form<MT_, MODE, NORM, W_, P_, true>(a, rp, kx, ks, st)                           \
+                   : launch_sg_form<MT_, MODE, NORM, W_, P_, false>(a, rp, kx, ks, st)
     SG_FORM(1, SG_WAVES, 1);
     SG_FORM(2, SG_WAVES, 1);
     SG_FORM(1, SG_WAVES_WIDE, 1);
@@ -1086,11 +1127,17 @@
     return TF_OK;
 }
 
-extern "C" int tf_skinny_gemm_act(const void* w_packed, const void* x, int64_t xs_m, int64_t xs_k, const void* ln_w,
-                                  float eps, const float* ss_in, const void* resid, int64_t rs_m, int64_t rs_k,
-                                  float* ss_out, void* y, int64_t ys_m, int64_t ys_k, int M, int N, int K, int out_f32,
-                                  void* stream) {
+static bool sg_win_args_ok(int win_waves, int win_p) {
+    return (win_waves == 0 && win_p == 0) || ((win_waves == SG_WAVES || win_waves == SG_WAVES_WIDE) && (win_p == 1 || win_p == 2));
+}
+
+extern "C" int tf_skinny_gemm_act_win(const void* w_packed, const void* x, int64_t xs_m, int64_t xs_k, const void* ln_w,
+                                      float eps, const float* ss_in, const void* resid, int64_t rs_m, int64_t rs_k,
+                                      float* ss_out, void* y, int64_t ys_m, int64_t ys_k, int M, int N, int K, int out_f32,
+                                      int win_waves, int win_p, void* stream) {
     SgArgs a = {};
+    if (!sg_win_args_ok(win_waves, win_p)) return TF_EINVAL;
+    a.win_waves = win_waves, a.win_p = win_p;
     a.wp = w_packed, a.x = x, a.ln_w = ln_w, a.resid = resid, a.y = y;
     a.xa = SgAct{xs_m, xs_k}, a.ra = SgAct{rs_m, rs_k}, a.ya = SgAct{ys_m, ys_k};
     a.eps = eps, a.M = M, a.N = N, a.K = K, a.ss_in = ss_in, a.ss_out = ss_out;
@@ -1103,6 +1150,14 @@
     return ln_w ? launch_sg<SG_PLAIN, true>(a, rp, st) : launch_sg<SG_PLAIN, false>(a, rp, st);
 }
 
+extern "C" int tf_skinny_gemm_act(const void* w_packed, const void* x, int64_t xs_m, int64_t xs_k, const void* ln_w,
+                                  float eps, const float* ss_in, const void* resid, int64_t rs_m, int64_t rs_k,
+                                  float* ss_out, void* y, int64_t ys_m, int64_t ys_k, int M, int N, int K, int out_f32,
+                                  void* stream) {
+    return tf_skinny_gemm_act_win(w_packed, x, xs_m, xs_k, ln_w, eps, ss_in, resid, rs_m, rs_k, ss_out, y, ys_m, ys_k, M, N, K,
+                                  out_f32, 0, 0, stream);
+}
+
 extern "C" int tf_skinny_gemm_ex(const void* w_packed, const void* x, int64_t ldx, const void* ln_w, float eps,
                                  const float* ss_in, const void* resid, int64_t ldr, float* ss_out, void* y,
                                  int64_t ldy, int M, int N, int K, int out_f32, void* stream) {
@@ -1115,10 +1170,13 @@
     return tf_skinny_gemm_ex(w_packed, x, ldx, nullptr, 0.f, nullptr, nullptr, 0, nullptr, y, ldy, M, N, K, out_f32, stream);
 }
 
-extern "C" int tf_skinny_gemm_swiglu_act(const void* gate_packed, const void* up_packed, const void* x, int64_t xs_m,
-                                         int64_t xs_k, const void* ln_w, float eps, const float* ss_in, void* act,
-                                         int64_t ys_m, int64_t ys_k, int M, int I, int K, void* stream) {
+extern "C" int tf_skinny_gemm_swiglu_act_win(const void* gate_packed, const void* up_packed, const void* x, int64_t xs_m,
+                                             int64_t xs_k, const void* ln_w, float eps, const float* ss_in, void* act,
+                                             int64_t ys_m, int64_t ys_k, int M, int I, int K, int win_waves, int win_p,
+                                             void* stream) {
     SgArgs a = {};
+    if (!sg_win_args_ok(win_waves, win_p)) return TF_EINVAL;
+    a.win_waves = win_waves, a.win_p = win_p;
     a.wp = gate_packed, a.wp_up = up_packed, a.x = x, a.ln_w = ln_w, a.y = act;
     a.xa = SgAct{xs_m, xs_k}, a.ya = SgAct{ys_m, ys_k}, a.ra = SgAct{8, 8};
     a.eps = eps, a.M = M, a.N = I, a.K = K, a.ss_in = ss_in;
@@ -1129,6 +1187,13 @@
     return ln_w ? launch_sg<SG_GATEUP, true>(a, rp, st) : launch_sg<SG_GATEUP, false>(a, rp, st);
 }
 
+extern "C" int tf_skinny_gemm_swiglu_act(const void* gate_packed, const void* up_packed, const void* x, int64_t xs_m,
+                                         int64_t xs_k, const void* ln_w, float eps, const float* ss_in, void* act,
+                                         int64_t ys_m, int64_t ys_k, int M, int I, int K, void* stream) {
+    return tf_skinny_gemm_swiglu_act_win(gate_packed, up_packed, x, xs_m, xs_k, ln_w, eps, ss_in, act, ys_m, ys_k, M, I, K, 0, 0,
+                                         stream);
+}
+
 extern "C" int tf_skinny_gemm_swiglu_ex(const void* gate_packed, const void* up_packed, const void* x, int64_t ldx,
                                         const void* ln_w, float eps, const float* ss_in, void* act, int64_t ldy, int M,
                                         int I, int K, void* stream) {
@@ -1140,13 +1205,16 @@
     return tf_skinny_gemm_swiglu_ex(gate_packed, up_packed, x, ldx, nullptr, 0.f, nullptr, act, ldy, M, I, K, stream);
 }
 
-extern "C" int tf_skinny_qkv_rope_act(const void* wqkv_packed, const void* x, int64_t xs_m, int64_t xs_k,
-                                      const void* ln_w, float eps, const float* ss_in, const void* cosb,
-                                      const void* sinb, const int64_t* positions, void* q_out, void* k_cache,
-                                      void* v_cache, int64_t stride_t, int64_t stride_h, int slot0,
-                                      const int32_t* slot0_dev, int M, int H, int D, int K, int rotate_k, void* stream) {
+extern "C" int tf_skinny_qkv_rope_act_win(const void* wqkv_packed, const void* x, int64_t xs_m, int64_t xs_k,
+                                          const void* ln_w, float eps, const float* ss_in, const void* cosb,
+                                          const void* sinb, const int64_t* positions, void* q_out, void* k_cache,
+                                          void* v_cache, int64_t stride_t, int64_t stride_h, int slot0,
+                                          const int32_t* slot0_dev, int M, int H, int D, int K, int rotate_k,
+                                          int win_waves, int win_p, void* stream) {
     if (!wqkv_packed || !x || !cosb || !sinb || !positions || !q_out || !k_cache || !v_cache) return TF_EINVAL;
     SgArgs a = {};
+    if (!sg_win_args_ok(win_waves, win_p)) return TF_EINVAL;
+    a.win_waves = win_waves, a.win_p = win_p;
     a.wp = wqkv_packed, a.x = x, a.ln_w = ln_w;
     a.xa = SgAct{xs_m, xs_k}, a.ra = SgAct{8, 8}, a.ya = SgAct{8, 8};
     a.eps = eps, a.M = M, a.N = 3 * H * D, a.K = K, a.ss_in = ss_in;
@@ -1170,15 +1238,26 @@
     return ln_w ? launch_sg<SG_QKV, true>(a, rp, st) : launch_sg<SG_QKV, false>(a, rp, st);
 }
 
-extern "C" int tf_skinny_qkv_rope_gqa_act(const void* wqkv_packed, const void* x, int64_t xs_m, int64_t xs_k,
-                                          const void* ln_w, float eps, const float* ss_in, const void* cosb,
-                                          const void* sinb, const int64_t* positions, void* q_out, void* k_cache,
-                                          void* v_cache, int64_t stride_t, int64_t stride_h, int slot0,
-                                          const int32_t* slot0_dev, int M, int H, int Hkv, int D, int K, int rotate_k,
-                                          void* stream) {
+extern "C" int tf_skinny_qkv_rope_act(const void* wqkv_packed, const void* x, int64_t xs_m, int64_t xs_k,
+                                      const void* ln_w, float eps, const float* ss_in, const void* cosb,
+                                      const void* sinb, const int64_t* positions, void* q_out, void* k_cache,
+                                      void* v_cache, int64_t stride_t, int64_t stride_h, int slot0,
+                                      const int32_t* slot0_dev, int M, int H, int D, int K, int rotate_k, void* stream) {
+    return tf_skinny_qkv_rope_act_win(wqkv_packed, x, xs_m, xs_k, ln_w, eps, ss_in, cosb, sinb, positions, q_out, k_cache,
+                                      v_cache, stride_t, stride_h, slot0, slot0_dev, M, H, D, K, rotate_k, 0, 0, stream);
+}
+
+extern "C" int tf_skinny_qkv_rope_gqa_act_win(const void* wqkv_packed, const void* x, int64_t xs_m, int64_t xs_k,
+                                              const void* ln_w, float eps, const float* ss_in, const void* cosb,
+                                              const void* sinb, const int64_t* positions, void* q_out, void* k_cache,
+                                              void* v_cache, int64_t stride_t, int64_t stride_h, int slot0,
+                                              const int32_t* slot0_dev, int M, int H, int Hkv, int D, int K, int rotate_k,
+                                              int win_waves, int win_p, void* stream) {
     if (!wqkv_packed || !x || !cosb || !sinb || !positions || !q_out || !k_cache || !v_cache) return TF_EINVAL;
     if (H < 1 || Hkv < 1 || (H % Hkv) || H > 0x7fff || (D != 64 && D != 128)) return TF_EINVAL;
     SgArgs a = {};
+    if (!sg_win_args_ok(win_waves, win_p)) return TF_EINVAL;
+    a.win_waves = win_waves, a.win_p = win_p;
     a.wp = wqkv_packed, a.x = x, a.ln_w = ln_w;
     a.xa = SgAct{xs_m, xs_k}, a.ra = SgAct{8, 8}, a.ya = SgAct{8, 8};
     a.eps = eps, a.M = M, a.N = (H + 2 * Hkv) * D, a.K = K, a.ss_in = ss_in;
@@ -1200,6 +1279,35 @@
     rp.D = D;
     rp.rotate_k = rotate_k;
     return ln_w ? launch_sg<SG_QKVG, true>(a, rp, st) : launch_sg<SG_QKVG, false>(a, rp, st);
+}
+
+extern "C" int tf_skinny_qkv_rope_gqa_act(const void* wqkv_packed, const void* x, int64_t xs_m, int64_t xs_k,
+                                          const void* ln_w, float eps, const float* ss_in, const void* cosb,
+                                          const void* sinb, const int64_t* positions, void* q_out, void* k_cache,
+                                          void* v_cache, int64_t stride_t, int64_t stride_h, int slot0,
+                                          const int32_t* slot0_dev, int M, int H, int Hkv, int D, int K, int rotate_k,
+                                          void* stream) {
+    return tf_skinny_qkv_rope_gqa_act_win(wqkv_packed, x, xs_m, xs_k, ln_w, eps, ss_in, cosb, sinb, positions, q_out, k_cache,
+                                          v_cache, stride_t, stride_h, slot0, slot0_dev, M, H, Hkv, D, K, rotate_k, 0, 0, stream);
+}
+
+extern "C" int tf_sg_window_form(int mode, int N, int K, int* waves, int* P, int* U) {
+    if (!waves || !P || !U || mode < SG_PLAIN || mode > SG_QKVG || N < 16 || (N % 16) || K < 32 || (K % 32)) return TF_EINVAL;
+    const SgForm f1 = sg_pick_form(mode, false, 1, N, K, g_sg_knobs);
+    for (int M = 1; M <= 32; ++M) {
+        const SgForm f = sg_pick_form(mode, false, M, N, K, g_sg_knobs);
+        if (f.WAVES != f1.WAVES || f.P != f1.P) return 0;
+    }
+    const int u = sg_batch(f1.P, mode == SG_GATEUP ? 2 : 1);
+    if (sg_pick_ks(N / 16, f1.P, K >> 5, f1.WAVES, mode, g_sg_knobs) != 1) return 0;
+    if (!sg_window_ok(SgWindow{N / 16, K >> 5, f1.WAVES, f1.P, u})) return 0;
+    *waves = f1.WAVES, *P = f1.P, *U = u;
+    return 1;
+}
+
+extern "C" int tf_sg_window_perm(int NP, int NC, int waves, int P, int U, int64_t* perm) {
+    if (!perm || !sg_window_perm(SgWindow{NP, NC, waves, P, U}, perm)) return TF_EINVAL;
+    return TF_OK;
 }
 
 extern "C" int tf_skinny_qkv_rope(const void* wqkv_packed, const void* x, int64_t ldx, const void* ln_w, float eps,
@@ -1314,7 +1422,7 @@
     const SgKsplit kx = {nullptr, nullptr, sg_stamps_ptr()};
     const bool wide = sg_xchg_waves(K) == SG_WAVES_WIDE;
 #define XCHG_LAUNCH(MT_, W_)                                                                                                  \
-    hipLaunchKernelGGL((skinny_gemm_kernel<MT_, SG_PLAIN, false, W_, 1, false, true>), dim3(N / 16), dim3(W_ * 64), 0, st, \
+    hipLaunchKernelGGL((skinny_gemm_kernel<MT_, SG_PLAIN, false, W_, 1, false, false, true>), dim3(N / 16), dim3(W_ * 64), 0, st, \
                        (const half8*)a.wp, (const half8*)nullptr, (const h16*)a.x, (const float*)nullptr,              \
                        (const h16*)nullptr, a.K, a.M, (int)a.xa.sm, (int)a.xa.sk, 0.f, a.N, (const h16*)a.resid, a.ra, a.y, a.ya, rp, a.ss_out, \
                        kx, xc)
diff --git a/triforce_amd/csrc/sg_window.h b/triforce_amd/csrc/sg_window.h
--- /dev/null
+++ b/triforce_amd/csrc/sg_window.h
@@ -0,0 +1,64 @@
+#pragma once
+#include <cstdint>
+
+#if defined(__HIPCC__)
+#define SGW_HD __host__ __device__ inline
+#else
+#define SGW_HD inline
+#endif
+
+struct SgWindow {
+    int NP, NC;
+    int WAVES, P, U;
+};
+
+SGW_HD constexpr int sg_batch(int P, int NA) { return P * NA >= 2 ? 8 / (P * NA) : 4; }
+
+SGW_HD bool sg_window_ok(const SgWindow& w) {
+    return w.NP >= 1 && w.NC >= 1 && w.WAVES >= 1 && w.P >= 1 && w.U >= 1 && w.NP % w.P == 0 && w.NC % w.WAVES == 0;
+}
+
+SGW_HD int64_t sg_window_tiles(const SgWindow& w) { return (int64_t)w.NP * w.NC; }
+SGW_HD int sg_window_full(const SgWindow& w) { return w.NC / w.WAVES / w.U; }
+SGW_HD int sg_window_rem(const SgWindow& w) { return (w.NC / w.WAVES) % w.U; }
+SGW_HD int64_t sg_window_it_stride(const SgWindow& w) { return (int64_t)w.NP * w.WAVES * w.U; }
+SGW_HD int sg_window_j_stride(const SgWindow& w, int it) { return w.WAVES * (it < sg_window_full(w) ? w.U : sg_window_rem(w)); }
+
+SGW_HD int64_t sg_window_batch(const SgWindow& w, int it, int wg, int j, int wave) {
+    const int64_t slot = ((int64_t)wg * w.P + j) * w.WAVES + wave;
+    const int nfull = sg_window_full(w);
+    if (it < nfull) return (int64_t)it * sg_window_it_stride(w) + slot * w.U;
+    return (int64_t)nfull * sg_window_it_stride(w) + slot * sg_window_rem(w);
+}
+
+SGW_HD int64_t sg_window_first(const SgWindow& w, int wg, int j, int wave) {
+    return (((int64_t)wg * w.P + j) * w.WAVES + wave) * (sg_window_full(w) > 0 ? w.U : sg_window_rem(w));
+}
+
+SGW_HD void sg_window_tile(const SgWindow& w, int64_t t, int& panel, int& chunk) {
+    const int cpw = w.NC / w.WAVES, nfull = sg_window_full(w), rem = sg_window_rem(w);
+    const int64_t per_it = sg_window_it_stride(w), full = (int64_t)nfull * per_it;
+    int64_t slot;
+    int c_rel;
+    if (t < full) {
+        const int64_t r = t % per_it;
+        slot = r / w.U;
+        c_rel = (int)(t / per_it) * w.U + (int)(r % w.U);
+    } else {
+        slot = (t - full) / rem;
+        c_rel = nfull * w.U + (int)((t - full) % rem);
+    }
+    panel = (int)(slot / w.WAVES);
+    chunk = (int)(slot % w.WAVES) * cpw + c_rel;
+}
+
+inline bool sg_window_perm(const SgWindow& w, int64_t* perm) {
+    if (!sg_window_ok(w)) return false;
+    const int64_t n = sg_window_tiles(w);
+    for (int64_t t = 0; t < n; ++t) {
+        int panel, chunk;
+        sg_window_tile(w, t, panel, chunk);
+        perm[t] = (int64_t)panel * w.NC + chunk;
+    }
+    return true;
+}
diff --git a/triforce_amd/hip.py b/triforce_amd/hip.py
--- a/triforce_amd/hip.py
+++ b/triforce_amd/hip.py
@@ -159,6 +159,13 @@
 SIGNATURES["tf_rope_append_gqa"] = (_i32, [_vp, _i64, _vp, _vp, _vp, _vp, _vp, _vp, _i64, _i64, _i32, _vp, _i32, _i32, _i32,
                                            _i32, _i32, _vp])
 
+for _name, _at in (("tf_skinny_gemm_act", -1), ("tf_skinny_gemm_swiglu_act", -1), ("tf_skinny_qkv_rope_act", -1),
+                   ("tf_skinny_qkv_rope_gqa_act", -1)):
+    _res, _args = SIGNATURES[_name]
+    SIGNATURES[_name + "_win"] = (_res, _args[:_at] + [_i32, _i32] + _args[_at:])
+SIGNATURES["tf_sg_window_form"] = (_i32, [_i32, _i32, _i32, _c.POINTER(_c.c_int), _c.POINTER(_c.c_int), _c.POINTER(_c.c_int)])
+SIGNATURES["tf_sg_window_perm"] = (_i32, [_i32, _i32, _i32, _i32, _i32, _vp])
+
 ABI_VERSION = 1
 _lib = None
 
diff --git a/triforce_amd/models/llama_core.py b/triforce_amd/models/llama_core.py
--- a/triforce_amd/models/llama_core.py
+++ b/triforce_amd/models/llama_core.py
@@ -178,14 +178,18 @@
         if isinstance(self.lm_head, PL):
             return self
         tied = self.lm_head is self.embed
-        self.lm_head = PL(self.lm_head)
+
+        def win(role, w, split=1):
+            return self.world_size == 1 and ops.window_adopted(role, w.shape[0] // split, w.shape[1])
+
+        self.lm_head = PL(self.lm_head, window=win("lm_head", self.lm_head))
         if tied:
             self.embed = self.lm_head.w
         rope = (self.H_local, self.D) if self.Hkv == self.H else (self.H_local, self.Hkv_local, self.D)
-        self.wqkv = [PL(w, rope=rope) for w in self.wqkv]
-        self.wo = [PL(w) for w in self.wo]
-        self.wgu = [PL(w, split=2) for w in self.wgu]
-        self.wd = [PL(w) for w in self.wd]
+        self.wqkv = [PL(w, rope=rope, window=win("qkv", w)) for w in self.wqkv]
+        self.wo = [PL(w, window=win("o", w)) for w in self.wo]
+        self.wgu = [PL(w, split=2, window=win("gate_up", w, 2)) for w in self.wgu]
+        self.wd = [PL(w, window=win("down", w)) for w in self.wd]
         if self.retrieval_fp8:
             self.build_fp8_()
         return self
diff --git a/triforce_amd/ops.py b/triforce_amd/ops.py
--- a/triforce_amd/ops.py
+++ b/triforce_amd/ops.py
@@ -120,6 +120,53 @@
     _SG_WS[device] = ws
 
 
+WINDOW_MODE = _os.environ.get("TRIFORCE_GEMM_WINDOW", "1")
+if WINDOW_MODE not in ("0", "1", "all"):
+    raise ValueError(f"TRIFORCE_GEMM_WINDOW={WINDOW_MODE!r}: expected 0, 1 or all")
+WINDOW_ENABLED = WINDOW_MODE != "0"
+WINDOW_ROLES = ("down", "lm_head")
+WINDOW_ROLES_ALL = ("qkv", "gate_up", "down", "lm_head")
+WINDOW_MIN_BYTES = 64 << 20
+SG_PLAIN, SG_GATEUP, SG_F32, SG_QKV, SG_QKVG = 0, 1, 2, 3, 4
+_WINDOW_PERMS = {}
+
+
+def window_form(mode, N, K):
+    import ctypes
+    wv, P, U = ctypes.c_int(0), ctypes.c_int(0), ctypes.c_int(0)
+    if hip.lib().tf_sg_window_form(mode, N, K, ctypes.byref(wv), ctypes.byref(P), ctypes.byref(U)) != 1:
+        return None
+    return wv.value, P.value, U.value
+
+
+def window_perm(NP, NC, form, device=None):
+    key = (NP, NC, form[0], form[2], str(device))
+    if key not in _WINDOW_PERMS:
+        perm = torch.empty(NP * NC, dtype=torch.int64)
+        hip.check(hip.lib().tf_sg_window_perm(NP, NC, form[0], form[1], form[2], perm.data_ptr()), "tf_sg_window_perm")
+        _WINDOW_PERMS[key] = perm.to(device) if device is not None else perm
+    return _WINDOW_PERMS[key]
+
+
+def pack_weight_window(w, form):
+    N, K = w.shape
+    wp = pack_weight(w)
+    perm = window_perm(N // 16, K // 32, form, w.device)
+    return wp.view(-1, 512).index_select(0, perm).view(wp.shape)
+
+
+def unpack_weight_window(wp, form):
+    NP, NC = wp.shape[0], wp.shape[1]
+    tiles = torch.empty_like(wp).view(-1, 512)
+    tiles[window_perm(NP, NC, form, wp.device)] = wp.view(-1, 512)
+    return tiles.view(NP, NC, 4, 16, 8).permute(0, 3, 1, 2, 4).reshape(NP * 16, NC * 32)
+
+
+def window_adopted(role, N, K):
+    roles = WINDOW_ROLES_ALL if WINDOW_MODE == "all" else WINDOW_ROLES
+    return WINDOW_ENABLED and role in roles and N * K * 2 >= WINDOW_MIN_BYTES
+
+
 def _rope3(rope):
     return (rope[0], rope[0], rope[1]) if len(rope) == 2 else tuple(rope)
 
@@ -131,7 +178,7 @@
 
 class PackedLinear:
 
-    def __init__(self, w, split=1, pack=None, rope=None):
+    def __init__(self, w, split=1, pack=None, rope=None, window=False):
         self.w = w
         self.N, self.K = w.shape
         self.split = split
@@ -139,7 +186,15 @@
         ok = pack and (self.N // split) % 16 == 0 and self.K % 32 == 0
         if ok and w.is_cuda:
             _ensure_sg_workspace(w.device)
-        self.parts = [pack_weight(b) for b in w.chunk(split, dim=0)] if ok else None
+        self.win = self.win_rope = None
+        gqa = rope is not None and len(rope) == 3 and rope[1] != rope[0]
+        if ok and window and WINDOW_ENABLED and not gqa:
+            form = window_form(SG_GATEUP if split == 2 else SG_QKV if rope is not None else SG_PLAIN, self.N // split, self.K)
+            if rope is not None:
+                self.win_rope = form
+            else:
+                self.win = form
+        self.parts = [self._pack(b, self.win) for b in w.chunk(split, dim=0)] if ok else None
         self.wp = self.parts[0] if (ok and split == 1) else None
         self.rope = rope
         self.wp_rope = None
@@ -147,7 +202,9 @@
         if rope is not None and len(rope) == 3 and not self.gqa:
             self.rope = rope = (rope[0], rope[2])
         if ok and rope is not None and rope[-1] % 32 == 0 and self.N == _rope_rows(rope):
-            self.wp_rope = pack_weight(w[rope_row_order(*_rope3(rope), w.device)])
+            self.wp_rope = self._pack(w[rope_row_order(*_rope3(rope), w.device)], self.win_rope)
+        else:
+            self.win_rope = None
         self.parts_n8 = self.wp_rope_n8 = None
         if ok and w.is_cuda and split == 2 and n8_applies(self.N // split, self.K):
             self.parts_n8 = [pack_weight_n8(b) for b in w.chunk(split, dim=0)]
@@ -155,12 +212,16 @@
             self.wp_rope_n8 = pack_weight_n8(w[rope_row_order_n8(rope[0], rope[1], w.device)])
         self.fp8 = None
 
+    @staticmethod
+    def _pack(w, form):
+        return pack_weight(w) if form is None else pack_weight_window(w, form)
+
     def refresh_(self):
         if self.parts is not None:
             for dst, blk in zip(self.parts, self.w.chunk(self.split, dim=0)):
-                dst.copy_(pack_weight(blk))
+                dst.copy_(self._pack(blk, self.win))
         if self.wp_rope is not None:
-            self.wp_rope.copy_(pack_weight(self.w[rope_row_order(*_rope3(self.rope), self.w.device)]))
+            self.wp_rope.copy_(self._pack(self.w[rope_row_order(*_rope3(self.rope), self.w.device)], self.win_rope))
         if self.parts_n8 is not None:
             for dst, blk in zip(self.parts_n8, self.w.chunk(self.split, dim=0)):
                 dst.copy_(pack_weight_n8(blk))
@@ -413,6 +474,11 @@
                                                        _ptr(ss_in), rp, rsm, rsk, _ptr(ss_out), yp, ysm, ysk, M, w.N, w.K,
                                                        1 if out_f32 else 0, _stream()), "tf_skinny_gemm_fp8_act")
             return out
+        if w.win is not None:
+            hip.check(hip.lib().tf_skinny_gemm_act_win(_ptr(w.wp), xp, xsm, xsk, _ptr(ln), float(eps), _ptr(ss_in), rp, rsm, rsk,
+                                                       _ptr(ss_out), yp, ysm, ysk, M, w.N, w.K, 1 if out_f32 else 0,
+                                                       w.win[0], w.win[1], _stream()), "tf_skinny_gemm_act_win")
+            return out
         hip.check(hip.lib().tf_skinny_gemm_act(_ptr(w.wp), xp, xsm, xsk, _ptr(ln), float(eps), _ptr(ss_in), rp, rsm, rsk,
                                                _ptr(ss_out), yp, ysm, ysk, M, w.N, w.K, 1 if out_f32 else 0, _stream()),
                   "tf_skinny_gemm_act")
@@ -447,6 +513,11 @@
             hip.check(hip.lib().tf_skinny_gemm_swiglu_n8(_ptr(wgu.parts_n8[0]), _ptr(wgu.parts_n8[1]), hp, hsm, hsk, _ptr(ln),
                                                          float(eps), _ptr(ss_in), ap, asm, ask, M, I, wgu.K, _stream()),
                       "tf_skinny_gemm_swiglu_n8")
+            return act
+        if wgu.win is not None:
+            hip.check(hip.lib().tf_skinny_gemm_swiglu_act_win(_ptr(wgu.parts[0]), _ptr(wgu.parts[1]), hp, hsm, hsk, _ptr(ln),
+                                                              float(eps), _ptr(ss_in), ap, asm, ask, M, I, wgu.K,
+                                                              wgu.win[0], wgu.win[1], _stream()), "tf_skinny_gemm_swiglu_act_win")
             return act
         hip.check(hip.lib().tf_skinny_gemm_swiglu_act(_ptr(wgu.parts[0]), _ptr(wgu.parts[1]), hp, hsm, hsk, _ptr(ln),
                                                       float(eps), _ptr(ss_in), ap, asm, ask, M, I, wgu.K, _stream()),
@@ -497,6 +568,13 @@
                                                   _ptr(v_layer), st, sh, int(slot0), _ptr(slot0_dev), rows, H, D, wqkv.K,
                                                   1 if rotate_k else 0, _stream()), "tf_skinny_qkv_rope_n8")
         return q
+    if wqkv.win_rope is not None:
+        hip.check(hip.lib().tf_skinny_qkv_rope_act_win(_ptr(wqkv.wp_rope), xp, xsm, xsk, _ptr(ln), float(eps), _ptr(ss_in),
+                                                       _ptr(cos), _ptr(sin), _ptr(positions), _ptr(q), _ptr(k_layer),
+                                                       _ptr(v_layer), st, sh, int(slot0), _ptr(slot0_dev), rows, H, D, wqkv.K,
+                                                       1 if rotate_k else 0, wqkv.win_rope[0], wqkv.win_rope[1], _stream()),
+                  "tf_skinny_qkv_rope_act_win")
+        return q
     hip.check(hip.lib().tf_skinny_qkv_rope_act(_ptr(wqkv.wp_rope), xp, xsm, xsk, _ptr(ln), float(eps), _ptr(ss_in),
                                                _ptr(cos), _ptr(sin), _ptr(positions), _ptr(q), _ptr(k_layer),
                                                _ptr(v_layer), st, sh, int(slot0), _ptr(slot0_dev), rows, H, D, wqkv.K,
@@ -964,6 +1042,8 @@
         return None
     if any(w.wp_rope is None for w in wqkv) or any(w.split != 2 for w in wgu) or not embed.is_cuda:
         return None
+    if any(w.win is not None or w.win_rope is not None for w in ws):
+        return None
     m = hip.TfDraftModel()
     m.embed = embed.data_ptr()
     for i in range(L):
```

Result: no change. 241.1 (-0.2%).
